# zichunhao/lgn-autoencoder

Measured on AMD Instinct MI355X. Metric: jets/sec fwd+bwd, 30-particle maxdim=2 bs=512, higher is better.
Workload: dtype f64

## Files before the change

### include/lgn_amd.h

```cpp
#ifndef LGN_AMD_H
#define LGN_AMD_H

#include <stddef.h>
#include <stdint.h>

#ifdef __cplusplus
extern "C" {
#endif

#define LGN_AMD_ABI_VERSION 19

int lgn_abi_version(void);
const char* lgn_last_error(void);

int lgn_level_fwd_f64(int B, int N, int C, int CO, int decoder,
                      const double* s_in, const double* v_in, const double* p, const uint8_t* mask,
                      const double* ra, const double* rb, const double* rc,
                      const double* w0, const double* b0, const double* w1, const double* b1,
                      const double* wm0, const double* wm1,
                      double* ag0, double* ag1, double* s_out, double* v_out, void* stream);

int lgn_level_bwd_partial_rows(int B, int N, int decoder, int* rows_mix, int* rows_rad);
int lgn_level_rad_partial_len(int C, int decoder);
int lgn_level_jet_split(int B, int N);

int lgn_level_bwd_f64(int B, int N, int C, int CO, int decoder,
                      const double* s_in, const double* v_in, const double* p, const uint8_t* mask,
                      const double* ra, const double* rb, const double* rc,
                      const double* w0, const double* b0, const double* w1, const double* b1,
                      const double* wm0, const double* wm1, const double* ag0, const double* ag1,
                      const double* g_s_out, const double* g_v_out,
                      double* g_ag, double* g_s_in, double* g_v_in, double* g_p,
                      double* part_mix, double* part_rad, void* stream);

int lgn_cg_product_fwd_f64(int R, int N, int C, int D1, int D2, int DO, int mode, int nnz, const int* row_ptr, const int* col,
                           const double* coef, const double* x1, const double* x2, double* out, void* stream);
int lgn_cg_product_bwd_f64(int R, int N, int C, int D1, int D2, int DO, int mode, int nnz, const int* row_ptr, const int* col,
                           const double* coef, const double* x1, const double* x2, const double* g_out, double* g_x1, double* g_x2,
                           void* stream);

int lgn_reduce_partials_f64(const double* part, int rows, int n, double* out, int accumulate, void* stream);

int lgn_radial_finalize_f64(const double* tot, int C, const double* ra, const double* rb, const double* rc,
                            const double* w0, const double* w1,
                            double* g_a, double* g_b, double* g_c,
                            double* g_w0, double* g_b0, double* g_w1, double* g_b1, void* stream);

#define LGN_ACT_LEAKYRELU 0
#define LGN_ACT_RELU 1
#define LGN_ACT_ELU 2
#define LGN_ACT_SIGMOID 3
#define LGN_ACT_LOGSIGMOID 4
#define LGN_ACT_ATAN 5
#define LGN_ACT_COUNT 6
int lgn_cgmlp_fwd_f64(int M, int C, int H, int nlin, int activation, const double* const* w, const double* const* b,
                      const double* s_in, double* s_out, void* stream);
int lgn_cgmlp_partial_rows(int M, int H);
int lgn_cgmlp_bwd_f64(int M, int C, int H, int nlin, int activation, const double* const* w, const double* const* b,
                      const double* s_in, const double* g_out, double* g_in, double* part, int psize, void* stream);

int lgn_mixreps_fwd_f64(int rows, int Cin, int Cout, int d, const double* w, const double* x, double* y, void* stream);
int lgn_mixreps_partial_rows(int rows);
int lgn_mixreps_bwd_f64(int rows, int Cin, int Cout, int d, const double* w, const double* x, const double* g_y,
                        double* g_x, double* part, void* stream);

int lgn_moments_fwd_f64(int B, int N, int C, int Q, int decoder, const double* X, const double* p, const uint8_t* mask,
                        const double* ra, const double* rb, const double* rc, const double* w0, const double* b0,
                        const double* w1, const double* b1, double* U, void* stream);
long long lgn_moments_scratch_doubles(int B, int N, int C, int decoder);
int lgn_moments_bwd_f64(int B, int N, int C, int Q, int decoder, const double* X, const double* p, const uint8_t* mask,
                        const double* ra, const double* rb, const double* rc, const double* w0, const double* b0,
                        const double* w1, const double* b1, const double* gU, double* gX, double* g_p,
                        double* part_rad, double* scratch, void* stream);

typedef struct lgn_local_tables {
  int n_rows, n_out, n_w;
  int n_terms, n_u, n_x;
  int n_units, static_kind;
  const int *row_ptr, *t_type, *t_a, *t_b;
  const double* t_coef;
  const int *out_dim, *out_nblk, *out_row0, *out_q0, *out_w0;
  const int *u_ptr, *u_row;
  const double* u_coef;
  const int *x_ptr, *x_row, *x_other;
  const double* x_coef;
  int h_out_w0[8];
} lgn_local_tables;

int lgn_local_fwd_f64(int nodes, int C, int CO, int Q, int Qout, const lgn_local_tables* t, const double* X, const double* U,
                      const double* wcat, double* out, void* stream);
int lgn_local_partial_rows(int nodes);
int lgn_local_bwd_f64(int nodes, int C, int CO, int Q, int Qout, const lgn_local_tables* t, const double* X, const double* U,
                      const double* wcat, const double* g_out, double* gU, double* gX, double* part, void* stream);

long long lgn_local_static_packed_doubles(int kind, int C, int CO);
int lgn_local_bwd_static_f64(int kind, int nodes, int C, int CO, const double* XT, const double* UT, const double* wcat,
                             const int* w0, double* wpacked, const double* goT, double* gUT, double* gXT, double* part,
                             double* gpacked, double* g_wcat, void* stream);
int lgn_local_fwd_static_f64(int kind, int nodes, int C, int CO, const double* XT, const double* UT, const double* wcat,
                             const int* w0, double* wpacked, double* outT, double* s_copy, int q_s, void* stream);

typedef struct lgn_net_desc {
  int B, N;
  int n_levels;
  int enc_channels[5];
  int dec_channels[5];
  int tau_s, tau_v;
  int mlp_hidden_mul;
  int mlp_nlin;
  int tau_v_in;
  const lgn_local_tables* enc_tables[4];
  const lgn_local_tables* dec_tables[4];
  int enc_Q[5], enc_qs[5], enc_qv[5];
  int dec_Q[5], dec_qs[5], dec_qv[5];
  int flags;
  int activation;
  int n_in_scalars;
  int latent_pool;
  int dec_N;
  int get_real;
  double jet_loss_scale;
} lgn_net_desc;
#define LGN_REAL_SUM 0
#define LGN_REAL_REAL 1
#define LGN_REAL_IMAG 2
#define LGN_REAL_MEAN 3
#define LGN_REAL_NORM 4
#define LGN_LOSS_CHAMFER 0
#define LGN_LOSS_MSE 1
#define LGN_LOSS_HUNGARIAN 2
typedef struct lgn_loss_desc {
  int kind;
  int abs_coord;
  int polar_coord;
  double scale;
} lgn_loss_desc;
#define LGN_POOL_MIN 0
#define LGN_POOL_MAX 1
#define LGN_POOL_MEAN 2
#define LGN_POOL_MIX 3
#define LGN_POOL(n, avg, o0, o1, o2, o3) ((n) | ((avg) << 3) | ((o0) << 4) | ((o1) << 6) | ((o2) << 8) | ((o3) << 10))
#define LGN_NET_NO_STATIC 1
#define LGN_NET_DEC_PAIRWISE 2
#define LGN_NET_LEVEL_V2 4
#define LGN_NET_MLP_V1 8
#define LGN_NET_MOMENTS_V1 16
#define LGN_NET_BWD_ORDERED 64
#define LGN_NET_DEC_UNFUSED 256
#define LGN_NET_MOMENTS_SPLIT 512
#define LGN_NET_MLP_BWD1 1024
#define LGN_NET_MLP_FULLTILE 2048
#define LGN_NET_SPLIT_TAIL 128

#define LGN_LDS_LIMIT (160 * 1024)
long long lgn_encoder_end_lds_bytes(int N, int C0, int K, int CL, int Ts, int Tv, int pool);
long long lgn_decoder_end_lds_bytes(int N, int C0, int Tin, int CL);
long long lgn_junction_lds_bytes(int N, int CL, int Ts, int Tv, int pool, int C0);

int lgn_step_param_slots(const lgn_net_desc* d, int decoder);
long long lgn_step_workspace_doubles(const lgn_net_desc* d);
int lgn_step_fwd_bwd_f64(const lgn_net_desc* d, const double* params, double* grads, long long n_params,
                         const int64_t* enc_off, const int64_t* dec_off, const double* p4, const double* target,
                         const uint8_t* mask, const double* in_scalars, double* workspace, long long workspace_doubles,
                         double* recon, double* loss_part, const lgn_loss_desc* loss, int* assignment ,
                         int* status , void* stream);
#define LGN_FINALIZE_SCRATCH 2048
int lgn_step_finalize_f64(double* params, double* grads, long long n_params, const double* loss_part, int n_loss,
                          double l1_lambda, double* adam_m, double* adam_v, long long* step_dev,
                          double lr, double beta1, double beta2, double eps, int do_adam, double* loss_out, void* stream);
int lgn_step_train_f64(const lgn_net_desc* d, double* params, double* grads, long long n_params, const int64_t* enc_off,
                       const int64_t* dec_off, const double* p4, const double* target, const uint8_t* mask, const double* in_scalars,
                       double* workspace, long long workspace_doubles, double* recon, double* loss_part, int n_loss, double l1_lambda,
                       double* adam_m, double* adam_v, long long* step_dev, double lr, double beta1, double beta2, double eps,
                       int do_adam, double* loss_out, const lgn_loss_desc* loss, int* assignment ,
                       int* status , void* stream);

#define LGN_OPT_ADAM 0
#define LGN_OPT_RMSPROP 1
typedef struct {
  int kind;
  double l1_lambda, l2_lambda, lr, eps;
  double beta1, beta2;
  double alpha, momentum;
} lgn_optim_desc;
#define LGN_FINALIZE_OPT_SCRATCH 4096
int lgn_step_finalize_opt_f64(double* params, double* grads, long long n_params, const double* loss_part, int n_loss,
                              const lgn_optim_desc* opt, double* state_m, double* state_v, long long* step_dev, int do_step,
                              double* loss_out, void* stream);
int lgn_step_train_opt_f64(const lgn_net_desc* d, double* params, double* grads, long long n_params, const int64_t* enc_off,
                           const int64_t* dec_off, const double* p4, const double* target, const uint8_t* mask,
                           const double* in_scalars, double* workspace, long long workspace_doubles, double* recon,
                           double* loss_part, int n_loss, const lgn_optim_desc* opt, double* state_m, double* state_v,
                           long long* step_dev, int do_step, double* loss_out, const lgn_loss_desc* loss,
                           int* assignment , int* status , void* stream);

long long lgn_eval_workspace_doubles(const lgn_net_desc* d);
int lgn_step_eval_f64(const lgn_net_desc* d, const double* params, const int64_t* enc_off, const int64_t* dec_off,
                      const double* p4_scaled, const double* p4_target, const uint8_t* mask, const double* in_scalars,
                      double* workspace, long long workspace_doubles, double* recon_real, double* lat_s ,
                      double* lat_v , double* loss_part, double* loss_out, const lgn_loss_desc* loss,
                      int* assignment , int* status , void* stream);

long long lgn_net_workspace_doubles(const lgn_net_desc* d, int decoder, int which);
int lgn_encoder_fwd_f64(const lgn_net_desc* d, const double* params, const int64_t* off, const double* p4, const uint8_t* mask,
                        const double* in_scalars, double* act, long long act_doubles, double* lat_s, double* lat_v, void* stream);
int lgn_encoder_bwd_f64(const lgn_net_desc* d, const double* params, double* grads, long long n_params, const int64_t* off,
                        const double* p4, const uint8_t* mask, const double* in_scalars, const double* act, long long act_doubles,
                        const double* g_lat_s, const double* g_lat_v, double* scratch, long long scratch_doubles, void* stream);
int lgn_decoder_fwd_f64(const lgn_net_desc* d, const double* params, const int64_t* off, const double* lat_v, double* act,
                        long long act_doubles, double* recon, void* stream);
int lgn_decoder_bwd_f64(const lgn_net_desc* d, const double* params, double* grads, long long n_params, const int64_t* off,
                        const double* lat_v, const double* act, long long act_doubles, const double* g_recon, double* g_lat_v,
                        double* scratch, long long scratch_doubles, void* stream);

int lgn_chamfer_f64(int B, int N, int M, const double* x, const double* y, int jet_features, double* loss_part, double* gx, double* gy,
                    void* stream);

#define LGN_ANOMALY_NMAX 192
#define LGN_ANOMALY_NSCORES 21
#define LGN_ANOMALY_ALL 0x1FFFFF
#define LGN_ANOMALY_HUNGARIAN 0x403E0
#define LGN_ANOMALY_NO_HUNGARIAN (LGN_ANOMALY_ALL & ~LGN_ANOMALY_HUNGARIAN)
int lgn_anomaly_scores_f64(const double* recons, const double* target, const double* recons_n, const double* target_n, int B, int N,
                           int score_mask, double* scores, int* col4row , int* status, void* stream);

#define LGN_ROC_TILE 2048
#define LGN_ROC_MAX_COLS 65535
#define LGN_ROC_NONFINITE 1
#define LGN_ROC_SINGLE_CLASS 2
#define LGN_ROC_BAD_LABEL 4
#define LGN_ROC_NAN 8
long long lgn_roc_workspace_bytes(long long M, int K);
int lgn_roc_auc_f64(const double* scores, long long M, int ld, int K, const double* labels, double* fpr, double* tpr,
                    double* thresholds, int* length, double* auc, int* flipped, int* status, void* workspace,
                    long long workspace_bytes, void* stream);

#define LGN_EMD_NMAX 191
#define LGN_EMD_INVALID 1
#define LGN_EMD_EMPTY 2
#define LGN_EMD_ITER 4
#define LGN_EMD_INFEASIBLE 8
long long lgn_emd_workspace_bytes(int B, int N);
long long lgn_emd_lds_bytes(int N);
int lgn_emd_f64(const double* ev0, const double* ev1, int B, int n, int m, double R, double* emd, double* flow ,
                double* dual0 , double* dual1 , int* status, void* work, long long work_bytes, void* stream);
int lgn_emd_relative_f64(const double* recons, const double* target, int B, int N, double* emd, int* status, void* work,
                         long long work_bytes, void* stream);
int lgn_emd_debug_max_augmentations(int* out, int reset);

int lgn_linear_sum_assignment_f64(const double* cost, int B, int n, int* col4row, int* status, void* stream);

int lgn_recon_analysis_f64(const double* target, const double* recons, int B, int N, int abs_coord, int find_match,
                           double* part_polar , double* part_polarrel , double* jet_cart, double* jet_polar,
                           double* jet_rel_err, uint8_t* jet_keep, double* rel_err , int* col4row ,
                           uint8_t* is_padded, int* status, void* stream);

int lgn_match_rel_err_f64(const double* target3, const double* recons3, const double* target_polar, const double* recons_polar,
                          const double* target_polarrel, const double* recons_polarrel, int B, int N, double* rel_err,
                          int* col4row , uint8_t* is_padded, int* status, void* stream);

#define LGN_HIST_MAX_EDGES 1025
#define LGN_HIST_MAX_COLS 16
int lgn_histogram_f64(const double* x, long long rows, int ld, int cols, const double* edges, const int* n_edges , int max_edges,
                      const uint8_t* keep , const double* weights , long long* counts, double* wcounts,
                      int max_bins, void* stream);

#define LGN_STATS_TILE 2048
#define LGN_STATS_MAX_COLS 16
#define LGN_STATS_EMPTY 1
#define LGN_STATS_NONFINITE 2
#define LGN_STAT_MEDIAN 0
#define LGN_STAT_IQR 1
#define LGN_STAT_FIRST_QUARTILE 2
#define LGN_STAT_THIRD_QUARTILE 3
#define LGN_STAT_IDR 4
#define LGN_STAT_MAD 5
#define LGN_STAT_MEAN 6
#define LGN_STAT_MAX 7
#define LGN_STAT_MIN 8
#define LGN_STAT_ABS_MIN 9
#define LGN_STAT_STD_DEV 10
#define LGN_STAT_SKEW 11
#define LGN_STAT_KURTOSIS 12
#define LGN_STAT_FWHM 13
#define LGN_STAT_ABS_MEAN 14
#define LGN_STAT_ABS_MEAN_WITHIN_IQR 15
#define LGN_STAT_ABS_MEAN_WITHIN_IDR 16
#define LGN_STAT_Q10 17
#define LGN_STAT_Q90 18
#define LGN_STATS_COUNT 19
long long lgn_column_stats_workspace_bytes(long long rows, int cols);
int lgn_column_stats_f64(const double* x, long long rows, int ld, int cols, const uint8_t* mask , int mask_keep,
                         double alpha, int num_edges, double* stats ,
                         double* edges , long long* kept ,
                         int* status , void* workspace, long long workspace_bytes, void* stream);

int lgn_hist_fwhm_f64(const long long* counts, int max_bins, const double* edges, int max_edges, const int* n_edges , int cols,
                      double* fwhm , void* stream);

#define LGN_JET_IMAGE_MAX_NPIX 64
#define LGN_JET_IMAGE_PARTS 512
long long lgn_jet_images_workspace_bytes(int B, int npix);
int lgn_jet_images_f64(const double* jets, const double* frame_jets , int B, int N, int mode, int npix, double maxR,
                       int first_n, double* images , double* average, void* workspace, long long workspace_bytes,
                       void* stream);

#define LGN_EQUI_TILE 256
#define LGN_EQUI_MAX_PARTS 64
int lgn_transform_jets_f64(const double* p4, const double* R, const int* perm , const double* scalars , int T,
                           int B, int N, int K, double* out, double* scalars_out , void* stream);
long long lgn_rep_deviation_workspace_bytes(int parts, int T, int B, const int* N , const int* C ,
                                            const int* d );
int lgn_rep_deviation_f64(int parts, int T, int B, const double* const* a , const double* const* b ,
                          const double* const* D , const int* N , const int* C , const int* d ,
                          const int* perm , double* stats , void* workspace, long long workspace_bytes,
                          void* stream);

int lgn_hungarian_mse_f64(int B, int N, const double* x, const double* y, int kind, int abs_coord, int polar_coord, double scale,
                          double* loss_part, double* gx, int* assignment , int* status ,
                          void* stream);
long long lgn_assign_loss_lds_bytes(int N, int C);

#define LGN_NORM_NONE 0
#define LGN_NORM_COMPONENT_MAX 1
#define LGN_NORM_OVERALL_MAX 2
#define LGN_NORM_JET_E 3
int lgn_stage_batch_f64(const double* p4, const uint8_t* labels , const double* scalars , int B, int B_pad, int N,
                        int method, double scale, int jet_features, int K, double* p4_in, double* target, uint8_t* mask,
                        double* in_scalars , double* factor, void* stream);
int lgn_denormalize_f64(const double* x0, const double* x1 , const double* factor, int B, int N, double* out0,
                        double* out1 , void* stream);

#define LGN_EPOCH_MAX_COLLECT 4
#define LGN_EPOCH_BAD_INDEX 1
int lgn_stage_gather_f64(const double* p4, const uint8_t* labels , const double* scalars , long long M,
                         const int* index, long long count, const long long* cursor, int B_pad, int N, int method, double scale,
                         int jet_features, int K, double* p4_in, double* target, uint8_t* mask, double* in_scalars ,
                         double* factor, int* status, void* stream);
int lgn_epoch_collect_f64(const double* loss, double* epoch, long long* cursor, long long count, int B, int n,
                          const double* const* src , double* const* dst , const int* row_doubles , void* stream);
int lgn_epoch_reset(long long* cursor, double* epoch, int* status, void* stream);

#ifdef __cplusplus
}
#endif
#endif
```

### lgn-autoencoder_amd/csrc/api_common.cpp

```cpp
#include <stdarg.h>
#include <stdlib.h>

#include "level.hpp"
#include "../../include/lgn_amd.h"

namespace lgn {
static thread_local char g_err[512] = "";
void set_error(const char* fmt, ...) {
  va_list ap;
  va_start(ap, fmt);
  vsnprintf(g_err, sizeof(g_err), fmt, ap);
  va_end(ap);
}
int level_flags_from_env() {
  auto on = [](const char* name) { const char* e = getenv(name); return e && e[0] == '1'; };
  return (on("LGN_AMD_DEC_PAIRWISE") ? LVL_DEC_PAIRWISE : 0) | (on("LGN_AMD_LEVEL_V2") ? LVL_LEVEL_V2 : 0) |
         (on("LGN_AMD_MOMENTS_V1") ? LVL_MOMENTS_V1 : 0) | (on("LGN_AMD_MLP_V1") ? LVL_MLP_V1 : 0) | (on("LGN_AMD_BWD_ORDERED") ? LVL_BWD_ORDERED : 0) |
         (on("LGN_AMD_MOMENTS_SPLIT") ? LVL_MOMENTS_SPLIT : 0) | (on("LGN_AMD_MLP_BWD1") ? LVL_MLP_BWD1 : 0) |
         (on("LGN_AMD_MLP_FULLTILE") ? LVL_MLP_FULLTILE : 0);
}
static_assert(LVL_DEC_PAIRWISE == LGN_NET_DEC_PAIRWISE && LVL_LEVEL_V2 == LGN_NET_LEVEL_V2 && LVL_MOMENTS_V1 == LGN_NET_MOMENTS_V1 &&
                  LVL_MLP_V1 == LGN_NET_MLP_V1 && LVL_MLP_BWD1 == LGN_NET_MLP_BWD1 && LVL_MLP_FULLTILE == LGN_NET_MLP_FULLTILE &&
                  LVL_BWD_ORDERED == LGN_NET_BWD_ORDERED && LVL_MOMENTS_SPLIT == LGN_NET_MOMENTS_SPLIT, "LVL_* and LGN_NET_* are the same bits");
}

extern "C" {
const char* lgn_last_error(void) { return lgn::g_err; }
int lgn_abi_version(void) { return LGN_AMD_ABI_VERSION; }
}
```

### lgn-autoencoder_amd/csrc/level.hpp

```cpp
#pragma once
#include "common.hpp"

namespace lgn {

constexpr int LVL_DEC_PAIRWISE = 2;
constexpr int LVL_LEVEL_V2 = 4;
constexpr int LVL_MLP_V1 = 8;
constexpr int LVL_MOMENTS_V1 = 16;
constexpr int LVL_MLP_BWD1 = 1024;
constexpr int LVL_MLP_FULLTILE = 2048;
constexpr int LVL_MOMENTS_SPLIT = 512;
constexpr int LVL_BWD_ORDERED = 64;
int level_flags_from_env();

template <typename T>
struct LevelArgs {
  int B, N, C, CO;
  const T* s_in;
  const T* v_in;
  const T* p;
  const uint8_t* mask;
  const T *ra, *rb, *rc, *w0, *b0, *w1, *b1;
  const T *wm0, *wm1;
  T* ag0;
  T* ag1;
  T* s_out;
  T* v_out;
  const T* in_w0 = nullptr;
  const T* in_w1 = nullptr;
  T* in_s = nullptr;
  T* in_v = nullptr;
  T* z1 = nullptr;
  size_t z1n = 0;
  T* z2 = nullptr;
  size_t z2n = 0;
  const T* loss_wo1 = nullptr;
  const T* loss_target = nullptr;
  T loss_scale = T(1);
  int loss_real = 0;
  T loss_jscale = T(0);
  T* loss_recon = nullptr;
  T* loss_part = nullptr;
  T* loss_gv = nullptr;
  T* loss_wpart = nullptr;
  int flags = 0;
};

template <typename T>
struct LevelBwdArgs {
  int B, N, C, CO;
  const T *s_in, *v_in, *p;
  const uint8_t* mask;
  const T *ra, *rb, *rc, *w0, *b0, *w1, *b1;
  const T *wm0, *wm1;
  const T *ag0, *ag1;
  const T* g_s_out;
  const T* g_v_out;
  T* g_ag;
  T* g_s_in;
  T* g_v_in;
  T* g_p;
  T* part_mix;
  T* part_rad;
  T* part_in0 = nullptr;
  int flags = 0;
};

__host__ __device__ constexpr int node_stride(int C) { return 10 * C + 4; }

__host__ __device__ constexpr int rad_partial_size(int C, bool dec) {
  return dec ? 2 * C : (2 * 4 * C * NB + 8 * C);
}

inline int level_jet_split(int B, int N) {
  const int groups = (N + 3) / 4;
  int s = 1;
  while (s * 2 <= groups && B * s * 2 <= 512) s *= 2;
  return s;
}

}
```

### lgn-autoencoder_amd/csrc/level_bwd3.hip

```cpp
#include "level_dev.hpp"
#include "ops.hpp"
#include "wave_sum.hpp"

namespace lgn {

typedef double v4d __attribute__((ext_vector_type(4)));

namespace {
__device__ __forceinline__ double dppq(double v, int xor2) {
  int lo = __double2loint(v), hi = __double2hiint(v);
  if (xor2) {
    lo = __builtin_amdgcn_mov_dpp(lo, 0x4E, 0xF, 0xF, true);
    hi = __builtin_amdgcn_mov_dpp(hi, 0x4E, 0xF, 0xF, true);
  } else {
    lo = __builtin_amdgcn_mov_dpp(lo, 0xB1, 0xF, 0xF, true);
    hi = __builtin_amdgcn_mov_dpp(hi, 0xB1, 0xF, 0xF, true);
  }
  return __hiloint2double(hi, lo);
}
__device__ __forceinline__ double quad_sum(double v) {
  v += dppq(v, 0);
  v += dppq(v, 1);
  return v;
}
__device__ __forceinline__ double fast_rcp(double u) {
  double r = __builtin_amdgcn_rcp(u);
  double e = __builtin_fma(-u, r, 1.0);
  r = __builtin_fma(r, e, r);
  e = __builtin_fma(-u, r, 1.0);
  return __builtin_fma(r, e, r);
}
__device__ __forceinline__ void wave_sync() {
  __builtin_amdgcn_fence(__ATOMIC_RELEASE, "workgroup");
  __builtin_amdgcn_wave_barrier();
  __builtin_amdgcn_fence(__ATOMIC_ACQUIRE, "workgroup");
}
template <int C> struct GA3 {
  static constexpr int A3 = 0, A4 = 2 * C, A1 = 4 * C, A2 = 12 * C, SIZE = 20 * C + 2;
};
constexpr int TS = 18;
LGN_STAMP_DECL
}
LGN_STAMP_READER(lgn_debug_stamps_bwd3)

template <int C, bool DEC, int NWV = 4>
struct Bwd3 {
  static constexpr int BLK = 64 * NWV;
  static constexpr int NG = (C + 3) / 4;
  static constexpr int NS = node_stride(C);
  static constexpr int PS = DEC ? 8 : 4;
  static constexpr int TRSZ = DEC ? NWV * 64 : (NWV * (NG + 3) * 16 * TS > NWV * 64 * NG * 12 ? NWV * (NG + 3) * 16 * TS : NWV * 64 * NG * 12);
  static constexpr int MIXP = BLK / (5 * C) < 16 ? BLK / (5 * C) : 16;
  __host__ __device__ static size_t scratch(int N, int CO) {
    size_t p1 = (size_t)N * 10 * CO + 4 * CO * 5 * C + (size_t)N * 20 * C;
    const size_t red = (size_t)MIXP * CO * 5 * C * 4;
    if (red > p1) p1 = red;
    return p1 > (size_t)TRSZ ? p1 : (size_t)TRSZ;
  }
  static constexpr int SMS = 52;
  static constexpr int SEPSZ = DEC ? SMS * C : 0;
  static size_t smem(int N, int CO) {
    return sizeof(double) * ((((size_t)N * NS + 1) & ~size_t(1)) + (size_t)N * (20 * C + 2) + (size_t)N * 10 * C + (size_t)N * PS +
                             scratch(N, CO) + SEPSZ) + N + 16;
  }
};

template <int C, bool DEC, bool SEP, int NWV, bool SYM = false>
__global__ __launch_bounds__(64 * NWV) __attribute__((amdgpu_waves_per_eu(C <= 4 || DEC ? 2 : 1, C <= 4 || DEC ? 2 : 1))) void level_bwd3_kernel(LevelBwdArgs<double> a) {
  static_assert(!SYM || !DEC, "the symmetric sweep is the encoder's");
  using F = Bwd3<C, DEC, NWV>;
  constexpr int BLK = F::BLK;
  using G = GA3<C>;
  constexpr int NG = F::NG, NS = F::NS, PS = F::PS, K = 5 * C;
  const int N = a.N, B = a.B, CO = a.CO;
  const int b = blockIdx.x, tid = threadIdx.x, lane = tid & 63, wave = tid >> 6;
  const int ngroups = (N + 3) >> 2, gper = (ngroups + (int)gridDim.y - 1) / (int)gridDim.y;
  const int glo = min(ngroups, (int)blockIdx.y * gper), ghi = min(ngroups, glo + gper);
  const int nlo = min(N, 4 * glo), nhi = min(N, 4 * ghi);
  const size_t prow = (size_t)b * gridDim.y + blockIdx.y;

  extern __shared__ __align__(16) unsigned char smem_raw[];
  double* nd = reinterpret_cast<double*>(smem_raw);
  double* ga = nd + ((N * NS + 1) & ~1);
  double* gd = ga + N * G::SIZE;
  double* pj = gd + N * 10 * C;
  double* tr = pj + N * PS;
  double* go = tr;
  double* wm = go + N * 10 * CO;
  double* agl = wm + 4 * CO * K;
  double* sm = tr + F::scratch(N, CO);
  uint8_t* mk = reinterpret_cast<uint8_t*>(sm + F::SEPSZ);

  STAMP(0);
  {
    const size_t plo = (size_t)B * N * CO, pa = (size_t)B * N * 2 * C;
    JetRegs<double> jr;
    load_jet_issue<double, C, DEC>(a.s_in, a.v_in, a.p, a.mask, B, N, b, jr);
    const int eg = tid < N * CO ? tid : 0, ea_ = tid < N * 2 * C ? tid : 0, ew = tid < 2 * CO * K ? tid : 0;
    const size_t ig = (size_t)b * N * CO + eg, ia = (size_t)b * N * 2 * C + ea_;
    double rg[10], ra[10];
    rg[0] = a.g_s_out[ig];
    rg[1] = a.g_s_out[plo + ig];
    ra[0] = a.ag0[ia];
    ra[1] = a.ag0[pa + ia];
#pragma unroll
    for (int m = 0; m < 4; ++m) {
      rg[2 + m] = a.g_v_out[ig * 4 + m];
      rg[6 + m] = a.g_v_out[plo * 4 + ig * 4 + m];
      ra[2 + m] = a.ag1[ia * 4 + m];
      ra[6 + m] = a.ag1[(pa + ia) * 4 + m];
    }
    const double w0v = a.wm0[ew], w1v = a.wm1[ew];
    load_jet_commit<double, C, DEC>(a.s_in, a.v_in, a.p, a.mask, B, N, b, jr, nd, pj, mk);
    if (tid < N * CO) {
#pragma unroll
      for (int m = 0; m < 10; ++m) go[tid * 10 + m] = rg[m];
    }
    if (tid < N * 2 * C) {
#pragma unroll
      for (int m = 0; m < 10; ++m) agl[tid * 10 + m] = ra[m];
    }
    if (tid < 2 * CO * K) {
      wm[tid] = w0v;
      wm[2 * CO * K + tid] = w1v;
    }
    for (int e = tid + BLK; e < 2 * CO * K; e += BLK) {
      wm[e] = a.wm0[e];
      wm[2 * CO * K + e] = a.wm1[e];
    }
    for (int e = tid + BLK; e < N * CO; e += BLK) {
      const size_t idx = (size_t)b * N * CO + e;
      double* g = go + e * 10;
      g[0] = a.g_s_out[idx];
      g[1] = a.g_s_out[plo + idx];
#pragma unroll
      for (int m = 0; m < 4; ++m) {
        g[2 + m] = a.g_v_out[idx * 4 + m];
        g[6 + m] = a.g_v_out[plo * 4 + idx * 4 + m];
      }
    }
    for (int e = tid + BLK; e < N * 2 * C; e += BLK) {
      const size_t ea = (size_t)b * N * 2 * C + e;
      double* x = agl + e * 10;
      x[0] = a.ag0[ea];
      x[1] = a.ag0[pa + ea];
#pragma unroll
      for (int m = 0; m < 4; ++m) {
        x[2 + m] = a.ag1[ea * 4 + m];
        x[6 + m] = a.ag1[(pa + ea) * 4 + m];
      }
    }
  }
  __syncthreads();
  STAMP(1);

  {
    const int half = tid >= BLK / 2;
    for (int e = half ? tid - BLK / 2 : tid; e < N * C; e += BLK / 2) {
      const int n = e / C, c = e - n * C;
      const double* w0r = wm + c;
      const double* w1r = wm + 2 * CO * K + c;
      if (half == 0) {
        cx<double> gx0[2] = {{0, 0}, {0, 0}}, gx1[2][4] = {{{0, 0}, {0, 0}, {0, 0}, {0, 0}}, {{0, 0}, {0, 0}, {0, 0}, {0, 0}}};
        for (int o = 0; o < CO; ++o) {
          const double* g = go + (n * CO + o) * 10;
          const cx<double> gs = {g[0], g[1]};
          cx<double> gv[4];
#pragma unroll
          for (int m = 0; m < 4; ++m) gv[m] = {g[2 + m], g[6 + m]};
#pragma unroll
          for (int q = 0; q < 2; ++q) {
            const cx<double> w0 = {w0r[(0 * CO + o) * K + q * C], w0r[(1 * CO + o) * K + q * C]};
            const cx<double> w1 = {w1r[(0 * CO + o) * K + q * C], w1r[(1 * CO + o) * K + q * C]};
            cfmac(gx0[q], gs, w0);
#pragma unroll
            for (int m = 0; m < 4; ++m) cfmac(gx1[q][m], gv[m], w1);
          }
        }
        double* gan = ga + n * G::SIZE;
        gan[G::A3 + 2 * c] = gx0[0].r;  gan[G::A3 + 2 * c + 1] = gx0[0].i;
        gan[G::A4 + 2 * c] = gx0[1].r;  gan[G::A4 + 2 * c + 1] = gx0[1].i;
#pragma unroll
        for (int m = 0; m < 4; ++m) {
          gan[G::A1 + (c * 4 + m) * 2] = gx1[0][m].r;  gan[G::A1 + (c * 4 + m) * 2 + 1] = gx1[0][m].i;
          gan[G::A2 + (c * 4 + m) * 2] = gx1[1][m].r;  gan[G::A2 + (c * 4 + m) * 2 + 1] = gx1[1][m].i;
        }
      } else {
        cx<double> a2 = {0, 0}, a3 = {0, 0}, a4 = {0, 0};
        cx<double> b2[4] = {{0, 0}, {0, 0}, {0, 0}, {0, 0}}, b34[4] = {{0, 0}, {0, 0}, {0, 0}, {0, 0}};
        for (int o = 0; o < CO; ++o) {
          const double* g = go + (n * CO + o) * 10;
          const cx<double> gs = {g[0], g[1]};
          const double* wr0 = w0r + (0 * CO + o) * K;
          const double* wi0 = w0r + (1 * CO + o) * K;
          const double* wr1 = w1r + (0 * CO + o) * K;
          const double* wi1 = w1r + (1 * CO + o) * K;
          cfmac(a2, gs, cx<double>{wr0[2 * C], wi0[2 * C]});
          cfmac(a3, gs, cx<double>{wr0[3 * C], wi0[3 * C]});
          cfmac(a4, gs, cx<double>{wr0[4 * C], wi0[4 * C]});
          const cx<double> w2 = {wr1[2 * C], wi1[2 * C]};
          const cx<double> w34 = {wr1[3 * C] + wr1[4 * C], wi1[3 * C] + wi1[4 * C]};
#pragma unroll
          for (int m = 0; m < 4; ++m) {
            const cx<double> gv = {g[2 + m], g[6 + m]};
            cfmac(b2[m], gv, w2);
            cfmac(b34[m], gv, w34);
          }
        }
        const double* ni = nd + n * NS + c * 10;
        const cx<double> s = {ni[0], ni[1]};
        cx<double> v[4], vt[4];
#pragma unroll
        for (int m = 0; m < 4; ++m) v[m] = {ni[2 + m], ni[6 + m]};
        metric_perm(v, vt);
        cx<double> gs = a2;
        cfmac(gs, cx<double>{2.0 * a4.r, 2.0 * a4.i}, s);
        double* gdn = gd + (n * C + c) * 10;
#pragma unroll
        for (int m = 0; m < 4; ++m) {
          cfmac(gs, b34[m], v[m]);
          cx<double> gv = b2[m];
          cfmac(gv, b34[m], s);
          cfmac(gv, a3, vt[m]);
          gdn[2 + m] = gv.r;
          gdn[6 + m] = gv.i;
        }
        gdn[0] = gs.r;
        gdn[1] = gs.i;
      }
    }
  }
  STAMP(2);
  {
    double* part = a.part_mix + prow * (4 * CO * K);
    constexpr int NPART = F::MIXP;
    const int OK = CO * K, nper = (nhi - nlo + NPART - 1) / NPART;
    const int pi = tid / K, k = tid - pi * K;
    cx<double> d0[8], d1[8];
#pragma unroll
    for (int o = 0; o < 8; ++o) d0[o] = d1[o] = {0, 0};
    if (pi < NPART) {
      const int q = k / C, c = k - q * C;
      const int n1 = min(nhi, nlo + (pi + 1) * nper);
      for (int n = nlo + pi * nper; n < n1; ++n) {
        cx<double> x0, x1[4];
        if (q < 2) {
          const double* x = agl + (n * 2 * C + k) * 10;
          x0 = {x[0], x[1]};
#pragma unroll
          for (int m = 0; m < 4; ++m) x1[m] = {x[2 + m], x[6 + m]};
        } else {
          const double* ni = nd + n * NS + c * 10;
          const cx<double> s = {ni[0], ni[1]};
          cx<double> v[4];
#pragma unroll
          for (int m = 0; m < 4; ++m) v[m] = {ni[2 + m], ni[6 + m]};
          if (q == 2) {
            x0 = s;
#pragma unroll
            for (int m = 0; m < 4; ++m) x1[m] = v[m];
          } else {
            if (q == 3) { x0 = bil2(v, v); x0.r *= 0.5; x0.i *= 0.5; } else x0 = cmul(s, s);
#pragma unroll
            for (int m = 0; m < 4; ++m) x1[m] = cmul(v[m], s);
          }
        }
#pragma unroll
        for (int o = 0; o < 8; ++o)
          if (o < CO) {
            const double* g = go + (n * CO + o) * 10;
            cfmac(d0[o], cx<double>{g[0], g[1]}, x0);
#pragma unroll
            for (int m = 0; m < 4; ++m) cfmac(d1[o], cx<double>{g[2 + m], g[6 + m]}, x1[m]);
          }
      }
    }
    STAMP(48);
    __syncthreads();
    STAMP(49);
    double* red = tr;
    if (pi < NPART) {
#pragma unroll
      for (int o = 0; o < 8; ++o)
        if (o < CO) {
          double* r4 = red + ((pi * CO + o) * K + k) * 4;
          r4[0] = d0[o].r;  r4[1] = d0[o].i;  r4[2] = d1[o].r;  r4[3] = d1[o].i;
        }
    }
    STAMP(50);
    __syncthreads();
    STAMP(51);
    for (int ex = tid; ex < 4 * OK; ex += BLK) {
      const int e = ex >> 2, x = ex & 3;
      double v = red[ex];
#pragma unroll
      for (int pp = 1; pp < NPART; ++pp) v += red[pp * OK * 4 + ex];
      part[x * OK + e] = v;
    }
  }

  if constexpr (DEC && SEP) {
    STAMP(3);
    __syncthreads();
    STAMP(4);
    if (tid < 64) {
      const int k = tid & 7, part = tid >> 3;
      double mean = 0.0;
      for (int n = part; n < N; n += 8) mean += pj[n * 8 + k];
      mean += shfl_xor(mean, 8);
      mean += shfl_xor(mean, 16);
      mean += shfl_xor(mean, 32);
      if (part == 0) sm[k] = mean / N;
    }
    __syncthreads();
    for (int e = tid; e < N * 8; e += BLK) pj[e] -= sm[e & 7];
    __syncthreads();
#define LGN_PUT(k, val)                                       \
  do {                                                        \
    if ((k) < 16) a0[(k) < 16 ? (k) : 0] += (val);                                        \
    else if ((k) < 32) a1[(k) >= 16 && (k) < 32 ? (k) - 16 : 0] += (val);                 \
    else if ((k) < 44) a2[(k) >= 32 && (k) < 44 ? (k) - 32 : 0] += (val);                 \
    else a3[(k) >= 44 ? (k) - 44 : 0] += (val);                                           \
  } while (0)
    for (int c = wave; c < C; c += NWV) {
      double a0[16], a1[16], a2[12], a3[8];
#pragma unroll
      for (int k = 0; k < 16; ++k) a0[k] = a1[k] = 0.0;
#pragma unroll
      for (int k = 0; k < 12; ++k) a2[k] = 0.0;
#pragma unroll
      for (int k = 0; k < 8; ++k) a3[k] = 0.0;
      for (int n = lane; n < N; n += 64) {
        const double* ni = nd + n * NS + c * 10;
        const double* pn = pj + n * 8;
        const double* gi = ga + n * G::SIZE;
        cx<double> pc[4], v[4];
#pragma unroll
        for (int m = 0; m < 4; ++m) {
          pc[m] = {pn[m], pn[4 + m]};
          v[m] = {ni[2 + m], ni[6 + m]};
        }
        const cx<double> sn = {ni[0], ni[1]};
        LGN_PUT(0, sn.r);  LGN_PUT(1, sn.i);
#pragma unroll
        for (int m = 0; m < 4; ++m) {
          LGN_PUT(2 + 2 * m, v[m].r);  LGN_PUT(3 + 2 * m, v[m].i);
          const cx<double> sp = cmul(sn, pc[m]);
          LGN_PUT(10 + 2 * m, sp.r);  LGN_PUT(11 + 2 * m, sp.i);
        }
        const cx<double> vp = bil2(v, pc);
        LGN_PUT(18, vp.r);  LGN_PUT(19, vp.i);
        const cx<double> g3 = {0.5 * gi[G::A3 + 2 * c], 0.5 * gi[G::A3 + 2 * c + 1]};
        LGN_PUT(20, gi[G::A4 + 2 * c]);  LGN_PUT(21, gi[G::A4 + 2 * c + 1]);
        LGN_PUT(22, g3.r);  LGN_PUT(23, g3.i);
        cx<double> gp2 = {0, 0};
#pragma unroll
        for (int m = 0; m < 4; ++m) {
          const cx<double> g1 = {gi[G::A1 + (c * 4 + m) * 2], gi[G::A1 + (c * 4 + m) * 2 + 1]};
          const cx<double> g2 = {gi[G::A2 + (c * 4 + m) * 2], gi[G::A2 + (c * 4 + m) * 2 + 1]};
          LGN_PUT(24 + 2 * m, g1.r);  LGN_PUT(25 + 2 * m, g1.i);
          LGN_PUT(32 + 2 * m, g2.r);  LGN_PUT(33 + 2 * m, g2.i);
          cfmac(gp2, g2, pc[m]);
          const cx<double> gp3 = cmulc(g3, pc[m]);
          LGN_PUT(42 + 2 * m, gp3.r);  LGN_PUT(43 + 2 * m, gp3.i);
        }
        LGN_PUT(40, gp2.r);  LGN_PUT(41, gp2.i);
      }
      double* q = sm + c * F::SMS;
      wave_sum_store<16>(a0, q, lane);
      wave_sum_store<16>(a1, q + 16, lane);
      wave_sum_store<12>(a2, q + 32, lane);
      wave_sum_store<8>(a3, q + 44, lane);
    }
#undef LGN_PUT
    __syncthreads();

    STAMP(5);
    const size_t pls = (size_t)B * N * C;
    for (int e = tid; e < N * C; e += BLK) {
      const int n = e / C, c = e - n * C;
      const double* q = sm + c * F::SMS;
      const double* pn = pj + n * 8;
      const double* gdn = gd + e * 10;
      const cx<double> R0 = {a.b0[c], a.b0[c]}, R1 = {a.b1[c], a.b1[c]};
      const cx<double> e0 = {R0.r - R0.i, R0.r + R0.i};
      cx<double> pc[4], pt[4];
#pragma unroll
      for (int m = 0; m < 4; ++m) pc[m] = {pn[m], pn[4 + m]};
      metric_perm(pc, pt);
      const cx<double> SG4 = {q[20], q[21]}, SG3 = {q[22], q[23]}, GP2 = {q[40], q[41]};
      cx<double> GP3[4], GPT3[4];
#pragma unroll
      for (int m = 0; m < 4; ++m) GP3[m] = {q[42 + 2 * m], q[43 + 2 * m]};
      metric_perm(GP3, GPT3);
      cx<double> u = GP2;
#pragma unroll
      for (int m = 0; m < 4; ++m) {
        const cx<double> t = cmulc(cx<double>{q[32 + 2 * m], q[33 + 2 * m]}, pc[m]);
        u.r -= t.r;  u.i -= t.i;
      }
      cx<double> gs = cmulc(SG4, e0);
      cfmac(gs, u, R1);
      const size_t ge = ((size_t)b * N + n) * C + c;
      a.g_s_in[ge] = gdn[0] + gs.r;
      a.g_s_in[pls + ge] = gdn[1] + gs.i;
#pragma unroll
      for (int m = 0; m < 4; ++m) {
        cx<double> w = GPT3[m];
        const cx<double> t = cmulc(SG3, pt[m]);
        w.r -= t.r;  w.i -= t.i;
        cx<double> gv = cmulc(cx<double>{q[24 + 2 * m], q[25 + 2 * m]}, e0);
        cfmac(gv, w, R1);
        a.g_v_in[ge * 4 + m] = gdn[2 + m] + gv.r;
        a.g_v_in[pls * 4 + ge * 4 + m] = gdn[6 + m] + gv.i;
      }
    }
    STAMP(6);
    {
      const size_t plp = (size_t)B * N * 4;
      for (int e = tid; e < N * 4; e += BLK) {
        const int n = e >> 2, m = e & 3;
        const int mp = m == 1 ? 3 : (m == 3 ? 1 : m);
        const double sg = m == 2 ? -1.0 : 1.0;
        const double* gi = ga + n * G::SIZE;
        cx<double> acc = {0, 0};
        for (int c = 0; c < C; ++c) {
          const double* q = sm + c * F::SMS;
          const double* ni = nd + n * NS + c * 10;
          const cx<double> R1 = {a.b1[c], a.b1[c]};
          const cx<double> S = {q[0], q[1]}, SG3 = {q[22], q[23]};
          const cx<double> VSt = {sg * q[2 + 2 * mp], sg * q[3 + 2 * mp]};
          const cx<double> vt = {sg * ni[2 + mp], sg * ni[6 + mp]};
          const cx<double> g2 = {gi[G::A2 + (c * 4 + m) * 2], gi[G::A2 + (c * 4 + m) * 2 + 1]};
          const cx<double> g3 = {0.5 * gi[G::A3 + 2 * c], 0.5 * gi[G::A3 + 2 * c + 1]};
          cx<double> t = cmulc(g2, S);
          cfmac(t, g3, VSt);
          const cx<double> t2 = cmulc(cx<double>{q[32 + 2 * m], q[33 + 2 * m]}, cx<double>{ni[0], ni[1]});
          t.r -= t2.r;  t.i -= t2.i;
          const cx<double> t3 = cmulc(SG3, vt);
          t.r -= t3.r;  t.i -= t3.i;
          cfmac(acc, t, R1);
        }
        a.g_p[((size_t)b * N + n) * 4 + m] += acc.r;
        a.g_p[plp + ((size_t)b * N + n) * 4 + m] += acc.i;
      }
    }
    if (tid < 2 * C) {
      const int lin = tid / C, c = tid - lin * C;
      const double* q = sm + c * F::SMS;
      const cx<double> S = {q[0], q[1]};
      double* part = a.part_rad + (size_t)blockIdx.x * rad_partial_size(C, true);
      if (lin == 0) {
        cx<double> E0 = cmulc(cx<double>{q[20], q[21]}, S);
#pragma unroll
        for (int m = 0; m < 4; ++m) cfmac(E0, cx<double>{q[24 + 2 * m], q[25 + 2 * m]}, cx<double>{q[2 + 2 * m], q[3 + 2 * m]});
        part[tid] = (E0.r + E0.i) + (E0.i - E0.r);
      } else {
        cx<double> VS[4], VSt[4];
#pragma unroll
        for (int m = 0; m < 4; ++m) VS[m] = {q[2 + 2 * m], q[3 + 2 * m]};
        metric_perm(VS, VSt);
        cx<double> E1 = cmulc(cx<double>{q[40], q[41]}, S);
        cx<double> neg = cmulc(cx<double>{q[22], q[23]}, cx<double>{q[18], q[19]});
#pragma unroll
        for (int m = 0; m < 4; ++m) {
          cfmac(neg, cx<double>{q[32 + 2 * m], q[33 + 2 * m]}, cx<double>{q[10 + 2 * m], q[11 + 2 * m]});
          cfmac(E1, cx<double>{q[42 + 2 * m], q[43 + 2 * m]}, VSt[m]);
        }
        part[tid] = (E1.r - neg.r) + (E1.i - neg.i);
      }
    }
    STAMP(7);
    return;
  }

  STAMP(3);
  const int pr = lane & 15, cg = lane >> 4;
  const int tj = pr >> 2, ti = pr & 3;
  double ak[5], bk[5], ck2[5], wf[NG][5], bias[NG][4];
  if (!DEC) {
#pragma unroll
    for (int s = 0; s < 5; ++s) {
      const int k = 4 * s + cg;
      ak[s] = a.ra[k];
      bk[s] = a.rb[k];
      const double c = a.rc[k];
      ck2[s] = c * c;
    }
#pragma unroll
    for (int g = 0; g < NG; ++g) {
      const int rr = lane & 15, q = rr >> 2, ch = 4 * g + (rr & 3);
      const double* w = (q >> 1) ? a.w1 : a.w0;
#pragma unroll
      for (int s = 0; s < 5; ++s) wf[g][s] = ch < C ? w[(2 * ch + (q & 1)) * NB + 4 * s + cg] : 0.0;
    }
  }
#pragma unroll
  for (int g = 0; g < NG; ++g) {
    const int ch = 4 * g + cg;
#pragma unroll
    for (int q = 0; q < 4; ++q) {
      const double* bb = (q >> 1) ? a.b1 : a.b0;
      bias[g][q] = ch < C ? (DEC ? bb[ch] : bb[2 * ch + (q & 1)]) : 0.0;
    }
  }
  STAMP(4);
  __syncthreads();
  STAMP(5);

  double* trw = tr + wave * (NG + 3) * 16 * TS;
  v4d T[NG][3];
  double dB0[NG], dB1[NG];
#pragma unroll
  for (int g = 0; g < NG; ++g) {
    dB0[g] = dB1[g] = 0.0;
#pragma unroll
    for (int t = 0; t < 3; ++t) T[g][t] = v4d{0, 0, 0, 0};
  }
  const size_t pls = (size_t)B * N * C;
  double in0[NG][4];
#pragma unroll
  for (int g = 0; g < NG; ++g) in0[g][0] = in0[g][1] = in0[g][2] = in0[g][3] = 0.0;
  const int gcount = ghi - glo;
  const int rs = (!SYM && !DEC && NWV == 4 && gcount >= 1 && gcount <= 2) ? NWV / gcount : 1;
  const int rpart = rs > 1 ? wave % rs : 0;
  const int ntl = (N + 3) >> 2, i0lo = rs > 1 ? 4 * (rpart * ntl / rs) : 0, i0hi = rs > 1 ? min(N, 4 * ((rpart + 1) * ntl / rs)) : N;
  for (int u = 0;; ++u) {
    int rg;
    if constexpr (SYM) {
      const int p = wave + NWV * (u >> 1);
      if (p >= (ngroups + 1) >> 1) break;
      rg = (u & 1) ? ngroups - 1 - p : p;
      if ((u & 1) && rg == p) continue;
    } else if (rs > 1) {
      if (u > 0) break;
      rg = glo + wave / rs;
    } else {
      rg = glo + wave + NWV * u;
      if (rg >= ghi) break;
    }
    const int j = rg * 4 + tj;
    const bool jok = j < N;
    const int jj = jok ? j : N - 1;
    double pme[PS];
#pragma unroll
    for (int m = 0; m < PS; ++m) pme[m] = pj[jj * PS + m];
    const bool mj = DEC ? false : (mk[jj] != 0);
    cx<double> Gs[NG], Gv[NG][4], Gq[4];
    cx<double> sj[NG], vj[NG][4], vtj[NG][4];
    cx<double> dvj[NG], svj[NG];
#pragma unroll
    for (int g = 0; g < NG; ++g) {
      Gs[g] = {0, 0};
#pragma unroll
      for (int m = 0; m < 4; ++m) Gv[g][m] = {0, 0};
      const int ch = 4 * g + cg, cs = ch < C ? ch : 0;
      const double* nj = nd + jj * NS + cs * 10;
      sj[g] = {nj[0], nj[1]};
#pragma unroll
      for (int m = 0; m < 4; ++m) vj[g][m] = {nj[2 + m], nj[6 + m]};
      metric_perm(vj[g], vtj[g]);
      dvj[g] = {vj[g][3].r - vj[g][1].r, vj[g][3].i - vj[g][1].i};
      svj[g] = {vj[g][1].r + vj[g][3].r, vj[g][1].i + vj[g][3].i};
    }
#pragma unroll
    for (int m = 0; m < 4; ++m) Gq[m] = {0, 0};

    for (int i0 = i0lo; i0 < i0hi; i0 += 4) {
      if (rg == glo && i0 < 32) STAMP(16 + (i0 >> 2) * 4);
      const int kind = SYM ? ((i0 >> 2) < rg ? 2 : ((i0 >> 2) == rg ? 1 : 0)) : 1;
      const int i = i0 + ti;
      const bool ok = jok && i < N;
      const int ii = i < N ? i : N - 1;
      const double* pii = pj + ii * PS;
      cx<double> q[4];
      v4d R[NG];
      double rho[5], an = 0.0;
      double qd0 = 0.0, qd3 = 0.0, qa = 0.0, qb = 0.0;
      bool on = false;
      if (DEC) {
#pragma unroll
        for (int m = 0; m < 4; ++m) q[m] = {pii[m] - pme[m], pii[4 + m] - pme[4 + m]};
#pragma unroll
        for (int g = 0; g < NG; ++g) R[g] = v4d{bias[g][0], bias[g][1], bias[g][2], bias[g][3]};
      } else {
        const double d0 = pii[0] - pme[0], d1 = pii[1] - pme[1], d2 = pii[2] - pme[2], d3 = pii[3] - pme[3];
        const double q0 = d0 * d0, q1 = d1 * d1, q2 = d2 * d2, q3 = d3 * d3;
        const double nsq = (2.0 * q0 - (((q0 + q1) + q2) + q3)) + 1e-16;
        an = fabs(nsq);
        on = ok && mj && (mk[ii] != 0) && (nsq != 0.0);
        const double h = rsqrt2<double>();
        q[0] = {d0, 0.0};
        q[1] = {d1 * h, -d2 * h};
        q[2] = {d3, 0.0};
        q[3] = {-d1 * h, -d2 * h};
        qd0 = d0;  qd3 = d3;  qa = d1 * h;  qb = d2 * h;
        double beta[5] = {0.0, 0.0, 0.0, 0.0, 0.0};
#pragma unroll
        for (int s = 0; s < 5; ++s) rho[s] = 0.0;
        if (on) {
#pragma unroll
          for (int s = 0; s < 5; ++s) beta[s] = 1.0 + ck2[s] * an;
          rcp5(beta, rho);
#pragma unroll
          for (int s = 0; s < 5; ++s) beta[s] = __builtin_fma(bk[s], rho[s], ak[s]);
        }
#pragma unroll
        for (int g = 0; g < NG; ++g) {
          R[g] = v4d{bias[g][0], bias[g][1], bias[g][2], bias[g][3]};
#pragma unroll
          for (int s = 0; s < 5; ++s) R[g] = __builtin_amdgcn_mfma_f64_16x16x4f64(wf[g][s], beta[s], R[g], 0, 0, 0);
        }
        if (kind != 0) {
          double* xb = trw + NG * 16 * TS;
#pragma unroll
          for (int s = 0; s < 5; ++s) {
            const double x2 = an * rho[s] * rho[s];
            if (s < 4) {
              xb[pr * TS + 4 * s + cg] = rho[s];
              xb[16 * TS + pr * TS + 4 * s + cg] = x2;
            } else {
              xb[32 * TS + pr * TS + cg] = rho[s];
              xb[32 * TS + pr * TS + 4 + cg] = x2;
            }
          }
          xb[32 * TS + pr * TS + 8 + 2 * cg] = cg == 0 ? (on ? 1.0 : 0.0) : 0.0;
          xb[32 * TS + pr * TS + 9 + 2 * cg] = cg == 0 ? (ok ? 1.0 : 0.0) : 0.0;
        }
      }
      if (rg == glo && i0 < 32) STAMP(17 + (i0 >> 2) * 4);
      const double* gi = ga + ii * G::SIZE;
#pragma unroll
      for (int g = 0; g < NG; ++g) {
        const int ch = 4 * g + cg;
        double G0r = 0, G0i = 0, G1r = 0, G1i = 0;
        if (ok && ch < C) {
          const cx<double> R0 = {R[g][0], R[g][1]}, R1 = {R[g][2], R[g][3]};
          const cx<double> e0 = {R0.r - R0.i, R0.r + R0.i};
          const cx<double> gA3 = {0.5 * gi[G::A3 + 2 * ch], 0.5 * gi[G::A3 + 2 * ch + 1]};
          const cx<double> gA4 = {gi[G::A4 + 2 * ch], gi[G::A4 + 2 * ch + 1]};
          cx<double> gA1[4], gA2[4];
#pragma unroll
          for (int m = 0; m < 4; ++m) {
            gA1[m] = {gi[G::A1 + (ch * 4 + m) * 2], gi[G::A1 + (ch * 4 + m) * 2 + 1]};
            gA2[m] = {gi[G::A2 + (ch * 4 + m) * 2], gi[G::A2 + (ch * 4 + m) * 2 + 1]};
          }
          cfmac(Gs[g], gA4, e0);
          cx<double> ge0 = cmulc(gA4, sj[g]);
          cx<double> gR1;
          if (!DEC) {
            const cx<double> dg = {gA2[1].r - gA2[3].r, gA2[1].i - gA2[3].i}, sg = {gA2[1].r + gA2[3].r, gA2[1].i + gA2[3].i};
            cx<double> P2;
            P2.r = __builtin_fma(gA2[0].r, qd0, __builtin_fma(gA2[2].r, qd3, __builtin_fma(qa, dg.r, -qb * sg.i)));
            P2.i = __builtin_fma(gA2[0].i, qd0, __builtin_fma(gA2[2].i, qd3, __builtin_fma(qa, dg.i, qb * sg.r)));
            cfmac(Gs[g], P2, R1);
            const cx<double> Z = cmulc(gA3, R1);
#pragma unroll
            for (int m = 0; m < 4; ++m) cfmac(Gv[g][m], gA1[m], e0);
            Gv[g][0].r = __builtin_fma(Z.r, qd0, Gv[g][0].r);   Gv[g][0].i = __builtin_fma(Z.i, qd0, Gv[g][0].i);
            Gv[g][2].r = __builtin_fma(-Z.r, qd3, Gv[g][2].r);  Gv[g][2].i = __builtin_fma(-Z.i, qd3, Gv[g][2].i);
            const double aZr = qa * Z.r, aZi = qa * Z.i;
            const double bZr = qb * Z.r, bZi = qb * Z.i;
            Gv[g][1].r -= aZr + bZi;  Gv[g][1].i += bZr - aZi;
            Gv[g][3].r += aZr - bZi;  Gv[g][3].i += aZi + bZr;
            gR1 = {0, 0};
            if (kind != 0) {
#pragma unroll
              for (int m = 0; m < 4; ++m) cfmac(ge0, gA1[m], vj[g][m]);
              cx<double> V;
              V.r = __builtin_fma(vj[g][0].r, qd0, __builtin_fma(-vj[g][2].r, qd3, __builtin_fma(qa, dvj[g].r, qb * svj[g].i)));
              V.i = __builtin_fma(vj[g][0].i, qd0, __builtin_fma(-vj[g][2].i, qd3, __builtin_fma(qa, dvj[g].i, -qb * svj[g].r)));
              gR1 = cmulc(P2, sj[g]);
              cfmac(gR1, gA3, V);
            }
            if constexpr (SYM) {
              if (kind == 2) {
                const double* gj = ga + jj * G::SIZE;
                const double* ni = nd + ii * NS + ch * 10;
                const cx<double> si = {ni[0], ni[1]};
                cx<double> vi[4];
#pragma unroll
                for (int m = 0; m < 4; ++m) vi[m] = {ni[2 + m], ni[6 + m]};
                const cx<double> hA3 = {0.5 * gj[G::A3 + 2 * ch], 0.5 * gj[G::A3 + 2 * ch + 1]};
                const cx<double> hA4 = {gj[G::A4 + 2 * ch], gj[G::A4 + 2 * ch + 1]};
                cx<double> he0 = cmulc(hA4, si);
                cx<double> hA2[4];
#pragma unroll
                for (int m = 0; m < 4; ++m) {
                  const cx<double> hA1 = {gj[G::A1 + (ch * 4 + m) * 2], gj[G::A1 + (ch * 4 + m) * 2 + 1]};
                  hA2[m] = {gj[G::A2 + (ch * 4 + m) * 2], gj[G::A2 + (ch * 4 + m) * 2 + 1]};
                  cfmac(he0, hA1, vi[m]);
                }
                const cx<double> hd = {hA2[1].r - hA2[3].r, hA2[1].i - hA2[3].i}, hs = {hA2[1].r + hA2[3].r, hA2[1].i + hA2[3].i};
                cx<double> Q2;
                Q2.r = __builtin_fma(hA2[0].r, qd0, __builtin_fma(hA2[2].r, qd3, __builtin_fma(qa, hd.r, -qb * hs.i)));
                Q2.i = __builtin_fma(hA2[0].i, qd0, __builtin_fma(hA2[2].i, qd3, __builtin_fma(qa, hd.i, qb * hs.r)));
                const cx<double> dvi = {vi[3].r - vi[1].r, vi[3].i - vi[1].i}, svi = {vi[1].r + vi[3].r, vi[1].i + vi[3].i};
                cx<double> W;
                W.r = __builtin_fma(vi[0].r, qd0, __builtin_fma(-vi[2].r, qd3, __builtin_fma(qa, dvi.r, qb * svi.i)));
                W.i = __builtin_fma(vi[0].i, qd0, __builtin_fma(-vi[2].i, qd3, __builtin_fma(qa, dvi.i, -qb * svi.r)));
                cx<double> hR1 = cmulc(Q2, si);
                cfmac(hR1, hA3, W);
                ge0.r += he0.r;  ge0.i += he0.i;
                gR1.r -= hR1.r;  gR1.i -= hR1.i;
              }
            }
          } else {
            cx<double> e1[4], e1t[4];
#pragma unroll
            for (int m = 0; m < 4; ++m) e1[m] = cmul(R1, q[m]);
            metric_perm(e1, e1t);
            gR1 = {0, 0};
#pragma unroll
            for (int m = 0; m < 4; ++m) {
              cfmac(Gv[g][m], gA1[m], e0);
              cfmac(Gv[g][m], gA3, e1t[m]);
              cfmac(Gs[g], gA2[m], e1[m]);
              cfmac(ge0, gA1[m], vj[g][m]);
              cx<double> ge1 = cmulc(gA2[m], sj[g]);
              cfmac(ge1, gA3, vtj[g][m]);
              cfmac(gR1, ge1, q[m]);
              cfmac(Gq[m], ge1, R1);
            }
          }
          G0r = ge0.r + ge0.i;  G0i = ge0.i - ge0.r;
          G1r = gR1.r;  G1i = gR1.i;
        }
        if (DEC) {
          dB0[g] += G0r + G0i;
          dB1[g] += G1r + G1i;
        } else if (kind != 0) {
          double* ta = trw + g * 16 * TS;
          ta[pr * TS + cg] = G0r;
          ta[pr * TS + 4 + cg] = G0i;
          ta[pr * TS + 8 + cg] = G1r;
          ta[pr * TS + 12 + cg] = G1i;
        }
      }
      if (rg == glo && i0 < 32) STAMP(18 + (i0 >> 2) * 4);
      if (!DEC && kind != 0) {
        wave_sync();
        const double* xb = trw + NG * 16 * TS;
#pragma unroll
        for (int s = 0; s < 4; ++s) {
          const int prow = 4 * s + cg;
          double bv[3];
#pragma unroll
          for (int t = 0; t < 3; ++t) bv[t] = xb[t * 16 * TS + prow * TS + pr];
#pragma unroll
          for (int g = 0; g < NG; ++g) {
            const double av = trw[g * 16 * TS + prow * TS + pr];
#pragma unroll
            for (int t = 0; t < 3; ++t) T[g][t] = __builtin_amdgcn_mfma_f64_16x16x4f64(av, bv[t], T[g][t], 0, 0, 0);
          }
        }
        wave_sync();
      }
    }

    if (rg == glo) STAMP(6);
    if (rs > 1) {
      double* mine = trw + lane;
#pragma unroll
      for (int g = 0; g < NG; ++g) {
        Gs[g].r = quad_sum(Gs[g].r);  Gs[g].i = quad_sum(Gs[g].i);
#pragma unroll
        for (int m = 0; m < 4; ++m) { Gv[g][m].r = quad_sum(Gv[g][m].r);  Gv[g][m].i = quad_sum(Gv[g][m].i); }
        if (rpart != 0) {
          mine[(g * 10 + 0) * 64] = Gs[g].r;  mine[(g * 10 + 1) * 64] = Gs[g].i;
#pragma unroll
          for (int m = 0; m < 4; ++m) { mine[(g * 10 + 2 + m) * 64] = Gv[g][m].r;  mine[(g * 10 + 6 + m) * 64] = Gv[g][m].i; }
        }
      }
      __syncthreads();
      if (rpart != 0) break;
      for (int pp = 1; pp < rs; ++pp) {
        const double* oth = trw + pp * (NG + 3) * 16 * TS + lane;
#pragma unroll
        for (int g = 0; g < NG; ++g) {
          Gs[g].r += oth[(g * 10 + 0) * 64];  Gs[g].i += oth[(g * 10 + 1) * 64];
#pragma unroll
          for (int m = 0; m < 4; ++m) { Gv[g][m].r += oth[(g * 10 + 2 + m) * 64];  Gv[g][m].i += oth[(g * 10 + 6 + m) * 64]; }
        }
      }
    }
#pragma unroll
    for (int g = 0; g < NG; ++g) {
      const int ch = 4 * g + cg;
      const double sr = rs > 1 ? Gs[g].r : quad_sum(Gs[g].r), si = rs > 1 ? Gs[g].i : quad_sum(Gs[g].i);
      const bool wr = jok && ti == 0 && ch < C;
      const size_t e = ((size_t)b * N + jj) * C + (ch < C ? ch : 0);
      const double* gdn = gd + (jj * C + (ch < C ? ch : 0)) * 10;
      const double gsr = gdn[0] + sr, gsi = gdn[1] + si;
      if (wr) {
        a.g_s_in[e] = gsr;
        a.g_s_in[pls + e] = gsi;
      }
      cx<double> gvn[4];
#pragma unroll
      for (int m = 0; m < 4; ++m) {
        const double vr = rs > 1 ? Gv[g][m].r : quad_sum(Gv[g][m].r), vi = rs > 1 ? Gv[g][m].i : quad_sum(Gv[g][m].i);
        gvn[m] = {gdn[2 + m] + vr, gdn[6 + m] + vi};
        if (wr) {
          a.g_v_in[e * 4 + m] = gvn[m].r;
          a.g_v_in[pls * 4 + e * 4 + m] = gvn[m].i;
        }
      }
      if constexpr (!DEC) {
        if (a.part_in0 && wr) {
          const double q0 = pme[0] * pme[0], q1 = pme[1] * pme[1], q2 = pme[2] * pme[2], q3 = pme[3] * pme[3];
          const double mass = sqrt(fabs(2.0 * q0 - (((q0 + q1) + q2) + q3)));
          constexpr double H = 0.70710678118654752440084436210484903928;
          const cx<double> q[4] = {{pme[0], 0.0}, {pme[1] * H, -pme[2] * H}, {pme[3], 0.0}, {-pme[1] * H, -pme[2] * H}};
          cx<double> d1 = {0, 0};
#pragma unroll
          for (int m = 0; m < 4; ++m) cfmac(d1, gvn[m], q[m]);
          in0[g][0] += gsr * mass;
          in0[g][1] += gsi * mass;
          in0[g][2] += d1.r;
          in0[g][3] += d1.i;
        }
      }
    }
    if (DEC) {
      const size_t plp = (size_t)B * N * 4;
#pragma unroll
      for (int m = 0; m < 4; ++m) {
        double qr = quad_sum(Gq[m].r), qi = quad_sum(Gq[m].i);
        qr += shfl_xor(qr, 16);  qr += shfl_xor(qr, 32);
        qi += shfl_xor(qi, 16);  qi += shfl_xor(qi, 32);
        if (jok && ti == 0 && cg == 0) {
          a.g_p[((size_t)b * N + jj) * 4 + m] -= qr;
          a.g_p[plp + ((size_t)b * N + jj) * 4 + m] -= qi;
        }
      }
    }
  }

  STAMP(7);
  if (DEC) {
    const int ti2 = pr >> 2, tj2 = pr & 3;
    const size_t plp = (size_t)B * N * 4;
    for (int rg = glo + wave; rg < ghi; rg += NWV) {
      const int i = rg * 4 + ti2;
      const bool iok = i < N;
      const int ii = iok ? i : N - 1;
      const double* gi = ga + ii * G::SIZE;
      cx<double> Gq[4] = {{0, 0}, {0, 0}, {0, 0}, {0, 0}};
      for (int j0 = 0; j0 < N; j0 += 4) {
        const int j = j0 + tj2;
        if (iok && j < N) {
#pragma unroll
          for (int g = 0; g < NG; ++g) {
            const int ch = 4 * g + cg;
            if (ch < C) {
              const double* nj = nd + j * NS + ch * 10;
              const cx<double> s = {nj[0], nj[1]};
              cx<double> v[4], vt[4];
#pragma unroll
              for (int m = 0; m < 4; ++m) v[m] = {nj[2 + m], nj[6 + m]};
              metric_perm(v, vt);
              const cx<double> R1 = {bias[g][2], bias[g][3]};
              const cx<double> gA3 = {0.5 * gi[G::A3 + 2 * ch], 0.5 * gi[G::A3 + 2 * ch + 1]};
#pragma unroll
              for (int m = 0; m < 4; ++m) {
                const cx<double> gA2 = {gi[G::A2 + (ch * 4 + m) * 2], gi[G::A2 + (ch * 4 + m) * 2 + 1]};
                cx<double> ge1 = cmulc(gA2, s);
                cfmac(ge1, gA3, vt[m]);
                cfmac(Gq[m], ge1, R1);
              }
            }
          }
        }
      }
#pragma unroll
      for (int m = 0; m < 4; ++m) {
        double qr = quad_sum(Gq[m].r), qi = quad_sum(Gq[m].i);
        qr += shfl_xor(qr, 16);  qr += shfl_xor(qr, 32);
        qi += shfl_xor(qi, 16);  qi += shfl_xor(qi, 32);
        if (iok && tj2 == 0 && cg == 0) {
          a.g_p[((size_t)b * N + i) * 4 + m] += qr;
          a.g_p[plp + ((size_t)b * N + i) * 4 + m] += qi;
        }
      }
    }
  }

  __shared__ double in0l[NWV][8][4];
  if constexpr (!DEC) {
    if (a.part_in0) {
#pragma unroll
      for (int g = 0; g < NG; ++g)
#pragma unroll
        for (int k = 0; k < 4; ++k) {
          double x = in0[g][k];
          x += shfl_xor(x, 4);
          x += shfl_xor(x, 8);
          if (pr == 0 && 4 * g + cg < C) in0l[wave][4 * g + cg][k] = x;
        }
    }
  }

  STAMP(8);
  __syncthreads();
  STAMP(9);
  if constexpr (!DEC) {
    if (a.part_in0 && tid < 4 * C) {
      const int k = tid / C, c = tid - k * C;
      double s = 0;
#pragma unroll
      for (int w = 0; w < NWV; ++w) s += in0l[w][c][k];
      a.part_in0[prow * 4 * C + k * C + c] = s;
    }
  }
  double* part = a.part_rad + prow * rad_partial_size(C, DEC);
  if (DEC) {
    double* red = tr;
#pragma unroll
    for (int g = 0; g < NG; ++g) {
      double x0 = dB0[g], x1 = dB1[g];
      for (int m = 1; m < 16; m <<= 1) { x0 += shfl_xor(x0, m); x1 += shfl_xor(x1, m); }
      if (pr == 0) {
        red[(wave * NG + g) * 8 + cg] = x0;
        red[(wave * NG + g) * 8 + 4 + cg] = x1;
      }
    }
    __syncthreads();
    if (tid < 2 * C) {
      const int lin = tid / C, ch = tid - lin * C, g = ch >> 2, c4 = ch & 3;
      double s = 0;
      for (int w = 0; w < NWV; ++w) s += red[(w * NG + g) * 8 + lin * 4 + c4];
      part[tid] = s;
    }
  } else {
    double* red = tr;
    {
      double* mine = red + (size_t)(wave * 64 + lane) * NG * 12;
#pragma unroll
      for (int g = 0; g < NG; ++g)
#pragma unroll
        for (int t = 0; t < 3; ++t)
#pragma unroll
          for (int q = 0; q < 4; ++q) mine[(g * 3 + t) * 4 + q] = T[g][t][q];
    }
    __syncthreads();
    const int wq = __builtin_amdgcn_readfirstlane(wave);
    if (wq < 4) {
      constexpr int R = 4 * C;
      const int col = lane & 15;
#pragma unroll
      for (int g = 0; g < NG; ++g) {
        const int ch = 4 * g + cg;
#pragma unroll
        for (int t = 0; t < 3; ++t)
#pragma unroll
          for (int q = 0; q < 4; ++q) {
            if (q != wq) continue;
            const int e = (g * 3 + t) * 4 + q;
            double v = (red[(size_t)(0 * 64 + lane) * NG * 12 + e] + red[(size_t)(1 * 64 + lane) * NG * 12 + e]) +
                       (red[(size_t)(2 * 64 + lane) * NG * 12 + e] + red[(size_t)(3 * 64 + lane) * NG * 12 + e]);
            if (NWV == 8)
              v += (red[(size_t)(4 * 64 + lane) * NG * 12 + e] + red[(size_t)(5 * 64 + lane) * NG * 12 + e]) +
                   (red[(size_t)(6 * 64 + lane) * NG * 12 + e] + red[(size_t)(7 * 64 + lane) * NG * 12 + e]);
            if (ch >= C) continue;
            const int r = (q >> 1) * 2 * C + 2 * ch + (q & 1);
            if (t == 0) part[r * NB + col] = v;
            else if (t == 1) part[R * NB + r * NB + col] = v;
            else {
              if (col < 4) part[r * NB + 16 + col] = v;
              else if (col < 8) part[R * NB + r * NB + 16 + (col - 4)] = v;
              else if (col == 8) part[2 * R * NB + r] = v;
              else if (col == 9) part[2 * R * NB + R + r] = v;
            }
          }
      }
    }
  }
  STAMP(10);
}

bool level_bwd3_fits(int N) { return N <= 40; }

template <int C, bool DEC, bool SEP, int NWV>
static int launch_bwd3_w(const LevelBwdArgs<double>& a, int split, hipStream_t stream) {
  size_t smem = Bwd3<C, DEC, NWV>::smem(a.N, a.CO);
  LGN_CHECK_ARG(smem <= 160 * 1024, "level_bwd: N=%d C=%d needs %zu B of LDS", a.N, a.C, smem);
  LGN_CHECK_ARG(a.CO <= 8, "level_bwd: C_out=%d unsupported (1..8)", a.CO);
  auto kern = level_bwd3_kernel<C, DEC, SEP, NWV>;
  if constexpr (!DEC && C <= 4) {
    if (split == 1 && !(a.flags & LVL_BWD_ORDERED)) kern = level_bwd3_kernel<C, DEC, SEP, NWV, true>;
  }
  if (smem > 64 * 1024) (void)hipFuncSetAttribute(reinterpret_cast<const void*>(kern), hipFuncAttributeMaxDynamicSharedMemorySize, (int)smem);
  hipLaunchKernelGGL(kern, dim3(a.B, split), dim3(64 * NWV), smem, stream, a);
  LGN_CHECK_LAUNCH();
  return 0;
}
template <int C, bool DEC, bool SEP>
static int launch_bwd3(const LevelBwdArgs<double>& a, hipStream_t stream) {
  return launch_bwd3_w<C, DEC, SEP, 4>(a, SEP ? 1 : level_jet_split(a.B, a.N), stream);
}

int level_bwd3_dispatch(const LevelBwdArgs<double>& a, int decoder, hipStream_t stream) {
  const bool pairwise = (a.flags & LVL_DEC_PAIRWISE) != 0;
#define LGN_CASE(CC)                                                                \
  case CC:                                                                          \
    if (!decoder) return launch_bwd3<CC, false, false>(a, stream);                  \
    return pairwise ? launch_bwd3<CC, true, false>(a, stream) : launch_bwd3<CC, true, true>(a, stream);
  switch (a.C) {
#ifdef LGN_DEV_ONLY_C4
    LGN_CASE(4)
#else
    LGN_CASE(1) LGN_CASE(2) LGN_CASE(3) LGN_CASE(4) LGN_CASE(5) LGN_CASE(6) LGN_CASE(7) LGN_CASE(8)
#endif
    default: set_error("level_bwd: C_in=%d unsupported (1..8)", a.C); return -1;
  }
#undef LGN_CASE
}

}
```

### lgn-autoencoder_amd/csrc/level_fwd2.hip

```cpp
#include "level_dev.hpp"
#include "net_dev.hpp"
#include "ops.hpp"
#include "wave_sum.hpp"

namespace lgn {

typedef double v4d __attribute__((ext_vector_type(4)));
LGN_STAMP_DECL
LGN_STAMP_READER(lgn_debug_stamps_fwd2)

__device__ __forceinline__ double dpp_quad(double v, int ctrl_is_xor2) {
  int lo = __double2loint(v), hi = __double2hiint(v);
  if (ctrl_is_xor2) {
    lo = __builtin_amdgcn_mov_dpp(lo, 0x4E, 0xF, 0xF, true);
    hi = __builtin_amdgcn_mov_dpp(hi, 0x4E, 0xF, 0xF, true);
  } else {
    lo = __builtin_amdgcn_mov_dpp(lo, 0xB1, 0xF, 0xF, true);
    hi = __builtin_amdgcn_mov_dpp(hi, 0xB1, 0xF, 0xF, true);
  }
  return __hiloint2double(hi, lo);
}
__device__ __forceinline__ double quad_sum(double v) {
  v += dpp_quad(v, 0);
  v += dpp_quad(v, 1);
  return v;
}

__device__ __forceinline__ double fast_rcp(double u) {
  double r = __builtin_amdgcn_rcp(u);
  double e = __builtin_fma(-u, r, 1.0);
  r = __builtin_fma(r, e, r);
  e = __builtin_fma(-u, r, 1.0);
  return __builtin_fma(r, e, r);
}

template <int C, bool DEC>
struct Fwd2 {
  static constexpr int NG = (C + 3) / 4;
  static constexpr int NS = node_stride(C);
  static constexpr int PS = DEC ? 8 : 4;
  static constexpr int AGS = 20 * C;
  static constexpr int A3 = 0, A4 = 2 * C, A1 = 4 * C, A2 = 12 * C;
};

template <int C, bool DEC, bool SEP, bool TRAIN>
__global__ __launch_bounds__(2 * BLOCK) void level_fwd2_kernel(LevelArgs<double> a, int chunk) {
  using F = Fwd2<C, DEC>;
  constexpr int NG = F::NG;
  const int N = a.N, B = a.B, CO = a.CO;
  const int b = blockIdx.x, tid = threadIdx.x, lane = tid & 63, wave = tid >> 6;
  const int nthr = blockDim.x, nw = nthr >> 6;

  extern __shared__ __align__(16) unsigned char smem_raw[];
  double* nd = reinterpret_cast<double*>(smem_raw);
  double* pj = nd + ((N * F::NS + 1) & ~1);
  double* wm = pj + N * F::PS;
  double* agl = wm + 4 * CO * 5 * C;
  double* sums = agl + chunk * F::AGS;
  uint8_t* mk = reinterpret_cast<uint8_t*>(sums + 20 * C);

  STAMP(0);
  if (!DEC && a.in_w0) {
    {
      const size_t wg = (size_t)blockIdx.y * gridDim.x + blockIdx.x, stride = (size_t)gridDim.x * gridDim.y * nthr;
      for (size_t e = wg * nthr + tid; e < a.z1n; e += stride) a.z1[e] = 0.0;
      for (size_t e = wg * nthr + tid; e < a.z2n; e += stride) a.z2[e] = 0.0;
    }
    const double* p0 = a.p + (size_t)b * N * 4;
    const size_t plane_s = (size_t)B * N * C;
    const int nw2 = 2 * CO * 5 * C;
    for (int e = tid; e < N * 4; e += nthr) pj[e] = p0[e];
    for (int e = tid; e < N; e += nthr) mk[e] = a.mask[(size_t)b * N + e];
    for (int e = tid; e < nw2; e += nthr) {
      wm[e] = a.wm0[e];
      wm[nw2 + e] = a.wm1[e];
    }
    for (int e = tid; e < N * C; e += nthr) {
      const int j = e / C, c = e - j * C;
      const double* p = p0 + j * 4;
      const double pe = p[0], px = p[1], py = p[2], pz = p[3];
      const double q0 = pe * pe, q1 = px * px, q2 = py * py, q3 = pz * pz;
      const double mass = sqrt(fabs(2.0 * q0 - (((q0 + q1) + q2) + q3)));
      constexpr double H = 0.70710678118654752440084436210484903928;
      const cx<double> q[4] = {{pe, 0.0}, {px * H, -py * H}, {pz, 0.0}, {-px * H, -py * H}};
      const double w0r = a.in_w0[c], w0i = a.in_w0[C + c];
      const cx<double> w1 = {a.in_w1[c], a.in_w1[C + c]};
      double* d = nd + j * F::NS + c * 10;
      d[0] = w0r * mass;
      d[1] = w0i * mass;
#pragma unroll
      for (int m = 0; m < 4; ++m) {
        const cx<double> r = cmul(w1, q[m]);
        d[2 + m] = r.r;
        d[6 + m] = r.i;
      }
      if (blockIdx.y == 0) {
        const size_t ge = (size_t)b * N * C + e;
        a.in_s[ge] = d[0];
        a.in_s[plane_s + ge] = d[1];
#pragma unroll
        for (int m = 0; m < 4; ++m) {
          a.in_v[ge * 4 + m] = d[2 + m];
          a.in_v[plane_s * 4 + ge * 4 + m] = d[6 + m];
        }
      }
    }
  } else {
    JetRegs<double> jr;
    load_jet_issue<double, C, DEC>(a.s_in, a.v_in, a.p, a.mask, B, N, b, jr);
    const int nw2 = 2 * CO * 5 * C, ew = tid < nw2 ? tid : 0;
    const double w0v = a.wm0[ew], w1v = a.wm1[ew];
    load_jet_commit<double, C, DEC>(a.s_in, a.v_in, a.p, a.mask, B, N, b, jr, nd, pj, mk);
    if (tid < nw2) {
      wm[tid] = w0v;
      wm[nw2 + tid] = w1v;
    }
    for (int e = tid + nthr; e < nw2; e += nthr) {
      wm[e] = a.wm0[e];
      wm[nw2 + e] = a.wm1[e];
    }
  }

  const int pr = lane & 15, cg = lane >> 4;
  const int ti = pr >> 2, tj = pr & 3;
  double ak[5], bk[5], ck2[5];
  double wf[NG][5];
  double bias[NG][4];
  if (!DEC) {
#pragma unroll
    for (int s = 0; s < 5; ++s) {
      const int k = 4 * s + cg;
      ak[s] = a.ra[k];
      bk[s] = a.rb[k];
      const double c = a.rc[k];
      ck2[s] = c * c;
    }
#pragma unroll
    for (int g = 0; g < NG; ++g) {
      const int rr = lane & 15, q = rr >> 2, ch = 4 * g + (rr & 3);
      const double* w = (q >> 1) ? a.w1 : a.w0;
#pragma unroll
      for (int s = 0; s < 5; ++s) wf[g][s] = ch < C ? w[(2 * ch + (q & 1)) * NB + 4 * s + cg] : 0.0;
    }
  }
#pragma unroll
  for (int g = 0; g < NG; ++g) {
    const int ch = 4 * g + cg;
#pragma unroll
    for (int q = 0; q < 4; ++q) {
      const double* bb = (q >> 1) ? a.b1 : a.b0;
      bias[g][q] = ch < C ? (DEC ? bb[ch] : bb[2 * ch + (q & 1)]) : 0.0;
    }
  }
  __syncthreads();
  STAMP(1);

  if constexpr (DEC && SEP) {
    if (tid < 64) {
      const int k = tid & 7, part = tid >> 3;
      double mean = 0.0;
      for (int n = part; n < N; n += 8) mean += pj[n * 8 + k];
      mean += shfl_xor(mean, 8);
      mean += shfl_xor(mean, 16);
      mean += shfl_xor(mean, 32);
      if (part == 0) sums[k] = mean / N;
    }
    __syncthreads();
    for (int e = tid; e < N * 8; e += nthr) pj[e] -= sums[e & 7];
    __syncthreads();
#define LGN_PUT(k, val)                                           \
  do {                                                            \
    if ((k) < 12) a0[(k) < 12 ? (k) : 0] += (val);                \
    else a1[(k) >= 12 ? (k) - 12 : 0] += (val);                   \
  } while (0)
    for (int c = wave; c < C; c += nw) {
      double a0[12], a1[8];
#pragma unroll
      for (int k = 0; k < 12; ++k) a0[k] = 0.0;
#pragma unroll
      for (int k = 0; k < 8; ++k) a1[k] = 0.0;
      for (int n = lane; n < N; n += 64) {
        const double* ni = nd + n * F::NS + c * 10;
        const double* pn = pj + n * 8;
        const cx<double> sn = {ni[0], ni[1]};
        cx<double> v[4], pc[4];
#pragma unroll
        for (int m = 0; m < 4; ++m) {
          v[m] = {ni[2 + m], ni[6 + m]};
          pc[m] = {pn[m], pn[4 + m]};
        }
        LGN_PUT(0, sn.r);  LGN_PUT(1, sn.i);
#pragma unroll
        for (int m = 0; m < 4; ++m) {
          LGN_PUT(2 + 2 * m, v[m].r);  LGN_PUT(3 + 2 * m, v[m].i);
          const cx<double> sp = cmul(sn, pc[m]);
          LGN_PUT(10 + 2 * m, sp.r);  LGN_PUT(11 + 2 * m, sp.i);
        }
        const cx<double> vp = bil2(v, pc);
        LGN_PUT(18, vp.r);  LGN_PUT(19, vp.i);
      }
      wave_sum_store<12>(a0, sums + c * 20, lane);
      wave_sum_store<8>(a1, sums + c * 20 + 12, lane);
    }
#undef LGN_PUT
    __syncthreads();
  }

  const int ngroups = (N + 3) >> 2, gper = (ngroups + (int)gridDim.y - 1) / (int)gridDim.y;
  const int rlo = min(N, 4 * (int)blockIdx.y * gper), rhi = min(N, rlo + 4 * gper);
  auto catmix = [&](int c0, int c1) {
    constexpr int K = 5 * C;
    const int nr = c1 - c0;
    const size_t plo = (size_t)B * N * CO;
    if (wave == 0) {
      for (int rl = lane; rl < nr; rl += 64) {
        const int r = c0 + rl;
        const double* st = agl + rl * F::AGS;
        const double* ni = nd + r * F::NS;
        cx<double> x[K];
#pragma unroll
        for (int c = 0; c < C; ++c) {
          const cx<double> sc = {ni[c * 10], ni[c * 10 + 1]};
          cx<double> v[4];
#pragma unroll
          for (int mm = 0; mm < 4; ++mm) v[mm] = {ni[c * 10 + 2 + mm], ni[c * 10 + 6 + mm]};
          cx<double> vv = bil2(v, v);
          vv.r *= 0.5;  vv.i *= 0.5;
          x[c] = {st[F::A3 + 2 * c], st[F::A3 + 2 * c + 1]};
          x[C + c] = {st[F::A4 + 2 * c], st[F::A4 + 2 * c + 1]};
          x[2 * C + c] = sc;
          x[3 * C + c] = vv;
          x[4 * C + c] = cmul(sc, sc);
        }
#pragma unroll 2
        for (int o = 0; o < CO; ++o) {
          const double* wr = wm + (0 * CO + o) * K;
          const double* wi = wm + (1 * CO + o) * K;
          cx<double> acc = {0, 0};
#pragma unroll
          for (int k = 0; k < K; ++k) cfma(acc, cx<double>{wr[k], wi[k]}, x[k]);
          const size_t e = ((size_t)b * N + r) * CO + o;
          a.s_out[e] = acc.r;
          a.s_out[plo + e] = acc.i;
        }
      }
    } else {
      for (int it = lane + 64 * (wave - 1); it < nr * 4; it += 64 * (nw - 1)) {
        const int rl = it >> 2, m = it & 3, r = c0 + rl;
        const double* st = agl + rl * F::AGS;
        const double* ni = nd + r * F::NS;
        cx<double> x[K];
#pragma unroll
        for (int c = 0; c < C; ++c) {
          const cx<double> sc = {ni[c * 10], ni[c * 10 + 1]};
          const cx<double> v = {ni[c * 10 + 2 + m], ni[c * 10 + 6 + m]};
          x[c] = {st[F::A1 + (c * 4 + m) * 2], st[F::A1 + (c * 4 + m) * 2 + 1]};
          x[C + c] = {st[F::A2 + (c * 4 + m) * 2], st[F::A2 + (c * 4 + m) * 2 + 1]};
          x[2 * C + c] = v;
          x[3 * C + c] = x[4 * C + c] = cmul(v, sc);
        }
#pragma unroll 2
        for (int o = 0; o < CO; ++o) {
          const double* wr = wm + 2 * CO * K + (0 * CO + o) * K;
          const double* wi = wm + 2 * CO * K + (1 * CO + o) * K;
          cx<double> acc = {0, 0};
#pragma unroll
          for (int k = 0; k < K; ++k) cfma(acc, cx<double>{wr[k], wi[k]}, x[k]);
          const size_t e = ((size_t)b * N + r) * CO + o;
          a.v_out[e * 4 + m] = acc.r;
          a.v_out[plo * 4 + e * 4 + m] = acc.i;
        }
      }
    }
    };
  for (int c0 = rlo; c0 < rhi; c0 += chunk) {
  const int c1 = min(rhi, c0 + chunk);
  if constexpr (DEC && SEP) {
    for (int e = tid; e < (c1 - c0) * C; e += nthr) {
      const int rl = e / C, c = e - rl * C, n = c0 + rl;
      const double* sm = sums + c * 20;
      const double* pn = pj + n * 8;
      const cx<double> R0 = {a.b0[c], a.b0[c]}, R1 = {a.b1[c], a.b1[c]};
      const cx<double> e0 = {R0.r - R0.i, R0.r + R0.i};
      const cx<double> S = {sm[0], sm[1]};
      cx<double> VS[4], pc[4];
#pragma unroll
      for (int m = 0; m < 4; ++m) {
        VS[m] = {sm[2 + 2 * m], sm[3 + 2 * m]};
        pc[m] = {pn[m], pn[4 + m]};
      }
      double* st = agl + rl * F::AGS;
      const cx<double> a4 = cmul(S, e0);
      cx<double> t = bil2(VS, pc);
      t.r -= sm[18];  t.i -= sm[19];
      cx<double> a3 = cmul(R1, t);
      st[F::A3 + 2 * c] = 0.5 * a3.r;  st[F::A3 + 2 * c + 1] = 0.5 * a3.i;
      st[F::A4 + 2 * c] = a4.r;        st[F::A4 + 2 * c + 1] = a4.i;
#pragma unroll
      for (int m = 0; m < 4; ++m) {
        const cx<double> a1 = cmul(VS[m], e0);
        cx<double> u = cmul(pc[m], S);
        u.r -= sm[10 + 2 * m];  u.i -= sm[11 + 2 * m];
        const cx<double> a2 = cmul(R1, u);
        st[F::A1 + (c * 4 + m) * 2] = a1.r;  st[F::A1 + (c * 4 + m) * 2 + 1] = a1.i;
        st[F::A2 + (c * 4 + m) * 2] = a2.r;  st[F::A2 + (c * 4 + m) * 2 + 1] = a2.i;
      }
    }
  } else {
  const int ngr = (c1 - c0 + 3) >> 2;
  const int rs = (!DEC && nw == 4 && ngr >= 1 && ngr <= 2 && chunk >= 16) ? 4 / ngr : 1;
  const int rpart = rs > 1 ? wave % rs : 0, ntl = (N + 3) >> 2;
  auto row_group = [&](const int rg, const int jlo, const int jhi, const int slab) __attribute__((always_inline)) {
    const int i0 = rg * 4;
    const int i = i0 + ti;
    const bool iok = i < N;
    const int ii = iok ? i : N - 1;
    double pi[F::PS];
#pragma unroll
    for (int m = 0; m < F::PS; ++m) pi[m] = pj[ii * F::PS + m];
    const bool mi = DEC ? false : (mk[ii] != 0);

    cx<double> A1[NG][4], A2[NG][4], A3[NG], A4[NG];
#pragma unroll
    for (int g = 0; g < NG; ++g) {
      A3[g] = {0, 0};
      A4[g] = {0, 0};
#pragma unroll
      for (int m = 0; m < 4; ++m) { A1[g][m] = {0, 0}; A2[g][m] = {0, 0}; }
    }

    STAMP(2 + ((rg >> 2) & 3) * 4);
    struct Tile {
      cx<double> q[4];
      double qd0, qd3, qa, qb;
      v4d R[NG];
      int jj;
      bool ok;
    };
    auto prep = [&](int j0, Tile& T) {
      const int j = j0 + tj;
      T.ok = iok && j < N;
      T.jj = j < N ? j : N - 1;
      const double* pjj = pj + T.jj * F::PS;
      if (DEC) {
#pragma unroll
        for (int m = 0; m < 4; ++m) T.q[m] = {pi[m] - pjj[m], pi[4 + m] - pjj[4 + m]};
#pragma unroll
        for (int g = 0; g < NG; ++g) T.R[g] = v4d{bias[g][0], bias[g][1], bias[g][2], bias[g][3]};
      } else {
        const double d0 = pi[0] - pjj[0], d1 = pi[1] - pjj[1], d2 = pi[2] - pjj[2], d3 = pi[3] - pjj[3];
        const double q0 = d0 * d0, q1 = d1 * d1, q2 = d2 * d2, q3 = d3 * d3;
        const double nsq = (2.0 * q0 - (((q0 + q1) + q2) + q3)) + 1e-16;
        const double an = fabs(nsq);
        const bool on = T.ok && mi && (mk[T.jj] != 0) && (nsq != 0.0);
        const double h = rsqrt2<double>();
        T.qd0 = d0;  T.qd3 = d3;  T.qa = d1 * h;  T.qb = d2 * h;
        double beta[5] = {0.0, 0.0, 0.0, 0.0, 0.0};
        if (on) {
#pragma unroll
          for (int s = 0; s < 5; ++s) beta[s] = 1.0 + ck2[s] * an;
          double rho5[5];
          rcp5(beta, rho5);
#pragma unroll
          for (int s = 0; s < 5; ++s) beta[s] = __builtin_fma(bk[s], rho5[s], ak[s]);
        }
#pragma unroll
        for (int g = 0; g < NG; ++g) {
          T.R[g] = v4d{bias[g][0], bias[g][1], bias[g][2], bias[g][3]};
#pragma unroll
          for (int s = 0; s < 5; ++s) T.R[g] = __builtin_amdgcn_mfma_f64_16x16x4f64(wf[g][s], beta[s], T.R[g], 0, 0, 0);
        }
      }
    };
    auto agg = [&](const Tile& T) {
      if (T.ok) {
        const double* nj = nd + T.jj * F::NS;
#pragma unroll
        for (int g = 0; g < NG; ++g) {
          const int ch = 4 * g + cg;
          if (ch < C) {
            const cx<double> R0 = {T.R[g][0], T.R[g][1]}, R1 = {T.R[g][2], T.R[g][3]};
            const cx<double> e0 = {R0.r - R0.i, R0.r + R0.i};
            const cx<double> sj = {nj[ch * 10], nj[ch * 10 + 1]};
            cx<double> vj[4];
#pragma unroll
            for (int m = 0; m < 4; ++m) {
              vj[m] = {nj[ch * 10 + 2 + m], nj[ch * 10 + 6 + m]};
              cfma(A1[g][m], vj[m], e0);
            }
            cfma(A4[g], sj, e0);
            if (!DEC) {
              const double qd0 = T.qd0, qd3 = T.qd3, qa = T.qa, qb = T.qb;
              const cx<double> Tm = cmul(sj, R1);
              A2[g][0].r = __builtin_fma(Tm.r, qd0, A2[g][0].r);  A2[g][0].i = __builtin_fma(Tm.i, qd0, A2[g][0].i);
              A2[g][2].r = __builtin_fma(Tm.r, qd3, A2[g][2].r);  A2[g][2].i = __builtin_fma(Tm.i, qd3, A2[g][2].i);
              const double aTr = qa * Tm.r, aTi = qa * Tm.i, bTr = qb * Tm.r, bTi = qb * Tm.i;
              A2[g][1].r += aTr + bTi;  A2[g][1].i += aTi - bTr;
              A2[g][3].r += bTi - aTr;  A2[g][3].i -= aTi + bTr;
              const cx<double> dv = {vj[3].r - vj[1].r, vj[3].i - vj[1].i}, sv = {vj[1].r + vj[3].r, vj[1].i + vj[3].i};
              cx<double> V;
              V.r = __builtin_fma(vj[0].r, qd0, __builtin_fma(-vj[2].r, qd3, __builtin_fma(qa, dv.r, qb * sv.i)));
              V.i = __builtin_fma(vj[0].i, qd0, __builtin_fma(-vj[2].i, qd3, __builtin_fma(qa, dv.i, -qb * sv.r)));
              cfma(A3[g], R1, V);
            } else {
              cx<double> e1[4];
#pragma unroll
              for (int m = 0; m < 4; ++m) {
                e1[m] = cmul(R1, T.q[m]);
                cfma(A2[g][m], sj, e1[m]);
              }
              const cx<double> t = bil2(vj, e1);
              A3[g].r += t.r;
              A3[g].i += t.i;
            }
          }
        }
      }
    };
    if (jlo < jhi) {
      Tile ta, tb;
      prep(jlo, ta);
      int j0 = jlo;
      while (true) {
        if (j0 + 4 < jhi) prep(j0 + 4, tb);
        agg(ta);
        j0 += 4;
        if (j0 >= jhi) break;
        if (j0 + 4 < jhi) prep(j0 + 4, ta);
        agg(tb);
        j0 += 4;
        if (j0 >= jhi) break;
      }
    }

    STAMP(3 + ((rg >> 2) & 3) * 4);
#pragma unroll
    for (int g = 0; g < NG; ++g) {
      A3[g].r = quad_sum(A3[g].r) * 0.5;  A3[g].i = quad_sum(A3[g].i) * 0.5;
      A4[g].r = quad_sum(A4[g].r);        A4[g].i = quad_sum(A4[g].i);
#pragma unroll
      for (int m = 0; m < 4; ++m) {
        A1[g][m].r = quad_sum(A1[g][m].r);  A1[g][m].i = quad_sum(A1[g][m].i);
        A2[g][m].r = quad_sum(A2[g][m].r);  A2[g][m].i = quad_sum(A2[g][m].i);
      }
    }
    if (tj == 0) {
      double* st = agl + (slab + i0 + ti - c0) * F::AGS;
#pragma unroll
      for (int g = 0; g < NG; ++g) {
        const int ch = 4 * g + cg;
        if (ch < C) {
          st[F::A3 + 2 * ch] = A3[g].r;  st[F::A3 + 2 * ch + 1] = A3[g].i;
          st[F::A4 + 2 * ch] = A4[g].r;  st[F::A4 + 2 * ch + 1] = A4[g].i;
#pragma unroll
          for (int m = 0; m < 4; ++m) {
            st[F::A1 + (ch * 4 + m) * 2] = A1[g][m].r;  st[F::A1 + (ch * 4 + m) * 2 + 1] = A1[g][m].i;
            st[F::A2 + (ch * 4 + m) * 2] = A2[g][m].r;  st[F::A2 + (ch * 4 + m) * 2 + 1] = A2[g][m].i;
          }
        }
      }
    }
    STAMP(4 + ((rg >> 2) & 3) * 4);
  };
  if (rs > 1) {
    const int rg = (c0 >> 2) + wave / rs;
    if (rg * 4 < c1) row_group(rg, 4 * (rpart * ntl / rs), min(N, 4 * ((rpart + 1) * ntl / rs)), rpart * 4 * ngr);
  } else {
    for (int rg = (c0 >> 2) + wave; rg * 4 < c1; rg += nw) row_group(rg, 0, N, 0);
  }
  if (rs > 1) {
    __syncthreads();
    const int tot = 4 * ngr * F::AGS;
    for (int e = tid; e < tot; e += nthr) {
      double v = agl[e];
      for (int pp = 1; pp < rs; ++pp) v += agl[pp * tot + e];
      agl[e] = v;
    }
  }
  }
  __syncthreads();
  STAMP(20);

  if constexpr (TRAIN) {
    const size_t pl0 = (size_t)B * N * 2 * C;
    for (int e = tid; e < (c1 - c0) * 2 * C; e += nthr) {
      const int n = e / (2 * C), r = e - n * 2 * C, blk = r / C, ch = r - blk * C;
      const double* st = agl + n * F::AGS + (blk ? F::A4 : F::A3) + 2 * ch;
      const size_t ge = ((size_t)b * N + c0) * 2 * C + e;
      a.ag0[ge] = st[0];
      a.ag0[pl0 + ge] = st[1];
    }
    for (int e = tid; e < (c1 - c0) * 2 * C * 4; e += nthr) {
      const int n = e / (8 * C), r = e - n * 8 * C, blk = r / (4 * C), cm = r - blk * 4 * C;
      const double* st = agl + n * F::AGS + (blk ? F::A2 : F::A1) + 2 * cm;
      const size_t ge = ((size_t)b * N + c0) * 8 * C + e;
      a.ag1[ge] = st[0];
      a.ag1[pl0 * 4 + ge] = st[1];
    }
  }
  STAMP(21);

  catmix(c0, c1);
  STAMP(22);
  if (c1 < rhi) __syncthreads();
  }
  STAMP(40);
  if constexpr (DEC) {
    if (a.loss_wo1) {
      __syncthreads();
      dec_output_loss_body<TRAIN>(B, N, CO, a.v_out, a.loss_wo1, a.loss_target, a.loss_scale, a.loss_real, a.loss_jscale,
                                  a.loss_recon, a.loss_part, a.loss_gv, a.loss_wpart, smem_raw);
    }
  }
}

template <int C, bool DEC, bool SEP, bool TRAIN>
static int launch_level_fwd2(const LevelArgs<double>& a, hipStream_t stream) {
  using F = Fwd2<C, DEC>;
  const size_t fixed = sizeof(double) * (((size_t)a.N * F::NS + 1 & ~size_t(1)) + (size_t)a.N * F::PS + 4 * a.CO * 5 * C + 20 * C) + a.N + 16;
  const bool wide = a.B <= 320 && a.N >= 64;
  const size_t row = sizeof(double) * F::AGS, budget1 = 160 * 1024, budget2 = wide ? budget1 : 78 * 1024;
  const int full = (a.N + 15) & ~15;
  int chunk = full;
  if (fixed + full * row > budget2) {
    const size_t room = fixed + 16 * row <= budget2 ? budget2 - fixed : (fixed < budget1 ? budget1 - fixed : 0);
    chunk = (int)(room / row) & ~15;
    if (chunk > full) chunk = full;
    if (chunk < 16) chunk = 16;
  }
  size_t smem = fixed + chunk * row;
  if (a.loss_wo1) {
    LGN_CHECK_ARG(DEC && SEP && a.N <= 40 && !wide && a.loss_target && a.loss_recon && a.loss_part && (!TRAIN || (a.loss_gv && a.loss_wpart)),
                  "level_fwd: the loss rides on the separable decoder forward of jets of <= 40 particles only");
    if (smem < dec_out_loss_bytes(a.N, a.CO)) smem = dec_out_loss_bytes(a.N, a.CO);
  }
  LGN_CHECK_ARG(smem <= 160 * 1024, "level_fwd: N=%d C=%d needs %zu B of LDS (> 160 KiB)", a.N, a.C, smem);
  auto kern = level_fwd2_kernel<C, DEC, SEP, TRAIN>;
  if (smem > 64 * 1024) {
    hipError_t e = hipFuncSetAttribute(reinterpret_cast<const void*>(kern), hipFuncAttributeMaxDynamicSharedMemorySize, (int)smem);
    if (e != hipSuccess) { set_error("hipFuncSetAttribute: %s", hipGetErrorString(e)); return (int)e; }
  }
  const int nthreads = wide ? 2 * BLOCK : BLOCK;
  const int split = (SEP || a.N > 40) ? 1 : level_jet_split(a.B, a.N);
  hipLaunchKernelGGL(kern, dim3(a.B, split), dim3(nthreads), smem, stream, a, chunk);
  LGN_CHECK_LAUNCH();
  return 0;
}

bool level_fwd_carries_loss(int N, int flags) { return N <= 40 && !(flags & LVL_DEC_PAIRWISE); }

template <bool TRAIN>
static int level_fwd_run(const LevelArgs<double>& a, int decoder, hipStream_t stream) {
  LGN_CHECK_ARG(a.B > 0 && a.N > 0, "level_fwd: empty batch (B=%d N=%d)", a.B, a.N);
  LGN_CHECK_ARG(!a.in_w0 || (!decoder && a.in_w1 && a.in_s && a.in_v), "level_fwd: the input stage rides on encoder levels only");
  LGN_CHECK_ARG(a.CO >= 1 && a.CO <= 8, "level_fwd: C_out=%d unsupported (1..8)", a.CO);
  const bool pairwise = (a.flags & LVL_DEC_PAIRWISE) != 0;
#define LGN_CASE(CC)                                                                                         \
  case CC:                                                                                                   \
    if (!decoder) return launch_level_fwd2<CC, false, false, TRAIN>(a, stream);                              \
    return pairwise ? launch_level_fwd2<CC, true, false, TRAIN>(a, stream) : launch_level_fwd2<CC, true, true, TRAIN>(a, stream);
  switch (a.C) {
#ifdef LGN_DEV_ONLY_C4
    LGN_CASE(4)
#else
    LGN_CASE(1) LGN_CASE(2) LGN_CASE(3) LGN_CASE(4) LGN_CASE(5) LGN_CASE(6) LGN_CASE(7) LGN_CASE(8)
#endif
    default:
      set_error("level_fwd: C_in=%d unsupported (1..8)", a.C);
      return -1;
  }
#undef LGN_CASE
}

template <>
int level_fwd_dispatch<double>(const LevelArgs<double>& a, int decoder, hipStream_t stream) {
  return level_fwd_run<true>(a, decoder, stream);
}

int level_fwd_eval(const LevelArgs<double>& a, int decoder, hipStream_t stream) { return level_fwd_run<false>(a, decoder, stream); }

}
```

### lgn-autoencoder_amd/csrc/step.hip

```cpp
#include <stdlib.h>

#include <algorithm>
#include <mutex>
#include <vector>

#include "net.hpp"
#include "../../include/lgn_amd.h"

namespace lgn {
namespace {

struct Bump {
  double* base;
  size_t off = 0;
  double* take(size_t n) {
    n = (n + 15) & ~size_t(15);
    double* p = base ? base + off : nullptr;
    off += n;
    return p;
  }
};

struct NetBuf {
  double *s[5], *v[5], *smix[4], *ag0[4], *ag1[4];
  double* hsave[4];
};

struct Work {
  NetBuf enc, dec;
  double *lat_s, *lat_v, *pdec, *g_lat_s, *g_lat_v, *g_p;
  double *gs[2], *gv[2], *gsmix, *g_ag, *zeros_s;
  double *parts;
  size_t parts_size;
  double* tot[2][4];
  int* idx;
  size_t total;
  double* tail_cnt;
  double* zero0() const { return tail_cnt < zeros_s ? tail_cnt : zeros_s; }
  size_t zero_doubles;
};

struct Deferred {
  std::vector<RedSeg<double>> segs;
  double* parts;
  size_t off = 0, cap = 0;
  double* take(size_t n) {
    n = (n + 15) & ~size_t(15);
    if (off + n > cap) return nullptr;
    double* p = parts + off;
    off += n;
    return p;
  }
  void add(const double* part, int rows, int stride, int col0, int n, double* out) {
    if (n > 0) segs.push_back(RedSeg<double>{part, rows, stride, col0, n, out});
  }
  int flush(hipStream_t st) {
    for (size_t i = 0; i < segs.size(); i += RED_MAX_SEG) {
      RedJob<double> job{};
      for (size_t k = i; k < segs.size() && k < i + RED_MAX_SEG; ++k) job.seg[job.nseg++] = segs[k];
      if (int rc = reduce_segments<double>(job, st)) return rc;
    }
    segs.clear();
    return 0;
  }
};

int finish_reductions(Deferred& dq, const RadFinJob& fin, double* grads, long long n_params, double* counters, int flags, hipStream_t st) {
  if (counters && !(flags & LGN_NET_SPLIT_TAIL)) {
    StepTailArgs ro{};
    ro.g = grads;
    ro.n = (long)n_params;
    ro.reduce_only = 1;
    ro.counters = reinterpret_cast<unsigned long long*>(counters);
    const int rc = step_tail(dq.segs, fin, ro, st);
    if (rc == 0) { dq.segs.clear(); return 0; }
    if (rc != -2) return rc;
  }
  if (int rc = dq.flush(st)) return rc;
  return rad_finalize_batch(fin, st);
}

int finalize_tail(const StepTailArgs& t, hipStream_t st) {
  if (t.opt_form) return finalize_step_opt(t, st);
  return finalize_step(t.w, t.g, t.n, t.loss_part, t.nB, t.lambda, t.m, t.v, t.step_dev, t.lr, t.beta1, t.beta2, t.eps, t.do_adam,
                       t.loss_out, st);
}

int end_step(Deferred& dq, const RadFinJob& fin, double* grads, long long n_params, double* counters, int flags, const StepTailArgs* tail,
             hipStream_t st) {
  if (tail && !(flags & LGN_NET_SPLIT_TAIL)) {
    const int rc = step_tail(dq.segs, fin, *tail, st);
    if (rc != -2) return rc;
  }
  if (int rc = finish_reductions(dq, fin, grads, n_params, tail ? nullptr : counters, flags, st)) return rc;
  if (!tail) return 0;
  return finalize_tail(*tail, st);
}

inline int in_K(const lgn_net_desc& d) { return d.n_in_scalars > 1 ? d.n_in_scalars : 1; }

int mlp_psize(int C, int H, int nlin) {
  const int D = 2 * C;
  return nlin == 1 ? D * D + D : (H * D + H) + (nlin - 2) * (H * H + H) + (D * H + D);
}

inline int dec_nodes(const lgn_net_desc& d) { return d.dec_N > 0 ? d.dec_N : d.N; }
inline bool step_is_split(const lgn_net_desc& d) { return dec_nodes(d) != d.N || d.n_in_scalars > 1; }
inline int dec_tin(const lgn_net_desc& d) { return d.tau_v_in > 0 ? d.tau_v_in : pool_blocks(d.latent_pool) * d.tau_v; }
int check_latent_match(const lgn_net_desc& d) {
  const int Tin = pool_blocks(d.latent_pool) * d.tau_v;
  LGN_CHECK_ARG(d.tau_v_in == 0 || d.tau_v_in == Tin, "step: the decoder must consume the encoder's %d pooled latent vectors", Tin);
  return 0;
}

struct Slots {
  int L, nlin;
  int in0(bool dec) const { return dec ? 2 : 0; }
  int rad(bool dec, int l, int k) const { return in0(dec) + 2 + 7 * l + k; }
  int mix(bool dec, int l, int k) const { return in0(dec) + 2 + 7 * L + 2 * l + k; }
  int mlp(bool dec, int l, int k) const { return in0(dec) + 2 + 9 * L + 2 * nlin * l + k; }
  int out0(bool dec) const { return in0(dec) + 2 + 9 * L + 2 * nlin * L; }
  int count(bool dec) const { return out0(dec) + 2; }
};

struct RowLayout {
  int width, nseg, col[3], n[3], slot[3];
  void add(Deferred& dq, const double* part, int rows, double* G, const int64_t* off) const {
    for (int i = 0; i < nseg; ++i) dq.add(part, rows, width, col[i], n[i], G + off[slot[i]]);
  }
};
RowLayout enc_latent_rows(const lgn_net_desc& d, int N, int CL) {
  const int KL = pool_mix_in(d.latent_pool, N, CL), o = Slots{d.n_levels, d.mlp_nlin}.out0(false);
  return {2 * (d.tau_s + d.tau_v) * KL, 2, {0, 2 * d.tau_s * KL}, {2 * d.tau_s * KL, 2 * d.tau_v * KL}, {o, o + 1}};
}
RowLayout enc_input_rows(int K, int C0) { return {(2 * K + 2) * C0, 2, {0, 2 * C0 * K}, {2 * C0 * K, 2 * C0}, {0, 1}}; }
RowLayout dec_input_rows(int C0, int N, int Tin) {
  return {4 * C0 + 2 * N * Tin, 3, {0, 2 * C0, 4 * C0}, {2 * C0, 2 * C0, 2 * N * Tin}, {2, 3, 1}};
}
RowLayout dec_output_rows(const lgn_net_desc& d, int CL) {
  return {2 * CL, 1, {0}, {2 * CL}, {Slots{d.n_levels, d.mlp_nlin}.out0(true) + 1}};
}

inline size_t r16(size_t n) { return (n + 15) & ~size_t(15); }
size_t end_parts(const lgn_net_desc& d, bool dec, int N, int in_rows) {
  const int* ch = dec ? d.dec_channels : d.enc_channels;
  const int L = d.n_levels;
  if (dec) return r16((size_t)d.B * dec_output_rows(d, ch[L]).width) + r16((size_t)d.B * dec_input_rows(ch[0], N, dec_tin(d)).width);
  return r16((size_t)d.B * enc_latent_rows(d, N, ch[L]).width) + r16((size_t)in_rows * enc_input_rows(in_K(d), ch[0]).width);
}
size_t net_parts(const lgn_net_desc& d, bool dec, int N) {
  const int* ch = dec ? d.dec_channels : d.enc_channels;
  int rm, rr;
  level_bwd_partial_rows(d.B, N, dec, d.flags, &rm, &rr);
  size_t sum = 0;
  for (int l = 0; l < d.n_levels; ++l) {
    const int H = d.mlp_hidden_mul * 2 * ch[l + 1];
    sum += r16((size_t)rm * 4 * ch[l + 1] * 5 * ch[l]) + r16((size_t)rr * rad_partial_size(ch[l], dec)) +
           r16((size_t)mlp_partial_rows(d.B * (dec ? dec_nodes(d) : N), H) * mlp_psize(ch[l + 1], H, d.mlp_nlin));
  }
  return sum + end_parts(d, dec, N, rm > d.B ? rm : d.B);
}

Work carve(const lgn_net_desc& d, double* base) {
  Work w{};
  Bump b{base};
  const int Nd = dec_nodes(d), Nmax = d.N > Nd ? d.N : Nd;
  const size_t BNe = (size_t)d.B * d.N, BNd = (size_t)d.B * Nd, BN = (size_t)d.B * Nmax;
  const int L = d.n_levels;
  int cmax = 0;
  for (int l = 0; l <= L; ++l) cmax = cmax > d.enc_channels[l] ? cmax : d.enc_channels[l], cmax = cmax > d.dec_channels[l] ? cmax : d.dec_channels[l];
  auto net = [&](NetBuf& n, const int* ch, bool dec) {
    const size_t BN = dec ? BNd : BNe;
    for (int l = 0; l <= L; ++l) {
      n.s[l] = b.take(2 * BN * ch[l]);
      n.v[l] = b.take(8 * BN * ch[l]);
    }
    for (int l = 0; l < L; ++l) {
      n.smix[l] = b.take(2 * BN * ch[l + 1]);
      n.ag0[l] = b.take(4 * BN * ch[l]);
      n.ag1[l] = b.take(16 * BN * ch[l]);
      const size_t hs = l + 1 < L && BN <= mlp_save_max_rows()
                            ? mlp_saved_doubles((int)BN, d.mlp_hidden_mul * 2 * ch[l + 1], d.mlp_nlin) : 0;
      n.hsave[l] = hs ? b.take(hs) : nullptr;
    }
  };
  net(w.enc, d.enc_channels, false);
  net(w.dec, d.dec_channels, true);
  const int Ts = d.tau_s, Tv = d.tau_v, PB = pool_blocks(d.latent_pool);
  w.lat_s = b.take((size_t)2 * d.B * PB * Ts);
  w.lat_v = b.take((size_t)2 * d.B * PB * Tv * 4);
  w.g_lat_v = b.take((size_t)2 * d.B * PB * Tv * 4);
  w.pdec = b.take(8 * BN);
  for (int q = 0; q < 2; ++q) {
    w.gs[q] = b.take(2 * BN * cmax);
    w.gv[q] = b.take(8 * BN * cmax);
  }
  w.gsmix = b.take(2 * BN * cmax);
  w.g_ag = b.take(20 * BN * cmax);
  {
    const size_t z0 = b.off;
    w.zeros_s = b.take(2 * BN * cmax);
    w.g_p = b.take(8 * BN);
    w.g_lat_s = b.take((size_t)2 * d.B * PB * d.tau_s);
    w.tail_cnt = b.take(8);
    w.zero_doubles = b.off - z0;
  }
  w.idx = reinterpret_cast<int*>(b.take(((size_t)d.B * 2 * (Ts + Tv) * 2 + 1) / 2 + 8));
  for (int dec = 0; dec < 2; ++dec)
    for (int l = 0; l < L; ++l) w.tot[dec][l] = b.take(rad_partial_size((dec ? d.dec_channels : d.enc_channels)[l], dec != 0) + 16);
  const size_t psum = net_parts(d, false, d.N) + net_parts(d, true, Nd);
  w.parts = b.take(psum);
  w.parts_size = psum;
  w.total = b.off;
  return w;
}

#define HIPOK(e) do { hipError_t e_ = (e); if (e_ != hipSuccess) { set_error("%s: %s", #e, hipGetErrorString(e_)); return (int)e_; } } while (0)
#define DQ_NEW(var, n) double* var = nullptr; DQ_TAKE(var, n)
#define DQ_TAKE(lhs, n)                                                                                           \
  lhs = dq.take(n);                                                                                             \
  LGN_CHECK_ARG((lhs) != nullptr, "partial-row workspace overflow: %zu + %zu doubles > capacity %zu (carve / take mismatch)", \
                dq.off, (size_t)(n), dq.cap)
#define LGN_TRY(expr)            \
  do {                           \
    int rc_ = (expr);            \
    if (rc_ != 0) return rc_;    \
  } while (0)

struct InputStage {
  const double *w0, *w1;
  double* z1 = nullptr;
  size_t z1n = 0;
  double* z2 = nullptr;
  size_t z2n = 0;
};
struct LossStage {
  const double *wo1, *target;
  double scale;
  int method;
  double jscale;
  double *recon, *loss_part, *g_v, *wpart;
};

MlpArgs<double> level_mlp_args(const lgn_net_desc& d, bool dec, int l, const double* P, const int64_t* off) {
  const Slots S{d.n_levels, d.mlp_nlin};
  const int CO = (dec ? d.dec_channels : d.enc_channels)[l + 1];
  MlpArgs<double> m{};
  m.M = d.B * d.N; m.C = CO; m.H = d.mlp_hidden_mul * 2 * CO; m.nlin = d.mlp_nlin; m.act = d.activation; m.flags = d.flags;
  for (int q = 0; q < d.mlp_nlin; ++q) { m.w[q] = P + off[S.mlp(dec, l, 2 * q)]; m.b[q] = P + off[S.mlp(dec, l, 2 * q + 1)]; }
  return m;
}

int levels_fwd(const lgn_net_desc& d, bool dec, const int* ch, const double* P, const int64_t* off, NetBuf& n, const double* pos,
               const uint8_t* mask, hipStream_t st, const InputStage* in0 = nullptr, const LossStage* loss = nullptr, bool eval = false,
               bool last_scalars = true) {
  const Slots S{d.n_levels, d.mlp_nlin};
  for (int l = 0; l < d.n_levels; ++l) {
    auto p = [&](int slot) { return P + off[slot]; };
    LevelArgs<double> a{d.B, d.N, ch[l], ch[l + 1], n.s[l], n.v[l], pos, mask,
                        p(S.rad(dec, l, 0)), p(S.rad(dec, l, 1)), p(S.rad(dec, l, 2)), p(S.rad(dec, l, 3)), p(S.rad(dec, l, 4)),
                        p(S.rad(dec, l, 5)), p(S.rad(dec, l, 6)), p(S.mix(dec, l, 0)), p(S.mix(dec, l, 1)),
                        n.ag0[l], n.ag1[l], n.smix[l], n.v[l + 1]};
    if (l == 0 && !dec && in0) {
      a.in_w0 = in0->w0; a.in_w1 = in0->w1; a.in_s = n.s[0]; a.in_v = n.v[0];
      a.z1 = in0->z1; a.z1n = in0->z1n; a.z2 = in0->z2; a.z2n = in0->z2n;
    }
    if (l + 1 == d.n_levels && dec && loss) {
      a.loss_wo1 = loss->wo1; a.loss_target = loss->target; a.loss_scale = loss->scale; a.loss_real = loss->method;
      a.loss_jscale = loss->jscale; a.loss_recon = loss->recon;
      a.loss_part = loss->loss_part; a.loss_gv = loss->g_v; a.loss_wpart = loss->wpart;
    }
    a.flags = d.flags;
    LGN_TRY(eval ? level_fwd_eval(a, dec, st) : level_fwd_dispatch<double>(a, dec, st));
    if (l + 1 == d.n_levels && (!last_scalars || (eval && dec))) break;
    MlpArgs<double> m = level_mlp_args(d, dec, l, P, off);
    m.s_in = n.smix[l]; m.s_out = n.s[l + 1];
    m.h_saved = n.hsave[l]; m.h_rows = mlp_saved_rows(m.M);
    LGN_TRY(mlp_dispatch<double>(m, false, st));
  }
  return 0;
}

int levels_bwd(const lgn_net_desc& d, bool dec, const int* ch, const double* P, double* G, const int64_t* off, const NetBuf& n,
               const double* pos, const uint8_t* mask, Work& w, Deferred& dq, RadFinJob& fin, int& cur, bool has_s_grad,
               hipStream_t st, bool* in0_done = nullptr) {
  const Slots S{d.n_levels, d.mlp_nlin};
  const int BN = d.B * d.N;
  for (int l = d.n_levels - 1; l >= 0; --l) {
    auto p = [&](int slot) { return P + off[slot]; };
    auto g = [&](int slot) { return G + off[slot]; };
    const int C = ch[l], CO = ch[l + 1];
    const double* g_smix = w.zeros_s;
    if (has_s_grad) {
      MlpArgs<double> m = level_mlp_args(d, dec, l, P, off);
      m.s_in = n.smix[l]; m.g_out = w.gs[cur]; m.g_in = w.gsmix;
      m.h_saved = n.hsave[l];
      m.h_rows = mlp_saved_rows(BN);
      m.psize = mlp_psize(CO, m.H, m.nlin);
      DQ_TAKE(m.part, (size_t)mlp_partial_rows(BN, m.H) * m.psize);
      LGN_TRY(mlp_dispatch<double>(m, true, st));
      dq.add(m.part, mlp_partial_rows(BN, m.H), m.psize, 0, m.psize, g(S.mlp(dec, l, 0)));
      g_smix = w.gsmix;
    }
    int rm, rr;
    level_bwd_partial_rows(d.B, d.N, dec, d.flags, &rm, &rr);
    const int nmix = 4 * CO * 5 * C, nrad = rad_partial_size(C, dec);
    DQ_NEW(part_mix, (size_t)rm * nmix);
    DQ_NEW(part_rad, (size_t)rr * nrad);
    const int nxt = cur ^ 1;
    LevelBwdArgs<double> a{d.B, d.N, C, CO, n.s[l], n.v[l], pos, mask,
                           p(S.rad(dec, l, 0)), p(S.rad(dec, l, 1)), p(S.rad(dec, l, 2)), p(S.rad(dec, l, 3)), p(S.rad(dec, l, 4)),
                           p(S.rad(dec, l, 5)), p(S.rad(dec, l, 6)), p(S.mix(dec, l, 0)), p(S.mix(dec, l, 1)), n.ag0[l], n.ag1[l],
                           g_smix, w.gv[cur], w.g_ag, w.gs[nxt], w.gv[nxt], dec ? w.g_p : nullptr, part_mix, part_rad};
    const bool carry_in0 = !dec && l == 0 && in0_done && level_bwd_carries_input(d.N, d.flags);
    const RowLayout rin = enc_input_rows(1, C);
    if (carry_in0) { DQ_TAKE(a.part_in0, (size_t)rm * rin.width); }
    a.flags = d.flags;
    LGN_TRY(level_bwd_dispatch<double>(a, dec, st));
    if (carry_in0) {
      rin.add(dq, a.part_in0, rm, G, off);
      *in0_done = true;
    }
    dq.add(part_mix, rm, nmix, 0, nmix / 2, g(S.mix(dec, l, 0)));
    dq.add(part_mix, rm, nmix, nmix / 2, nmix / 2, g(S.mix(dec, l, 1)));
    if (dec) {
      dq.add(part_rad, rr, nrad, 0, C, g(S.rad(dec, l, 4)));
      dq.add(part_rad, rr, nrad, C, C, g(S.rad(dec, l, 6)));
    } else {
      double* tot = w.tot[0][l];
      dq.add(part_rad, rr, nrad, 0, nrad, tot);
      fin.it[fin.n++] = RadFinJob::Item{tot, C, p(S.rad(dec, l, 0)), p(S.rad(dec, l, 1)), p(S.rad(dec, l, 2)), p(S.rad(dec, l, 3)),
                                        p(S.rad(dec, l, 5)), g(S.rad(dec, l, 0)), g(S.rad(dec, l, 1)), g(S.rad(dec, l, 2)),
                                        g(S.rad(dec, l, 3)), g(S.rad(dec, l, 4)), g(S.rad(dec, l, 5)), g(S.rad(dec, l, 6))};
    }
    cur = nxt;
    has_s_grad = true;
  }
  return 0;
}

int check_desc(const lgn_net_desc* d) {
  LGN_CHECK_ARG(d, "step: null descriptor");
  LGN_CHECK_ARG(d->B > 0 && d->N > 0, "step: empty batch (B=%d N=%d)", d->B, d->N);
  LGN_CHECK_ARG(d->n_levels >= 1 && d->n_levels <= 4, "step: n_levels=%d unsupported (1..4)", d->n_levels);
  LGN_CHECK_ARG(d->mlp_nlin >= 4 && d->mlp_nlin <= 7, "step: mlp_depth must be 3 .. 6 (4 .. 7 Linear layers), got %d layers", d->mlp_nlin);
  LGN_CHECK_ARG(d->tau_s >= 1 && d->tau_v >= 1 && d->tau_v_in >= 0, "step: latent multiplicities must be positive");
  LGN_CHECK_ARG(d->n_in_scalars >= 0 && d->n_in_scalars <= 8, "step: n_in_scalars=%d unsupported (0..8)", d->n_in_scalars);
  LGN_CHECK_ARG(pool_valid(d->latent_pool), "step: latent_pool=%d is not an LGN_POOL(...) code", d->latent_pool);
  for (int l = 0; l <= d->n_levels; ++l)
    LGN_CHECK_ARG(d->enc_channels[l] >= 1 && d->enc_channels[l] <= 8 && d->dec_channels[l] >= 1 && d->dec_channels[l] <= 8,
                  "step: channel counts must be in 1..8");
  LGN_CHECK_ARG(d->get_real >= LGN_REAL_SUM && d->get_real <= LGN_REAL_NORM, "step: get_real=%d is not an LGN_REAL_* code", d->get_real);
  LGN_CHECK_ARG(d->jet_loss_scale >= 0.0, "step: jet_loss_scale=%g must be >= 0", d->jet_loss_scale);
  LGN_CHECK_ARG(d->dec_N >= 0, "step: dec_N=%d must be >= 0", d->dec_N);
  if (d->dec_N > 0) {
    const size_t need = decoder_end_lds_bytes(d->dec_N, d->dec_channels[0], dec_tin(*d), d->dec_channels[d->n_levels]);
    LGN_CHECK_ARG(need <= LGN_LDS_LIMIT, "step: dec_N=%d: the decoder end stages need %zu B of LDS (> %d)", d->dec_N, need, LGN_LDS_LIMIT);
  }
  return 0;
}

int plan_assign_loss(const lgn_net_desc* d, const lgn_loss_desc* loss, int* assignment, int* status, AssignLoss& al, const AssignLoss** out) {
  *out = nullptr;
  if (!loss || loss->kind == LGN_LOSS_CHAMFER) return 0;
  if (int rc = check_desc(d)) return rc;
  al = AssignLoss{loss->kind, loss->abs_coord, loss->polar_coord, loss->scale, assignment, status};
  const int Nd = dec_nodes(*d), CL = d->dec_channels[d->n_levels];
  if (int rc = check_assign_loss(al, Nd)) return rc;
  LGN_CHECK_ARG(d->jet_loss_scale == 0.0, "step: jet_loss_scale=%g with loss kind %d: the jet-feature term is a Chamfer option "
                "(--chamfer-jet-features)", d->jet_loss_scale, loss->kind);
  const size_t need = assign_loss_lds_bytes(Nd, CL);
  LGN_CHECK_ARG(need <= LGN_LDS_LIMIT, "step: the assignment-loss stage at N=%d needs %zu B of LDS (> %d)", Nd, need, LGN_LDS_LIMIT);
  *out = &al;
  return 0;
}

}

}


namespace lgn {
namespace {
struct ZeroJob { double* p[3]; size_t n[3]; };
__global__ __launch_bounds__(BLOCK) void zero_ranges_kernel(ZeroJob job) {
  const size_t stride = (size_t)gridDim.x * BLOCK;
#pragma unroll
  for (int q = 0; q < 3; ++q)
    for (size_t i = (size_t)blockIdx.x * BLOCK + threadIdx.x; i < job.n[q]; i += stride) job.p[q][i] = 0.0;
}
int zero_ranges(double* a, size_t na, double* b, size_t nb, double* c, size_t nc, hipStream_t st) {
  const ZeroJob job{{a, b, c}, {a ? na : 0, b ? nb : 0, c ? nc : 0}};
  const size_t most = std::max(job.n[0], std::max(job.n[1], job.n[2]));
  if (!most) return 0;
  const int blocks = (int)std::min<size_t>((most + BLOCK - 1) / BLOCK, 1024);
  hipLaunchKernelGGL(zero_ranges_kernel, dim3(blocks), dim3(BLOCK), 0, st, job);
  LGN_CHECK_LAUNCH();
  return 0;
}
int zero_grads_and_block(double* grads, size_t n, double* zeros, size_t nz, hipStream_t st) {
  if (zeros >= grads + n && zeros <= grads + n + 16) return zero_ranges(grads, (size_t)((zeros + nz) - grads), nullptr, 0, nullptr, 0, st);
  return zero_ranges(grads, n, zeros, nz, nullptr, 0, st);
}

int check_mlp_contiguous(const lgn_net_desc& d, bool dec, const int64_t* off) {
  const Slots S{d.n_levels, d.mlp_nlin};
  const int* ch = dec ? d.dec_channels : d.enc_channels;
  for (int l = 0; l < d.n_levels; ++l) {
    const int D = 2 * ch[l + 1], H = d.mlp_hidden_mul * D;
    int64_t expect = off[S.mlp(dec, l, 0)];
    for (int q = 0; q < d.mlp_nlin; ++q) {
      const int hin = q == 0 ? D : H, hout = q == d.mlp_nlin - 1 ? D : H;
      LGN_CHECK_ARG(off[S.mlp(dec, l, 2 * q)] == expect, "MLP weights are not contiguous in the flat parameter buffer");
      expect += (int64_t)hin * hout;
      LGN_CHECK_ARG(off[S.mlp(dec, l, 2 * q + 1)] == expect, "MLP biases are not contiguous in the flat parameter buffer");
      expect += hout;
    }
  }
  return 0;
}

}
}

namespace lgn {
namespace {

inline bool is_generic(const lgn_net_desc& d, bool dec) { return (dec ? d.dec_tables[0] : d.enc_tables[0]) != nullptr; }

struct GenGeom {
  const int *ch, *Q, *qs, *qv;
  const lgn_local_tables* const* tab;
};
inline GenGeom geom(const lgn_net_desc& d, bool dec) {
  return dec ? GenGeom{d.dec_channels, d.dec_Q, d.dec_qs, d.dec_qv, d.dec_tables}
             : GenGeom{d.enc_channels, d.enc_Q, d.enc_qs, d.enc_qv, d.enc_tables};
}

inline bool is_static(const lgn_net_desc& d, bool dec) {
  const GenGeom g = geom(d, dec);
  if (d.N > 32) return false;
  for (int l = 0; l < d.n_levels; ++l)
    if (!g.tab[l] || g.tab[l]->static_kind == 0) return false;
  return !(d.flags & LGN_NET_NO_STATIC);
}
inline bool is_sep_fused(const lgn_net_desc& d, bool dec) {
  return dec && is_static(d, dec) && !(d.flags & (LGN_NET_DEC_PAIRWISE | LGN_NET_DEC_UNFUSED));
}
inline size_t tb_doubles(const lgn_net_desc& d, int C, int Qx) { return (size_t)(((size_t)d.B * d.N + 63) / 64) * C * Qx * 128; }

int check_generic(const lgn_net_desc& d, bool dec) {
  const GenGeom g = geom(d, dec);
  for (int l = 0; l < d.n_levels; ++l) {
    LGN_CHECK_ARG(g.tab[l], "table-driven network: level %d has no tables (every level needs one)", l);
    LGN_CHECK_ARG(g.tab[l]->n_w > 0 && g.tab[l]->n_rows > 0, "table-driven network: empty tables at level %d", l);
  }
  for (int l = 0; l <= d.n_levels; ++l)
    LGN_CHECK_ARG(g.Q[l] >= 5 && g.Q[l] <= 64 && g.qs[l] >= 0 && g.qs[l] < g.Q[l] && g.qv[l] >= 0 && g.qv[l] + 4 <= g.Q[l],
                  "table-driven network: bad component layout at level %d (Q=%d qs=%d qv=%d)", l, g.Q[l], g.qs[l], g.qv[l]);
  LGN_CHECK_ARG(g.Q[0] == 5, "table-driven network: the input level carries (1,1) and (0,0) only (Q=5), got %d", g.Q[0]);
  return 0;
}

struct GenAct {
  double *s0, *v0;
  double *X[5], *U[4], *smix[4];
  double* wp[4];
  double* tbl[4];
  double* pc;
  double *sL, *vL;
  double* pdec;
  int* idx;
  size_t total;
};
GenAct carve_gen_act(const lgn_net_desc& d, bool dec, double* base) {
  GenAct a{};
  Bump b{base};
  const GenGeom g = geom(d, dec);
  const size_t BN = (size_t)d.B * d.N;
  const int L = d.n_levels;
  a.s0 = b.take(2 * BN * g.ch[0]);
  a.v0 = b.take(8 * BN * g.ch[0]);
  const bool tb = is_static(d, dec);
  const bool sep = is_sep_fused(d, dec);
  for (int l = 0; l <= L; ++l) a.X[l] = b.take(tb ? tb_doubles(d, g.ch[l], g.Q[l]) : 2 * BN * g.ch[l] * g.Q[l]);
  a.pc = sep ? b.take(8 * BN) : nullptr;
  for (int l = 0; l < L; ++l) {
    a.U[l] = sep ? nullptr : b.take(tb ? tb_doubles(d, g.ch[l], 5 * g.Q[l]) : 10 * BN * g.ch[l] * g.Q[l]);
    a.tbl[l] = sep ? b.take((size_t)d.B * g.ch[l] * g.Q[l] * SEP_TBL_STRIDE) : nullptr;
    a.smix[l] = b.take(2 * BN * g.ch[l + 1]);
    a.wp[l] = tb ? b.take(local_static_packed_doubles(g.tab[l]->static_kind, g.ch[l], g.ch[l + 1])) : nullptr;
  }
  a.sL = b.take(2 * BN * g.ch[L]);
  a.vL = b.take(8 * BN * g.ch[L]);
  if (dec) a.pdec = b.take(8 * BN);
  else a.idx = reinterpret_cast<int*>(b.take(((size_t)d.B * 2 * (d.tau_s + d.tau_v) * 2 + 1) / 2 + 8));
  a.total = b.off;
  return a;
}

struct GenScratch {
  double *zero0, *g_p, *g_lat_s;
  size_t zero_doubles;
  double *gs, *gv;
  double *gX[2], *gU;
  double* gbuf;
  double* gpk[4];
  double* gpb[4];
  double* tot[4];
  double* parts;
  size_t parts_size, total;
};
size_t gen_net_parts(const lgn_net_desc& d, bool dec) {
  const GenGeom g = geom(d, dec);
  const size_t BN = (size_t)d.B * d.N, tiles = (BN + 63) / 64;
  const bool tb = is_static(d, dec), sep = is_sep_fused(d, dec);
  size_t sum = 0;
  for (int l = 0; l < d.n_levels; ++l) {
    const int H = d.mlp_hidden_mul * 2 * g.ch[l + 1];
    const size_t lrows = tb ? (sep ? (size_t)local_sep_part_rows(d.B) : tiles) * local_static_packed_doubles(g.tab[l]->static_kind, g.ch[l], g.ch[l + 1])
                            : (size_t)local_partial_rows((int)BN) * 2 * g.tab[l]->n_w;
    sum += r16(lrows) + r16((size_t)d.B * rad_partial_size(g.ch[l], dec)) +
           r16((size_t)mlp_partial_rows((int)BN, H) * mlp_psize(g.ch[l + 1], H, d.mlp_nlin));
  }
  return sum + end_parts(d, dec, d.N, d.B);
}

GenScratch carve_gen_scratch(const lgn_net_desc& d, bool dec, double* base) {
  GenScratch s{};
  Bump b{base};
  const GenGeom g = geom(d, dec);
  const size_t BN = (size_t)d.B * d.N;
  const int L = d.n_levels;
  size_t cq = 0, cmax = 0;
  for (int l = 0; l <= L; ++l) {
    cq = cq > (size_t)g.ch[l] * g.Q[l] ? cq : (size_t)g.ch[l] * g.Q[l];
    cmax = cmax > (size_t)g.ch[l] ? cmax : (size_t)g.ch[l];
  }
  {
    const size_t z0 = b.off;
    s.zero0 = b.take(2 * BN * cmax);
    s.g_p = b.take(dec ? 8 * BN : 0);
    s.g_lat_s = b.take(dec ? 0 : (size_t)2 * d.B * pool_blocks(d.latent_pool) * d.tau_s);
    s.zero_doubles = b.off - z0;
  }
  s.gs = b.take(2 * BN * cmax);
  s.gv = b.take(8 * BN * cmax);
  const bool tb = is_static(d, dec), sep = is_sep_fused(d, dec);
  const size_t tiles = (BN + 63) / 64;
  s.gX[0] = b.take(tb ? tiles * cq * 128 : 2 * BN * cq);
  s.gX[1] = b.take(tb ? tiles * cq * 128 : 2 * BN * cq);
  s.gU = sep ? nullptr : b.take(tb ? tiles * cq * 640 : 10 * BN * cq);
  for (int l = 0; l < L; ++l) {
    s.gpk[l] = tb ? b.take(local_static_packed_doubles(g.tab[l]->static_kind, g.ch[l], g.ch[l + 1])) : nullptr;
    s.gpb[l] = sep ? b.take((size_t)g.ch[l] * BN * 8) : nullptr;
  }
  s.gbuf = (!dec && d.N <= 32) ? b.take(moments2_gbuf_doubles(d.B, d.N, (int)cmax)) : nullptr;
  for (int l = 0; l < L; ++l) s.tot[l] = b.take(rad_partial_size(g.ch[l], dec) + 16);
  const size_t psum = gen_net_parts(d, dec);
  s.parts = b.take(psum);
  s.parts_size = psum;
  s.total = b.off;
  return s;
}

GenArgs gen_level_args(const lgn_net_desc& d, bool dec, int l, const double* P, const int64_t* off, const double* X, const double* pos,
                       const uint8_t* mask) {
  const Slots S{d.n_levels, d.mlp_nlin};
  const GenGeom g = geom(d, dec);
  GenArgs a{};
  a.B = d.B; a.N = d.N; a.C = g.ch[l]; a.Q = g.Q[l]; a.X = X; a.p = pos; a.mask = mask;
  a.flags = d.flags;
  a.ra = P + off[S.rad(dec, l, 0)]; a.rb = P + off[S.rad(dec, l, 1)]; a.rc = P + off[S.rad(dec, l, 2)];
  a.w0 = P + off[S.rad(dec, l, 3)]; a.b0 = P + off[S.rad(dec, l, 4)]; a.w1 = P + off[S.rad(dec, l, 5)]; a.b1 = P + off[S.rad(dec, l, 6)];
  return a;
}

int gen_levels_fwd(const lgn_net_desc& d, bool dec, const double* P, const int64_t* off, GenAct& a, const double* pos,
                   const uint8_t* mask, hipStream_t st) {
  const Slots S{d.n_levels, d.mlp_nlin};
  const GenGeom g = geom(d, dec);
  const int BN = d.B * d.N;
  const bool tb = is_static(d, dec);
  if (tb) {
    StaticPackJob jobs[8];
    for (int l = 0; l < d.n_levels; ++l) {
      jobs[l] = StaticPackJob{g.tab[l]->static_kind, g.ch[l], g.ch[l + 1], {0, 0, 0, 0, 0}, P + off[S.mix(dec, l, 0)], a.wp[l]};
      for (int k = 0; k < 5; ++k) jobs[l].w0[k] = g.tab[l]->h_out_w0[k];
    }
    LGN_TRY(local_static_pack_batch(jobs, d.n_levels, false, st));
  }
  const bool sep = is_sep_fused(d, dec);
  for (int l = 0; l < d.n_levels; ++l) {
    GenArgs m = gen_level_args(d, dec, l, P, off, a.X[l], pos, mask);
    m.U = a.U[l];
    m.tb = tb;
    if (sep) {
      LGN_TRY(dec_sep_tab(m, a.tbl[l], a.pc, st));
      LGN_TRY(local_fwd_sep(g.tab[l]->static_kind, d.B, d.N, g.ch[l], g.ch[l + 1], a.X[l], a.tbl[l], a.pc, a.wp[l], a.X[l + 1], a.smix[l],
                            g.qs[l + 1], st));
    } else if (tb) {
      LGN_TRY(moments_dispatch(m, dec, 0, st));
      int w0[8];
      for (int k = 0; k < 5; ++k) w0[k] = g.tab[l]->h_out_w0[k];
      LGN_TRY(local_fwd_static(g.tab[l]->static_kind, BN, g.ch[l], g.ch[l + 1], a.X[l], a.U[l], P + off[S.mix(dec, l, 0)], w0, a.wp[l],
                               a.X[l + 1], a.smix[l], g.qs[l + 1], st, true));
    } else {
      LGN_TRY(moments_dispatch(m, dec, 0, st));
      LocalArgs la{};
      LGN_TRY(local_args(la, BN, g.ch[l], g.ch[l + 1], g.Q[l], g.Q[l + 1], g.tab[l]));
      la.X = a.X[l]; la.U = a.U[l]; la.wcat = P + off[S.mix(dec, l, 0)]; la.out = a.X[l + 1];
      la.s_copy = a.smix[l]; la.q_s = g.qs[l + 1];
      LGN_TRY(local_fwd(la, st));
    }
    MlpArgs<double> mm = level_mlp_args(d, dec, l, P, off);
    mm.s_in = a.smix[l];
    if (tb) { mm.s_out = a.X[l + 1] + (size_t)g.qs[l + 1] * 128; mm.tbQ = g.Q[l + 1]; }
    else { mm.s_out = a.X[l + 1] + g.qs[l + 1]; mm.ld = g.Q[l + 1]; }
    LGN_TRY(mlp_dispatch<double>(mm, false, st));
  }
  return 0;
}

typedef StaticPackJob UnpackJob;
int run_unpack_jobs(const std::vector<UnpackJob>& post, hipStream_t st) {
  if (post.empty()) return 0;
// ... 900 lines not shown
```

### lgn-autoencoder_amd/lgn/_native.py

```python
from __future__ import annotations

import ctypes as C
import os
from typing import Optional, Sequence

import torch

_HERE = os.path.dirname(os.path.abspath(__file__))
LIB_PATH = os.environ.get("LGN_AMD_LIB") or os.path.join(_HERE, "_lib", "liblgn_amd.so")
ABI_VERSION = 19
FINALIZE_SCRATCH = 2048
FINALIZE_OPT_SCRATCH = 4096

_lib: Optional[C.CDLL] = None

_vp, _i, _ip = C.c_void_p, C.c_int, C.POINTER(C.c_int)

_SIGNATURES = {
    "lgn_level_fwd_f64": [_i] * 5 + [_vp] * 18,
    "lgn_level_bwd_partial_rows": [_i, _i, _i, _ip, _ip],
    "lgn_level_rad_partial_len": [_i, _i],
    "lgn_level_jet_split": [_i, _i],
    "lgn_cg_product_fwd_f64": [_i] * 8 + [_vp] * 7,
    "lgn_cg_product_bwd_f64": [_i] * 8 + [_vp] * 9,
    "lgn_level_bwd_f64": [_i] * 5 + [_vp] * 24,
    "lgn_reduce_partials_f64": [_vp, _i, _i, _vp, _i, _vp],
    "lgn_radial_finalize_f64": [_vp, _i] + [_vp] * 13,
    "lgn_cgmlp_fwd_f64": [_i] * 5 + [_vp] * 5,
    "lgn_cgmlp_partial_rows": [_i, _i],
    "lgn_cgmlp_bwd_f64": [_i] * 5 + [_vp] * 6 + [_i, _vp],
    "lgn_mixreps_fwd_f64": [_i] * 4 + [_vp] * 4,
    "lgn_chamfer_f64": [_i] * 3 + [_vp] * 2 + [_i] + [_vp] * 4,
    "lgn_mixreps_partial_rows": [_i],
    "lgn_mixreps_bwd_f64": [_i] * 4 + [_vp] * 6,
}


class LocalTables(C.Structure):
    _fields_ = [("n_rows", C.c_int), ("n_out", C.c_int), ("n_w", C.c_int), ("n_terms", C.c_int), ("n_u", C.c_int),
                ("n_x", C.c_int), ("n_units", C.c_int), ("static_kind", C.c_int)] + [
        (name, C.c_void_p) for name in ("row_ptr", "t_type", "t_a", "t_b", "t_coef", "out_dim", "out_nblk", "out_row0", "out_q0",
                                        "out_w0", "u_ptr", "u_row", "u_coef", "x_ptr", "x_row", "x_other", "x_coef")] + [("h_out_w0", C.c_int * 8)]


_tp = C.POINTER(LocalTables)


_POOL_OPS = {"min": 0, "max": 1, "mean": 2, "average": 2}


def pool_code(map_to_latent: str):
    m = map_to_latent.lower()
    if m == "mix":
        return 1 | (3 << 4)
    if "&" in m and "+" in m:
        return None
    avg = "+" in m
    ops = m.split("+") if avg else m.split("&")
    if not 1 <= len(ops) <= 4 or any(o not in _POOL_OPS for o in ops):
        return None
    code = len(ops) | (int(avg) << 3)
    for i, o in enumerate(ops):
        code |= _POOL_OPS[o] << (4 + 2 * i)
    return code


def end_stages_fit(encoder=None, decoder=None, junction: bool = False) -> bool:
    L = lib()
    need = 0
    if encoder is not None:
        code = pool_code(encoder.map_to_latent)
        if code is None:
            return False
        n = encoder.num_input_particles
        ch = encoder.num_channels
        ts, tv = encoder.tau_latent[(0, 0)], encoder.tau_latent[(1, 1)]
        need = max(need, L.lgn_encoder_end_lds_bytes(n, ch[0], max(1, encoder.tau_input_scalars), ch[-1], ts, tv, code))
        if junction and decoder is not None:
            need = max(need, L.lgn_junction_lds_bytes(n, ch[-1], ts, tv, code, decoder.num_channels[0]))
    if decoder is not None:
        ch = decoder.num_channels
        need = max(need, L.lgn_decoder_end_lds_bytes(decoder.num_output_particles, ch[0], decoder.tau_latent_vectors, ch[-1]))
    return 0 <= need <= LDS_LIMIT


def pool_blocks(code: int) -> int:
    if code == 0:
        return 2
    return 1 if (code >> 3) & 1 else code & 7


class NetDesc(C.Structure):
    _fields_ = [("B", C.c_int), ("N", C.c_int), ("n_levels", C.c_int), ("enc_channels", C.c_int * 5),
                ("dec_channels", C.c_int * 5), ("tau_s", C.c_int), ("tau_v", C.c_int), ("mlp_hidden_mul", C.c_int),
                ("mlp_nlin", C.c_int), ("tau_v_in", C.c_int),
                ("enc_tables", _tp * 4), ("dec_tables", _tp * 4),
                ("enc_Q", C.c_int * 5), ("enc_qs", C.c_int * 5), ("enc_qv", C.c_int * 5),
                ("dec_Q", C.c_int * 5), ("dec_qs", C.c_int * 5), ("dec_qv", C.c_int * 5), ("flags", C.c_int),
                ("activation", C.c_int), ("n_in_scalars", C.c_int), ("latent_pool", C.c_int), ("dec_N", C.c_int),
                ("get_real", C.c_int), ("jet_loss_scale", C.c_double)]

    def __init__(self, *a, **kw):
        super().__init__(*a, **kw)
        self.flags = net_flags()


NET_NO_STATIC = 1
_NET_FLAG_ENV = {"LGN_AMD_NO_STATIC": 1, "LGN_AMD_DEC_PAIRWISE": 2, "LGN_AMD_LEVEL_V2": 4, "LGN_AMD_MLP_V1": 8,
                 "LGN_AMD_MOMENTS_V1": 16, "LGN_AMD_BWD_ORDERED": 64, "LGN_AMD_SPLIT_TAIL": 128, "LGN_AMD_DEC_UNFUSED": 256, "LGN_AMD_MOMENTS_SPLIT": 512,
                 "LGN_AMD_MLP_BWD1": 1024, "LGN_AMD_MLP_FULLTILE": 2048}
ACTIVATIONS = {"leakyrelu": 0, "relu": 1, "elu": 2, "sigmoid": 3, "logsigmoid": 4, "atan": 5}


def activation_id(name: str) -> int:
    try:
        return ACTIVATIONS[name.lower()]
    except KeyError:
        raise ValueError(f"Activation function {name} not implemented!") from None


def net_flags() -> int:
    return sum(bit for name, bit in _NET_FLAG_ENV.items() if os.environ.get(name, "") == "1")


class LossDesc(C.Structure):
    _fields_ = [("kind", C.c_int), ("abs_coord", C.c_int), ("polar_coord", C.c_int), ("scale", C.c_double)]


class OptimDesc(C.Structure):
    _fields_ = [("kind", C.c_int), ("l1_lambda", C.c_double), ("l2_lambda", C.c_double), ("lr", C.c_double), ("eps", C.c_double),
                ("beta1", C.c_double), ("beta2", C.c_double), ("alpha", C.c_double), ("momentum", C.c_double)]


OPT_ADAM, OPT_RMSPROP = 0, 1
LOSS_CHAMFER, LOSS_MSE, LOSS_HUNGARIAN = 0, 1, 2
ASSIGN_NMAX = 192
_dp = C.POINTER(NetDesc)
_lp = C.POINTER(LossDesc)
_op = C.POINTER(OptimDesc)
_ll = C.c_longlong
_d = C.c_double
_SIGNATURES.update({
    "lgn_moments_fwd_f64": [_i] * 5 + [_vp] * 12,
    "lgn_moments_bwd_f64": [_i] * 5 + [_vp] * 16,
    "lgn_local_fwd_f64": [_i] * 5 + [_tp] + [_vp] * 5,
    "lgn_local_partial_rows": [_i],
    "lgn_local_fwd_static_f64": [_i] * 4 + [_vp] * 3 + [_ip] + [_vp] * 3 + [_i, _vp],
    "lgn_local_bwd_static_f64": [_i] * 4 + [_vp] * 3 + [_ip] + [_vp] * 8,
    "lgn_local_bwd_f64": [_i] * 5 + [_tp] + [_vp] * 8,
    "lgn_step_param_slots": [_dp, _i],
    "lgn_step_fwd_bwd_f64": [_dp, _vp, _vp, _ll, _vp, _vp, _vp, _vp, _vp, _vp, _vp, _ll, _vp, _vp, _lp, _vp, _vp, _vp],
    "lgn_encoder_fwd_f64": [_dp, _vp, _vp, _vp, _vp, _vp, _vp, _ll, _vp, _vp, _vp],
    "lgn_encoder_bwd_f64": [_dp, _vp, _vp, _ll, _vp, _vp, _vp, _vp, _vp, _ll, _vp, _vp, _vp, _ll, _vp],
    "lgn_decoder_fwd_f64": [_dp, _vp, _vp, _vp, _vp, _ll, _vp, _vp],
    "lgn_decoder_bwd_f64": [_dp, _vp, _vp, _ll, _vp, _vp, _vp, _ll, _vp, _vp, _vp, _ll, _vp],
    "lgn_step_finalize_f64": [_vp, _vp, _ll, _vp, _i, _d, _vp, _vp, _vp, _d, _d, _d, _d, _i, _vp, _vp],
    "lgn_step_train_f64": [_dp, _vp, _vp, _ll, _vp, _vp, _vp, _vp, _vp, _vp, _vp, _ll, _vp, _vp, _i, _d, _vp, _vp, _vp, _d, _d, _d, _d, _i,
                           _vp, _lp, _vp, _vp, _vp],
    "lgn_step_finalize_opt_f64": [_vp, _vp, _ll, _vp, _i, _op, _vp, _vp, _vp, _i, _vp, _vp],
    "lgn_step_train_opt_f64": [_dp, _vp, _vp, _ll, _vp, _vp, _vp, _vp, _vp, _vp, _vp, _ll, _vp, _vp, _i, _op, _vp, _vp, _vp, _i, _vp, _lp,
                               _vp, _vp, _vp],
    "lgn_step_eval_f64": [_dp, _vp, _vp, _vp, _vp, _vp, _vp, _vp, _vp, _ll, _vp, _vp, _vp, _vp, _vp, _lp, _vp, _vp, _vp],
    "lgn_anomaly_scores_f64": [_vp] * 4 + [_i] * 3 + [_vp] * 4,
    "lgn_linear_sum_assignment_f64": [_vp, _i, _i, _vp, _vp, _vp],
    "lgn_hungarian_mse_f64": [_i, _i, _vp, _vp, _i, _i, _i, _d] + [_vp] * 5,
    "lgn_recon_analysis_f64": [_vp, _vp] + [_i] * 4 + [_vp] * 11,
    "lgn_match_rel_err_f64": [_vp] * 6 + [_i, _i] + [_vp] * 5,
    "lgn_histogram_f64": [_vp, _ll, _i, _i, _vp, _ip, _i, _vp, _vp, _vp, _vp, _i, _vp],
    "lgn_stage_batch_f64": [_vp] * 3 + [_i] * 4 + [_d, _i, _i] + [_vp] * 6,
    "lgn_denormalize_f64": [_vp] * 3 + [_i, _i] + [_vp] * 3,
    "lgn_stage_gather_f64": [_vp] * 3 + [_ll, _vp, _ll, _vp] + [_i] * 3 + [_d, _i, _i] + [_vp] * 7,
    "lgn_epoch_collect_f64": [_vp] * 3 + [_ll, _i, _i, C.POINTER(_vp), C.POINTER(_vp), _ip, _vp],
    "lgn_epoch_reset": [_vp] * 4,
    "lgn_roc_auc_f64": [_vp, _ll, _i, _i] + [_vp] * 9 + [_ll, _vp],
    "lgn_emd_f64": [_vp, _vp, _i, _i, _i, _d] + [_vp] * 6 + [_ll, _vp],
    "lgn_emd_relative_f64": [_vp, _vp, _i, _i, _vp, _vp, _vp, _ll, _vp],
    "lgn_emd_debug_max_augmentations": [_ip, _i],
    "lgn_column_stats_f64": [_vp, _ll, _i, _i, _vp, _i, _d, _i] + [_vp] * 5 + [_ll, _vp],
    "lgn_hist_fwhm_f64": [_vp, _i, _vp, _i, _ip, _i, _vp, _vp],
    "lgn_jet_images_f64": [_vp, _vp, _i, _i, _i, _i, _d, _i, _vp, _vp, _vp, _ll, _vp],
    "lgn_transform_jets_f64": [_vp] * 4 + [_i] * 4 + [_vp] * 3,
    "lgn_rep_deviation_f64": [_i] * 3 + [C.POINTER(_vp)] * 3 + [_ip] * 3 + [_vp] * 3 + [_ll, _vp],
})
EPOCH_MAX_COLLECT, EPOCH_BAD_INDEX = 4, 1
NORM_NONE, NORM_COMPONENT_MAX, NORM_OVERALL_MAX, NORM_JET_E = 0, 1, 2, 3


_LL_SIGNATURES = {
    "lgn_step_workspace_doubles": [_dp],
    "lgn_eval_workspace_doubles": [_dp],
    "lgn_net_workspace_doubles": [_dp, _i, _i],
    "lgn_moments_scratch_doubles": [_i, _i, _i, _i],
    "lgn_local_static_packed_doubles": [_i, _i, _i],
    "lgn_encoder_end_lds_bytes": [_i] * 7,
    "lgn_decoder_end_lds_bytes": [_i] * 4,
    "lgn_junction_lds_bytes": [_i] * 6,
    "lgn_assign_loss_lds_bytes": [_i, _i],
    "lgn_roc_workspace_bytes": [_ll, _i],
    "lgn_emd_workspace_bytes": [_i, _i],
    "lgn_emd_lds_bytes": [_i],
    "lgn_column_stats_workspace_bytes": [_ll, _i],
    "lgn_jet_images_workspace_bytes": [_i, _i],
    "lgn_rep_deviation_workspace_bytes": [_i, _i, _i, _ip, _ip, _ip],
}
ROC_TILE, ROC_MAX_COLS = 2048, 65535
ROC_NONFINITE, ROC_SINGLE_CLASS, ROC_BAD_LABEL, ROC_NAN = 1, 2, 4, 8
EMD_NMAX = 191
EMD_INVALID, EMD_EMPTY, EMD_ITER, EMD_INFEASIBLE = 1, 2, 4, 8
HIST_MAX_EDGES, HIST_MAX_COLS = 1025, 16
STATS_TILE, STATS_MAX_COLS, STATS_EMPTY, STATS_NONFINITE = 2048, 16, 1, 2
STAT_NAMES = ("median", "IQR", "first_quartile", "third_quartile", "IDR", "MAD", "mean", "max", "min", "abs_min", "std_dev", "skew",
              "kurtosis", "FWHM", "abs_mean", "abs_mean_within_iqr", "abs_mean_within_idr", "q10", "q90")
STATS_COUNT = len(STAT_NAMES)
JET_IMAGE_MAX_NPIX, JET_IMAGE_PARTS = 64, 512
EQUI_TILE, EQUI_MAX_PARTS = 256, 64
LDS_LIMIT = 160 * 1024
EXPORTED_SYMBOLS = ["lgn_abi_version", "lgn_last_error"] + list(_LL_SIGNATURES) + list(_SIGNATURES)


def lib() -> C.CDLL:
    global _lib
    if _lib is None:
        if not os.path.exists(LIB_PATH):
            raise RuntimeError(
                f"liblgn_amd.so not found at {LIB_PATH}. Build it with `python -c 'import __graft_entry__ as g; "
                "g.build()'` or `make -C lgn-autoencoder_amd/csrc`. There is no CPU fallback.")
        l = C.CDLL(LIB_PATH)
        l.lgn_abi_version.restype = C.c_int
        l.lgn_last_error.restype = C.c_char_p
        got = l.lgn_abi_version()
        if got != ABI_VERSION:
            raise RuntimeError(f"liblgn_amd.so ABI version {got} != expected {ABI_VERSION}; rebuild the library")
        for name, argtypes in _SIGNATURES.items():
            fn = getattr(l, name)
            fn.argtypes = argtypes
            fn.restype = C.c_int
        for name, argtypes in _LL_SIGNATURES.items():
            fn = getattr(l, name)
            fn.argtypes = argtypes
            fn.restype = C.c_longlong
        _lib = l
    return _lib


def last_error() -> str:
    return lib().lgn_last_error().decode()


def _check(rc: int, what: str):
    if rc != 0:
        raise RuntimeError(f"{what} failed (code {rc}): {last_error()}")


def stream_ptr() -> int:
    return torch.cuda.current_stream().cuda_stream


def ptr(t: Optional[torch.Tensor]):
    if t is None:
        return None
    if not t.is_cuda:
        raise RuntimeError("liblgn_amd.so operates on GPU tensors only (got a CPU tensor); there is no CPU fallback")
    if not t.is_contiguous():
        raise RuntimeError("non-contiguous tensor passed to the native library")
    return t.data_ptr()


def f64(t: torch.Tensor) -> torch.Tensor:
    if t.dtype != torch.float64:
        raise RuntimeError(f"the native path is fp64 (reference precision); got {t.dtype}")
    return t.contiguous()



def level_fwd(decoder, s_in, v_in, p, mask, rad, wm0, wm1):
    _, B, N, Cc = s_in.shape
    CO = wm0.shape[1]
    dev, dt = s_in.device, s_in.dtype
    ag0 = torch.empty(2, B, N, 2 * Cc, device=dev, dtype=dt)
    ag1 = torch.empty(2, B, N, 2 * Cc, 4, device=dev, dtype=dt)
    s_out = torch.empty(2, B, N, CO, device=dev, dtype=dt)
    v_out = torch.empty(2, B, N, CO, 4, device=dev, dtype=dt)
    a, b, c, w0, b0, w1, b1 = rad
    rc = lib().lgn_level_fwd_f64(B, N, Cc, CO, int(decoder), ptr(s_in), ptr(v_in), ptr(p), ptr(mask),
                                 ptr(a), ptr(b), ptr(c), ptr(w0), ptr(b0), ptr(w1), ptr(b1), ptr(wm0), ptr(wm1),
                                 ptr(ag0), ptr(ag1), ptr(s_out), ptr(v_out), stream_ptr())
    _check(rc, "lgn_level_fwd_f64")
    return ag0, ag1, s_out, v_out


def reduce_partials(part: torch.Tensor, out: torch.Tensor, accumulate: bool = False):
    rows, n = part.shape
    _check(lib().lgn_reduce_partials_f64(ptr(part), rows, n, ptr(out), int(accumulate), stream_ptr()),
           "lgn_reduce_partials_f64")
    return out


def level_bwd(decoder, s_in, v_in, p, mask, rad, wm0, wm1, ag0, ag1, g_s_out, g_v_out, g_p=None):
    _, B, N, Cc = s_in.shape
    CO = wm0.shape[1]
    dev, dt = s_in.device, s_in.dtype
    L = lib()
    rm, rr = C.c_int(), C.c_int()
    _check(L.lgn_level_bwd_partial_rows(B, N, int(decoder), C.byref(rm), C.byref(rr)), "lgn_level_bwd_partial_rows")
    nmix = 4 * CO * 5 * Cc
    nrad = L.lgn_level_rad_partial_len(Cc, int(decoder))
    part_mix = torch.empty(rm.value, nmix, device=dev, dtype=dt)
    part_rad = torch.empty(rr.value, nrad, device=dev, dtype=dt)
    g_ag = torch.empty(B, N, 20 * Cc, device=dev, dtype=dt)
    g_s_in = torch.empty_like(s_in)
    g_v_in = torch.empty_like(v_in)
    a, b, c, w0, b0, w1, b1 = rad
    rc = L.lgn_level_bwd_f64(B, N, Cc, CO, int(decoder), ptr(s_in), ptr(v_in), ptr(p), ptr(mask),
                             ptr(a), ptr(b), ptr(c), ptr(w0), ptr(b0), ptr(w1), ptr(b1), ptr(wm0), ptr(wm1),
                             ptr(ag0), ptr(ag1), ptr(g_s_out), ptr(g_v_out), ptr(g_ag), ptr(g_s_in), ptr(g_v_in),
                             ptr(g_p), ptr(part_mix), ptr(part_rad), stream_ptr())
    _check(rc, "lgn_level_bwd_f64")
    g_mix = torch.empty(nmix, device=dev, dtype=dt)
    reduce_partials(part_mix, g_mix)
    g_wm0 = g_mix[: nmix // 2].view(2, CO, 5 * Cc)
    g_wm1 = g_mix[nmix // 2:].view(2, CO, 5 * Cc)
    tot = torch.empty(nrad, device=dev, dtype=dt)
    reduce_partials(part_rad, tot)
    if decoder:
        rad_grads = (tot[:Cc], tot[Cc:])
    else:
        g_a, g_b, g_c = (torch.empty_like(x) for x in (a, b, c))
        g_w0, g_b0, g_w1, g_b1 = (torch.empty_like(x) for x in (w0, b0, w1, b1))
        _check(L.lgn_radial_finalize_f64(ptr(tot), Cc, ptr(a), ptr(b), ptr(c), ptr(w0), ptr(w1), ptr(g_a), ptr(g_b),
                                         ptr(g_c), ptr(g_w0), ptr(g_b0), ptr(g_w1), ptr(g_b1), stream_ptr()),
               "lgn_radial_finalize_f64")
        rad_grads = (g_a, g_b, g_c, g_w0, g_b0, g_w1, g_b1)
    return g_s_in, g_v_in, g_wm0, g_wm1, rad_grads


def _ptr_array(ts: Sequence[torch.Tensor]):
    arr = (C.c_void_p * len(ts))()
    for i, t in enumerate(ts):
        arr[i] = ptr(t)
    return arr


def cgmlp_fwd(s_in, ws, bs, act: int = 0):
    _, B, N, Cc = s_in.shape
    H = ws[0].shape[0]
    s_out = torch.empty_like(s_in)
    rc = lib().lgn_cgmlp_fwd_f64(B * N, Cc, H, len(ws), act, _ptr_array(ws), _ptr_array(bs), ptr(s_in), ptr(s_out), stream_ptr())
    _check(rc, "lgn_cgmlp_fwd_f64")
    return s_out


def cgmlp_bwd(s_in, ws, bs, g_out, act: int = 0):
    _, B, N, Cc = s_in.shape
    H = ws[0].shape[0]
    L = lib()
    rows = L.lgn_cgmlp_partial_rows(B * N, H)
    psize = sum(w.numel() + b.numel() for w, b in zip(ws, bs))
    part = torch.empty(rows, psize, device=s_in.device, dtype=s_in.dtype)
    g_in = torch.empty_like(s_in)
    rc = L.lgn_cgmlp_bwd_f64(B * N, Cc, H, len(ws), act, _ptr_array(ws), _ptr_array(bs), ptr(s_in), ptr(g_out), ptr(g_in),
                             ptr(part), psize, stream_ptr())
    _check(rc, "lgn_cgmlp_bwd_f64")
    flat = torch.empty(psize, device=s_in.device, dtype=s_in.dtype)
    reduce_partials(part, flat)
    gws, gbs, off = [], [], 0
    for w, b in zip(ws, bs):
        gws.append(flat[off: off + w.numel()].view_as(w)); off += w.numel()
        gbs.append(flat[off: off + b.numel()].view_as(b)); off += b.numel()
    return g_in, gws, gbs


def chamfer(x, y, jet_features=False):
    x, y = f64(x), f64(y)
    B, Np, M = x.shape[0], x.shape[1], y.shape[1]
    out = torch.empty(B + 4 * B * (Np + M), device=x.device, dtype=x.dtype)
    part, gx, gy = out[:B], out[B:B + 4 * B * Np].view(B, Np, 4), out[B + 4 * B * Np:].view(B, M, 4)
    _check(lib().lgn_chamfer_f64(B, Np, M, ptr(x), ptr(y), int(bool(jet_features)), ptr(part), ptr(gx), ptr(gy), stream_ptr()),
           "lgn_chamfer_f64")
    return part, gx, gy


def hungarian_mse(x, y, kind=LOSS_HUNGARIAN, abs_coord=True, polar_coord=False, scale=None):
    x, y = f64(x), f64(y)
    B, Np = x.shape[0], x.shape[1]
    if scale is None:
        scale = 1.0 / (B * Np * (4 if kind == LOSS_MSE or (abs_coord and not polar_coord) else 3))
    out = torch.empty(B + 4 * B * Np, device=x.device, dtype=x.dtype)
    ints = torch.empty(B * Np + B, device=x.device, dtype=torch.int32)
    part, gx = out[:B], out[B:].view(B, Np, 4)
    assignment, status = ints[:B * Np].view(B, Np), ints[B * Np:]
    _check(lib().lgn_hungarian_mse_f64(B, Np, ptr(x), ptr(y), int(kind), int(bool(abs_coord)), int(bool(polar_coord)), float(scale),
                                       ptr(part), ptr(gx), ptr(assignment), ptr(status), stream_ptr()), "lgn_hungarian_mse_f64")
    return part, gx, assignment, status


def mixreps_fwd(w, x):
    Co, Ci = w.shape[1], w.shape[2]
    d = x.shape[-1]
    rows = x[0].numel() // (Ci * d)
    y = torch.empty(x.shape[:-2] + (Co, d), device=x.device, dtype=x.dtype)
    _check(lib().lgn_mixreps_fwd_f64(rows, Ci, Co, d, ptr(w), ptr(x), ptr(y), stream_ptr()), "lgn_mixreps_fwd_f64")
    return y


def mixreps_bwd(w, x, g_y, need_gx=True):
    Co, Ci = w.shape[1], w.shape[2]
    d = x.shape[-1]
    rows = x[0].numel() // (Ci * d)
    L = lib()
    part = torch.empty(L.lgn_mixreps_partial_rows(rows), 2 * Co * Ci, device=x.device, dtype=x.dtype)
    g_x = torch.empty_like(x) if need_gx else None
    _check(L.lgn_mixreps_bwd_f64(rows, Ci, Co, d, ptr(w), ptr(x), ptr(g_y), ptr(g_x), ptr(part), stream_ptr()),
# ... 85 lines not shown
```

Measured before the change: 1.090 million.

## Skip dead scalar-channel work in last level forward and backward kernels

Adds a NOS template specialization to the level forward and backward kernels. It is selected when the scalar output of a level is unused: the last level without an MLP in forward, or no incoming scalar gradient in backward. In that case the kernels skip scalar loads, the A3/A4 aggregates, ag0 stores, scalar weight-gradient reductions and the related gradient terms, and the mix-0 weight gradient is zero-filled. An env flag restores the old path. This saves FLOPs, LDS traffic and memory traffic, at the cost of extra template instantiations and the risk of missing a term that is actually live.

After: 1.112 million, median of 6. +2.1%, better.

```diff
diff --git a/include/lgn_amd.h b/include/lgn_amd.h
--- a/include/lgn_amd.h
+++ b/include/lgn_amd.h
@@ -150,6 +150,7 @@
 #define LGN_NET_MOMENTS_SPLIT 512
 #define LGN_NET_MLP_BWD1 1024
 #define LGN_NET_MLP_FULLTILE 2048
+#define LGN_NET_LIVE_SCALARS 4096
 #define LGN_NET_SPLIT_TAIL 128
 
 #define LGN_LDS_LIMIT (160 * 1024)
diff --git a/lgn-autoencoder_amd/csrc/api_common.cpp b/lgn-autoencoder_amd/csrc/api_common.cpp
--- a/lgn-autoencoder_amd/csrc/api_common.cpp
+++ b/lgn-autoencoder_amd/csrc/api_common.cpp
@@ -21,7 +21,8 @@
 }
 static_assert(LVL_DEC_PAIRWISE == LGN_NET_DEC_PAIRWISE && LVL_LEVEL_V2 == LGN_NET_LEVEL_V2 && LVL_MOMENTS_V1 == LGN_NET_MOMENTS_V1 &&
                   LVL_MLP_V1 == LGN_NET_MLP_V1 && LVL_MLP_BWD1 == LGN_NET_MLP_BWD1 && LVL_MLP_FULLTILE == LGN_NET_MLP_FULLTILE &&
-                  LVL_BWD_ORDERED == LGN_NET_BWD_ORDERED && LVL_MOMENTS_SPLIT == LGN_NET_MOMENTS_SPLIT, "LVL_* and LGN_NET_* are the same bits");
+                  LVL_BWD_ORDERED == LGN_NET_BWD_ORDERED && LVL_MOMENTS_SPLIT == LGN_NET_MOMENTS_SPLIT &&
+                  LVL_LIVE_SCALARS == LGN_NET_LIVE_SCALARS, "LVL_* and LGN_NET_* are the same bits");
 }
 
 extern "C" {
diff --git a/lgn-autoencoder_amd/csrc/level.hpp b/lgn-autoencoder_amd/csrc/level.hpp
--- a/lgn-autoencoder_amd/csrc/level.hpp
+++ b/lgn-autoencoder_amd/csrc/level.hpp
@@ -10,6 +10,7 @@
 constexpr int LVL_MLP_BWD1 = 1024;
 constexpr int LVL_MLP_FULLTILE = 2048;
 constexpr int LVL_MOMENTS_SPLIT = 512;
+constexpr int LVL_LIVE_SCALARS = 4096;
 constexpr int LVL_BWD_ORDERED = 64;
 int level_flags_from_env();
 
@@ -44,6 +45,7 @@
   T* loss_gv = nullptr;
   T* loss_wpart = nullptr;
   int flags = 0;
+  int dead_scalars = 0;
 };
 
 template <typename T>
@@ -64,6 +66,7 @@
   T* part_rad;
   T* part_in0 = nullptr;
   int flags = 0;
+  int dead_scalars = 0;
 };
 
 __host__ __device__ constexpr int node_stride(int C) { return 10 * C + 4; }
diff --git a/lgn-autoencoder_amd/csrc/level_bwd3.hip b/lgn-autoencoder_amd/csrc/level_bwd3.hip
--- a/lgn-autoencoder_amd/csrc/level_bwd3.hip
+++ b/lgn-autoencoder_amd/csrc/level_bwd3.hip
@@ -65,7 +65,7 @@
   }
 };
 
-template <int C, bool DEC, bool SEP, int NWV, bool SYM = false>
+template <int C, bool DEC, bool SEP, int NWV, bool SYM = false, bool NOS = false>
 __global__ __launch_bounds__(64 * NWV) __attribute__((amdgpu_waves_per_eu(C <= 4 || DEC ? 2 : 1, C <= 4 || DEC ? 2 : 1))) void level_bwd3_kernel(LevelBwdArgs<double> a) {
   static_assert(!SYM || !DEC, "the symmetric sweep is the encoder's");
   using F = Bwd3<C, DEC, NWV>;
@@ -99,10 +99,12 @@
     const int eg = tid < N * CO ? tid : 0, ea_ = tid < N * 2 * C ? tid : 0, ew = tid < 2 * CO * K ? tid : 0;
     const size_t ig = (size_t)b * N * CO + eg, ia = (size_t)b * N * 2 * C + ea_;
     double rg[10], ra[10];
-    rg[0] = a.g_s_out[ig];
-    rg[1] = a.g_s_out[plo + ig];
-    ra[0] = a.ag0[ia];
-    ra[1] = a.ag0[pa + ia];
+    if constexpr (!NOS) {
+      rg[0] = a.g_s_out[ig];
+      rg[1] = a.g_s_out[plo + ig];
+      ra[0] = a.ag0[ia];
+      ra[1] = a.ag0[pa + ia];
+    }
 #pragma unroll
     for (int m = 0; m < 4; ++m) {
       rg[2 + m] = a.g_v_out[ig * 4 + m];
@@ -114,11 +116,11 @@
     load_jet_commit<double, C, DEC>(a.s_in, a.v_in, a.p, a.mask, B, N, b, jr, nd, pj, mk);
     if (tid < N * CO) {
 #pragma unroll
-      for (int m = 0; m < 10; ++m) go[tid * 10 + m] = rg[m];
+      for (int m = NOS ? 2 : 0; m < 10; ++m) go[tid * 10 + m] = rg[m];
     }
     if (tid < N * 2 * C) {
 #pragma unroll
-      for (int m = 0; m < 10; ++m) agl[tid * 10 + m] = ra[m];
+      for (int m = NOS ? 2 : 0; m < 10; ++m) agl[tid * 10 + m] = ra[m];
     }
     if (tid < 2 * CO * K) {
       wm[tid] = w0v;
@@ -131,8 +133,10 @@
     for (int e = tid + BLK; e < N * CO; e += BLK) {
       const size_t idx = (size_t)b * N * CO + e;
       double* g = go + e * 10;
-      g[0] = a.g_s_out[idx];
-      g[1] = a.g_s_out[plo + idx];
+      if constexpr (!NOS) {
+        g[0] = a.g_s_out[idx];
+        g[1] = a.g_s_out[plo + idx];
+      }
 #pragma unroll
       for (int m = 0; m < 4; ++m) {
         g[2 + m] = a.g_v_out[idx * 4 + m];
@@ -142,8 +146,10 @@
     for (int e = tid + BLK; e < N * 2 * C; e += BLK) {
       const size_t ea = (size_t)b * N * 2 * C + e;
       double* x = agl + e * 10;
-      x[0] = a.ag0[ea];
-      x[1] = a.ag0[pa + ea];
+      if constexpr (!NOS) {
+        x[0] = a.ag0[ea];
+        x[1] = a.ag0[pa + ea];
+      }
 #pragma unroll
       for (int m = 0; m < 4; ++m) {
         x[2 + m] = a.ag1[ea * 4 + m];
@@ -164,22 +170,26 @@
         cx<double> gx0[2] = {{0, 0}, {0, 0}}, gx1[2][4] = {{{0, 0}, {0, 0}, {0, 0}, {0, 0}}, {{0, 0}, {0, 0}, {0, 0}, {0, 0}}};
         for (int o = 0; o < CO; ++o) {
           const double* g = go + (n * CO + o) * 10;
-          const cx<double> gs = {g[0], g[1]};
           cx<double> gv[4];
 #pragma unroll
           for (int m = 0; m < 4; ++m) gv[m] = {g[2 + m], g[6 + m]};
 #pragma unroll
           for (int q = 0; q < 2; ++q) {
-            const cx<double> w0 = {w0r[(0 * CO + o) * K + q * C], w0r[(1 * CO + o) * K + q * C]};
             const cx<double> w1 = {w1r[(0 * CO + o) * K + q * C], w1r[(1 * CO + o) * K + q * C]};
-            cfmac(gx0[q], gs, w0);
+            if constexpr (!NOS) {
+              const cx<double> gs = {g[0], g[1]};
+              const cx<double> w0 = {w0r[(0 * CO + o) * K + q * C], w0r[(1 * CO + o) * K + q * C]};
+              cfmac(gx0[q], gs, w0);
+            }
 #pragma unroll
             for (int m = 0; m < 4; ++m) cfmac(gx1[q][m], gv[m], w1);
           }
         }
         double* gan = ga + n * G::SIZE;
-        gan[G::A3 + 2 * c] = gx0[0].r;  gan[G::A3 + 2 * c + 1] = gx0[0].i;
-        gan[G::A4 + 2 * c] = gx0[1].r;  gan[G::A4 + 2 * c + 1] = gx0[1].i;
+        if constexpr (!NOS) {
+          gan[G::A3 + 2 * c] = gx0[0].r;  gan[G::A3 + 2 * c + 1] = gx0[0].i;
+          gan[G::A4 + 2 * c] = gx0[1].r;  gan[G::A4 + 2 * c + 1] = gx0[1].i;
+        }
 #pragma unroll
         for (int m = 0; m < 4; ++m) {
           gan[G::A1 + (c * 4 + m) * 2] = gx1[0][m].r;  gan[G::A1 + (c * 4 + m) * 2 + 1] = gx1[0][m].i;
@@ -190,14 +200,16 @@
         cx<double> b2[4] = {{0, 0}, {0, 0}, {0, 0}, {0, 0}}, b34[4] = {{0, 0}, {0, 0}, {0, 0}, {0, 0}};
         for (int o = 0; o < CO; ++o) {
           const double* g = go + (n * CO + o) * 10;
-          const cx<double> gs = {g[0], g[1]};
-          const double* wr0 = w0r + (0 * CO + o) * K;
-          const double* wi0 = w0r + (1 * CO + o) * K;
           const double* wr1 = w1r + (0 * CO + o) * K;
           const double* wi1 = w1r + (1 * CO + o) * K;
-          cfmac(a2, gs, cx<double>{wr0[2 * C], wi0[2 * C]});
-          cfmac(a3, gs, cx<double>{wr0[3 * C], wi0[3 * C]});
-          cfmac(a4, gs, cx<double>{wr0[4 * C], wi0[4 * C]});
+          if constexpr (!NOS) {
+            const cx<double> gs = {g[0], g[1]};
+            const double* wr0 = w0r + (0 * CO + o) * K;
+            const double* wi0 = w0r + (1 * CO + o) * K;
+            cfmac(a2, gs, cx<double>{wr0[2 * C], wi0[2 * C]});
+            cfmac(a3, gs, cx<double>{wr0[3 * C], wi0[3 * C]});
+            cfmac(a4, gs, cx<double>{wr0[4 * C], wi0[4 * C]});
+          }
           const cx<double> w2 = {wr1[2 * C], wi1[2 * C]};
           const cx<double> w34 = {wr1[3 * C] + wr1[4 * C], wi1[3 * C] + wi1[4 * C]};
 #pragma unroll
@@ -214,14 +226,14 @@
         for (int m = 0; m < 4; ++m) v[m] = {ni[2 + m], ni[6 + m]};
         metric_perm(v, vt);
         cx<double> gs = a2;
-        cfmac(gs, cx<double>{2.0 * a4.r, 2.0 * a4.i}, s);
+        if constexpr (!NOS) cfmac(gs, cx<double>{2.0 * a4.r, 2.0 * a4.i}, s);
         double* gdn = gd + (n * C + c) * 10;
 #pragma unroll
         for (int m = 0; m < 4; ++m) {
           cfmac(gs, b34[m], v[m]);
           cx<double> gv = b2[m];
           cfmac(gv, b34[m], s);
-          cfmac(gv, a3, vt[m]);
+          if constexpr (!NOS) cfmac(gv, a3, vt[m]);
           gdn[2 + m] = gv.r;
           gdn[6 + m] = gv.i;
         }
@@ -246,7 +258,7 @@
         cx<double> x0, x1[4];
         if (q < 2) {
           const double* x = agl + (n * 2 * C + k) * 10;
-          x0 = {x[0], x[1]};
+          if constexpr (!NOS) x0 = {x[0], x[1]};
 #pragma unroll
           for (int m = 0; m < 4; ++m) x1[m] = {x[2 + m], x[6 + m]};
         } else {
@@ -256,11 +268,13 @@
 #pragma unroll
           for (int m = 0; m < 4; ++m) v[m] = {ni[2 + m], ni[6 + m]};
           if (q == 2) {
-            x0 = s;
+            if constexpr (!NOS) x0 = s;
 #pragma unroll
             for (int m = 0; m < 4; ++m) x1[m] = v[m];
           } else {
-            if (q == 3) { x0 = bil2(v, v); x0.r *= 0.5; x0.i *= 0.5; } else x0 = cmul(s, s);
+            if constexpr (!NOS) {
+              if (q == 3) { x0 = bil2(v, v); x0.r *= 0.5; x0.i *= 0.5; } else x0 = cmul(s, s);
+            }
 #pragma unroll
             for (int m = 0; m < 4; ++m) x1[m] = cmul(v[m], s);
           }
@@ -269,7 +283,7 @@
         for (int o = 0; o < 8; ++o)
           if (o < CO) {
             const double* g = go + (n * CO + o) * 10;
-            cfmac(d0[o], cx<double>{g[0], g[1]}, x0);
+            if constexpr (!NOS) cfmac(d0[o], cx<double>{g[0], g[1]}, x0);
 #pragma unroll
             for (int m = 0; m < 4; ++m) cfmac(d1[o], cx<double>{g[2 + m], g[6 + m]}, x1[m]);
           }
@@ -284,7 +298,8 @@
       for (int o = 0; o < 8; ++o)
         if (o < CO) {
           double* r4 = red + ((pi * CO + o) * K + k) * 4;
-          r4[0] = d0[o].r;  r4[1] = d0[o].i;  r4[2] = d1[o].r;  r4[3] = d1[o].i;
+          if constexpr (!NOS) { r4[0] = d0[o].r;  r4[1] = d0[o].i; }
+          r4[2] = d1[o].r;  r4[3] = d1[o].i;
         }
     }
     STAMP(50);
@@ -292,6 +307,7 @@
     STAMP(51);
     for (int ex = tid; ex < 4 * OK; ex += BLK) {
       const int e = ex >> 2, x = ex & 3;
+      if (NOS && x < 2) continue;
       double v = red[ex];
 #pragma unroll
       for (int pp = 1; pp < NPART; ++pp) v += red[pp * OK * 4 + ex];
@@ -350,9 +366,12 @@
         }
         const cx<double> vp = bil2(v, pc);
         LGN_PUT(18, vp.r);  LGN_PUT(19, vp.i);
-        const cx<double> g3 = {0.5 * gi[G::A3 + 2 * c], 0.5 * gi[G::A3 + 2 * c + 1]};
-        LGN_PUT(20, gi[G::A4 + 2 * c]);  LGN_PUT(21, gi[G::A4 + 2 * c + 1]);
-        LGN_PUT(22, g3.r);  LGN_PUT(23, g3.i);
+        cx<double> g3 = {0, 0};
+        if constexpr (!NOS) {
+          g3 = {0.5 * gi[G::A3 + 2 * c], 0.5 * gi[G::A3 + 2 * c + 1]};
+          LGN_PUT(20, gi[G::A4 + 2 * c]);  LGN_PUT(21, gi[G::A4 + 2 * c + 1]);
+          LGN_PUT(22, g3.r);  LGN_PUT(23, g3.i);
+        }
         cx<double> gp2 = {0, 0};
 #pragma unroll
         for (int m = 0; m < 4; ++m) {
@@ -361,8 +380,10 @@
           LGN_PUT(24 + 2 * m, g1.r);  LGN_PUT(25 + 2 * m, g1.i);
           LGN_PUT(32 + 2 * m, g2.r);  LGN_PUT(33 + 2 * m, g2.i);
           cfmac(gp2, g2, pc[m]);
-          const cx<double> gp3 = cmulc(g3, pc[m]);
-          LGN_PUT(42 + 2 * m, gp3.r);  LGN_PUT(43 + 2 * m, gp3.i);
+          if constexpr (!NOS) {
+            const cx<double> gp3 = cmulc(g3, pc[m]);
+            LGN_PUT(42 + 2 * m, gp3.r);  LGN_PUT(43 + 2 * m, gp3.i);
+          }
         }
         LGN_PUT(40, gp2.r);  LGN_PUT(41, gp2.i);
       }
@@ -399,18 +420,21 @@
         const cx<double> t = cmulc(cx<double>{q[32 + 2 * m], q[33 + 2 * m]}, pc[m]);
         u.r -= t.r;  u.i -= t.i;
       }
-      cx<double> gs = cmulc(SG4, e0);
+      cx<double> gs = {0, 0};
+      if constexpr (!NOS) gs = cmulc(SG4, e0);
       cfmac(gs, u, R1);
       const size_t ge = ((size_t)b * N + n) * C + c;
       a.g_s_in[ge] = gdn[0] + gs.r;
       a.g_s_in[pls + ge] = gdn[1] + gs.i;
 #pragma unroll
       for (int m = 0; m < 4; ++m) {
-        cx<double> w = GPT3[m];
-        const cx<double> t = cmulc(SG3, pt[m]);
-        w.r -= t.r;  w.i -= t.i;
         cx<double> gv = cmulc(cx<double>{q[24 + 2 * m], q[25 + 2 * m]}, e0);
-        cfmac(gv, w, R1);
+        if constexpr (!NOS) {
+          cx<double> w = GPT3[m];
+          const cx<double> t = cmulc(SG3, pt[m]);
+          w.r -= t.r;  w.i -= t.i;
+          cfmac(gv, w, R1);
+        }
         a.g_v_in[ge * 4 + m] = gdn[2 + m] + gv.r;
         a.g_v_in[pls * 4 + ge * 4 + m] = gdn[6 + m] + gv.i;
       }
@@ -432,13 +456,17 @@
           const cx<double> VSt = {sg * q[2 + 2 * mp], sg * q[3 + 2 * mp]};
           const cx<double> vt = {sg * ni[2 + mp], sg * ni[6 + mp]};
           const cx<double> g2 = {gi[G::A2 + (c * 4 + m) * 2], gi[G::A2 + (c * 4 + m) * 2 + 1]};
-          const cx<double> g3 = {0.5 * gi[G::A3 + 2 * c], 0.5 * gi[G::A3 + 2 * c + 1]};
           cx<double> t = cmulc(g2, S);
-          cfmac(t, g3, VSt);
+          if constexpr (!NOS) {
+            const cx<double> g3 = {0.5 * gi[G::A3 + 2 * c], 0.5 * gi[G::A3 + 2 * c + 1]};
+            cfmac(t, g3, VSt);
+          }
           const cx<double> t2 = cmulc(cx<double>{q[32 + 2 * m], q[33 + 2 * m]}, cx<double>{ni[0], ni[1]});
           t.r -= t2.r;  t.i -= t2.i;
-          const cx<double> t3 = cmulc(SG3, vt);
-          t.r -= t3.r;  t.i -= t3.i;
+          if constexpr (!NOS) {
+            const cx<double> t3 = cmulc(SG3, vt);
+            t.r -= t3.r;  t.i -= t3.i;
+          }
           cfmac(acc, t, R1);
         }
         a.g_p[((size_t)b * N + n) * 4 + m] += acc.r;
@@ -451,7 +479,8 @@
       const cx<double> S = {q[0], q[1]};
       double* part = a.part_rad + (size_t)blockIdx.x * rad_partial_size(C, true);
       if (lin == 0) {
-        cx<double> E0 = cmulc(cx<double>{q[20], q[21]}, S);
+        cx<double> E0 = {0, 0};
+        if constexpr (!NOS) E0 = cmulc(cx<double>{q[20], q[21]}, S);
 #pragma unroll
         for (int m = 0; m < 4; ++m) cfmac(E0, cx<double>{q[24 + 2 * m], q[25 + 2 * m]}, cx<double>{q[2 + 2 * m], q[3 + 2 * m]});
         part[tid] = (E0.r + E0.i) + (E0.i - E0.r);
@@ -461,11 +490,12 @@
         for (int m = 0; m < 4; ++m) VS[m] = {q[2 + 2 * m], q[3 + 2 * m]};
         metric_perm(VS, VSt);
         cx<double> E1 = cmulc(cx<double>{q[40], q[41]}, S);
-        cx<double> neg = cmulc(cx<double>{q[22], q[23]}, cx<double>{q[18], q[19]});
+        cx<double> neg = {0, 0};
+        if constexpr (!NOS) neg = cmulc(cx<double>{q[22], q[23]}, cx<double>{q[18], q[19]});
 #pragma unroll
         for (int m = 0; m < 4; ++m) {
           cfmac(neg, cx<double>{q[32 + 2 * m], q[33 + 2 * m]}, cx<double>{q[10 + 2 * m], q[11 + 2 * m]});
-          cfmac(E1, cx<double>{q[42 + 2 * m], q[43 + 2 * m]}, VSt[m]);
+          if constexpr (!NOS) cfmac(E1, cx<double>{q[42 + 2 * m], q[43 + 2 * m]}, VSt[m]);
         }
         part[tid] = (E1.r - neg.r) + (E1.i - neg.i);
       }
@@ -637,16 +667,22 @@
         if (ok && ch < C) {
           const cx<double> R0 = {R[g][0], R[g][1]}, R1 = {R[g][2], R[g][3]};
           const cx<double> e0 = {R0.r - R0.i, R0.r + R0.i};
-          const cx<double> gA3 = {0.5 * gi[G::A3 + 2 * ch], 0.5 * gi[G::A3 + 2 * ch + 1]};
-          const cx<double> gA4 = {gi[G::A4 + 2 * ch], gi[G::A4 + 2 * ch + 1]};
+          cx<double> gA3 = {0, 0}, gA4 = {0, 0};
+          if constexpr (!NOS) {
+            gA3 = {0.5 * gi[G::A3 + 2 * ch], 0.5 * gi[G::A3 + 2 * ch + 1]};
+            gA4 = {gi[G::A4 + 2 * ch], gi[G::A4 + 2 * ch + 1]};
+          }
           cx<double> gA1[4], gA2[4];
 #pragma unroll
           for (int m = 0; m < 4; ++m) {
             gA1[m] = {gi[G::A1 + (ch * 4 + m) * 2], gi[G::A1 + (ch * 4 + m) * 2 + 1]};
             gA2[m] = {gi[G::A2 + (ch * 4 + m) * 2], gi[G::A2 + (ch * 4 + m) * 2 + 1]};
           }
-          cfmac(Gs[g], gA4, e0);
-          cx<double> ge0 = cmulc(gA4, sj[g]);
+          cx<double> ge0 = {0, 0};
+          if constexpr (!NOS) {
+            cfmac(Gs[g], gA4, e0);
+            ge0 = cmulc(gA4, sj[g]);
+          }
           cx<double> gR1;
           if (!DEC) {
             const cx<double> dg = {gA2[1].r - gA2[3].r, gA2[1].i - gA2[3].i}, sg = {gA2[1].r + gA2[3].r, gA2[1].i + gA2[3].i};
@@ -654,24 +690,28 @@
             P2.r = __builtin_fma(gA2[0].r, qd0, __builtin_fma(gA2[2].r, qd3, __builtin_fma(qa, dg.r, -qb * sg.i)));
             P2.i = __builtin_fma(gA2[0].i, qd0, __builtin_fma(gA2[2].i, qd3, __builtin_fma(qa, dg.i, qb * sg.r)));
             cfmac(Gs[g], P2, R1);
-            const cx<double> Z = cmulc(gA3, R1);
 #pragma unroll
             for (int m = 0; m < 4; ++m) cfmac(Gv[g][m], gA1[m], e0);
-            Gv[g][0].r = __builtin_fma(Z.r, qd0, Gv[g][0].r);   Gv[g][0].i = __builtin_fma(Z.i, qd0, Gv[g][0].i);
-            Gv[g][2].r = __builtin_fma(-Z.r, qd3, Gv[g][2].r);  Gv[g][2].i = __builtin_fma(-Z.i, qd3, Gv[g][2].i);
-            const double aZr = qa * Z.r, aZi = qa * Z.i;
-            const double bZr = qb * Z.r, bZi = qb * Z.i;
-            Gv[g][1].r -= aZr + bZi;  Gv[g][1].i += bZr - aZi;
-            Gv[g][3].r += aZr - bZi;  Gv[g][3].i += aZi + bZr;
+            if constexpr (!NOS) {
+              const cx<double> Z = cmulc(gA3, R1);
+              Gv[g][0].r = __builtin_fma(Z.r, qd0, Gv[g][0].r);   Gv[g][0].i = __builtin_fma(Z.i, qd0, Gv[g][0].i);
+              Gv[g][2].r = __builtin_fma(-Z.r, qd3, Gv[g][2].r);  Gv[g][2].i = __builtin_fma(-Z.i, qd3, Gv[g][2].i);
+              const double aZr = qa * Z.r, aZi = qa * Z.i;
+              const double bZr = qb * Z.r, bZi = qb * Z.i;
+              Gv[g][1].r -= aZr + bZi;  Gv[g][1].i += bZr - aZi;
+              Gv[g][3].r += aZr - bZi;  Gv[g][3].i += aZi + bZr;
+            }
             gR1 = {0, 0};
             if (kind != 0) {
 #pragma unroll
               for (int m = 0; m < 4; ++m) cfmac(ge0, gA1[m], vj[g][m]);
-              cx<double> V;
-              V.r = __builtin_fma(vj[g][0].r, qd0, __builtin_fma(-vj[g][2].r, qd3, __builtin_fma(qa, dvj[g].r, qb * svj[g].i)));
-              V.i = __builtin_fma(vj[g][0].i, qd0, __builtin_fma(-vj[g][2].i, qd3, __builtin_fma(qa, dvj[g].i, -qb * svj[g].r)));
               gR1 = cmulc(P2, sj[g]);
-              cfmac(gR1, gA3, V);
+              if constexpr (!NOS) {
+                cx<double> V;
+                V.r = __builtin_fma(vj[g][0].r, qd0, __builtin_fma(-vj[g][2].r, qd3, __builtin_fma(qa, dvj[g].r, qb * svj[g].i)));
+                V.i = __builtin_fma(vj[g][0].i, qd0, __builtin_fma(-vj[g][2].i, qd3, __builtin_fma(qa, dvj[g].i, -qb * svj[g].r)));
+                cfmac(gR1, gA3, V);
+              }
             }
             if constexpr (SYM) {
               if (kind == 2) {
@@ -681,9 +721,11 @@
                 cx<double> vi[4];
 #pragma unroll
                 for (int m = 0; m < 4; ++m) vi[m] = {ni[2 + m], ni[6 + m]};
-                const cx<double> hA3 = {0.5 * gj[G::A3 + 2 * ch], 0.5 * gj[G::A3 + 2 * ch + 1]};
-                const cx<double> hA4 = {gj[G::A4 + 2 * ch], gj[G::A4 + 2 * ch + 1]};
-                cx<double> he0 = cmulc(hA4, si);
+                cx<double> he0 = {0, 0};
+                if constexpr (!NOS) {
+                  const cx<double> hA4 = {gj[G::A4 + 2 * ch], gj[G::A4 + 2 * ch + 1]};
+                  he0 = cmulc(hA4, si);
+                }
                 cx<double> hA2[4];
 #pragma unroll
                 for (int m = 0; m < 4; ++m) {
@@ -695,12 +737,15 @@
                 cx<double> Q2;
                 Q2.r = __builtin_fma(hA2[0].r, qd0, __builtin_fma(hA2[2].r, qd3, __builtin_fma(qa, hd.r, -qb * hs.i)));
                 Q2.i = __builtin_fma(hA2[0].i, qd0, __builtin_fma(hA2[2].i, qd3, __builtin_fma(qa, hd.i, qb * hs.r)));
-                const cx<double> dvi = {vi[3].r - vi[1].r, vi[3].i - vi[1].i}, svi = {vi[1].r + vi[3].r, vi[1].i + vi[3].i};
-                cx<double> W;
-                W.r = __builtin_fma(vi[0].r, qd0, __builtin_fma(-vi[2].r, qd3, __builtin_fma(qa, dvi.r, qb * svi.i)));
-                W.i = __builtin_fma(vi[0].i, qd0, __builtin_fma(-vi[2].i, qd3, __builtin_fma(qa, dvi.i, -qb * svi.r)));
                 cx<double> hR1 = cmulc(Q2, si);
-                cfmac(hR1, hA3, W);
+                if constexpr (!NOS) {
+                  const cx<double> hA3 = {0.5 * gj[G::A3 + 2 * ch], 0.5 * gj[G::A3 + 2 * ch + 1]};
+                  const cx<double> dvi = {vi[3].r - vi[1].r, vi[3].i - vi[1].i}, svi = {vi[1].r + vi[3].r, vi[1].i + vi[3].i};
+                  cx<double> W;
+                  W.r = __builtin_fma(vi[0].r, qd0, __builtin_fma(-vi[2].r, qd3, __builtin_fma(qa, dvi.r, qb * svi.i)));
+                  W.i = __builtin_fma(vi[0].i, qd0, __builtin_fma(-vi[2].i, qd3, __builtin_fma(qa, dvi.i, -qb * svi.r)));
+                  cfmac(hR1, hA3, W);
+                }
                 ge0.r += he0.r;  ge0.i += he0.i;
                 gR1.r -= hR1.r;  gR1.i -= hR1.i;
               }
@@ -714,11 +759,11 @@
 #pragma unroll
             for (int m = 0; m < 4; ++m) {
               cfmac(Gv[g][m], gA1[m], e0);
-              cfmac(Gv[g][m], gA3, e1t[m]);
+              if constexpr (!NOS) cfmac(Gv[g][m], gA3, e1t[m]);
               cfmac(Gs[g], gA2[m], e1[m]);
               cfmac(ge0, gA1[m], vj[g][m]);
               cx<double> ge1 = cmulc(gA2[m], sj[g]);
-              cfmac(ge1, gA3, vtj[g][m]);
+              if constexpr (!NOS) cfmac(ge1, gA3, vtj[g][m]);
               cfmac(gR1, ge1, q[m]);
               cfmac(Gq[m], ge1, R1);
             }
@@ -789,10 +834,11 @@
       const int ch = 4 * g + cg;
       const double sr = rs > 1 ? Gs[g].r : quad_sum(Gs[g].r), si = rs > 1 ? Gs[g].i : quad_sum(Gs[g].i);
       const bool wr = jok && ti == 0 && ch < C;
+      const bool st = wr && (DEC || !a.part_in0);
       const size_t e = ((size_t)b * N + jj) * C + (ch < C ? ch : 0);
       const double* gdn = gd + (jj * C + (ch < C ? ch : 0)) * 10;
       const double gsr = gdn[0] + sr, gsi = gdn[1] + si;
-      if (wr) {
+      if (st) {
         a.g_s_in[e] = gsr;
         a.g_s_in[pls + e] = gsi;
       }
@@ -801,7 +847,7 @@
       for (int m = 0; m < 4; ++m) {
         const double vr = rs > 1 ? Gv[g][m].r : quad_sum(Gv[g][m].r), vi = rs > 1 ? Gv[g][m].i : quad_sum(Gv[g][m].i);
         gvn[m] = {gdn[2 + m] + vr, gdn[6 + m] + vi};
-        if (wr) {
+        if (st) {
           a.g_v_in[e * 4 + m] = gvn[m].r;
           a.g_v_in[pls * 4 + e * 4 + m] = gvn[m].i;
         }
@@ -861,12 +907,13 @@
               for (int m = 0; m < 4; ++m) v[m] = {nj[2 + m], nj[6 + m]};
               metric_perm(v, vt);
               const cx<double> R1 = {bias[g][2], bias[g][3]};
-              const cx<double> gA3 = {0.5 * gi[G::A3 + 2 * ch], 0.5 * gi[G::A3 + 2 * ch + 1]};
+              cx<double> gA3 = {0, 0};
+              if constexpr (!NOS) gA3 = {0.5 * gi[G::A3 + 2 * ch], 0.5 * gi[G::A3 + 2 * ch + 1]};
 #pragma unroll
               for (int m = 0; m < 4; ++m) {
                 const cx<double> gA2 = {gi[G::A2 + (ch * 4 + m) * 2], gi[G::A2 + (ch * 4 + m) * 2 + 1]};
                 cx<double> ge1 = cmulc(gA2, s);
-                cfmac(ge1, gA3, vt[m]);
+                if constexpr (!NOS) cfmac(ge1, gA3, vt[m]);
                 cfmac(Gq[m], ge1, R1);
               }
             }
@@ -981,14 +1028,14 @@
 
 bool level_bwd3_fits(int N) { return N <= 40; }
 
-template <int C, bool DEC, bool SEP, int NWV>
+template <int C, bool DEC, bool SEP, int NWV, bool NOS>
 static int launch_bwd3_w(const LevelBwdArgs<double>& a, int split, hipStream_t stream) {
   size_t smem = Bwd3<C, DEC, NWV>::smem(a.N, a.CO);
   LGN_CHECK_ARG(smem <= 160 * 1024, "level_bwd: N=%d C=%d needs %zu B of LDS", a.N, a.C, smem);
   LGN_CHECK_ARG(a.CO <= 8, "level_bwd: C_out=%d unsupported (1..8)", a.CO);
-  auto kern = level_bwd3_kernel<C, DEC, SEP, NWV>;
+  auto kern = level_bwd3_kernel<C, DEC, SEP, NWV, false, NOS>;
   if constexpr (!DEC && C <= 4) {
-    if (split == 1 && !(a.flags & LVL_BWD_ORDERED)) kern = level_bwd3_kernel<C, DEC, SEP, NWV, true>;
+    if (split == 1 && !(a.flags & LVL_BWD_ORDERED)) kern = level_bwd3_kernel<C, DEC, SEP, NWV, true, NOS>;
   }
   if (smem > 64 * 1024) (void)hipFuncSetAttribute(reinterpret_cast<const void*>(kern), hipFuncAttributeMaxDynamicSharedMemorySize, (int)smem);
   hipLaunchKernelGGL(kern, dim3(a.B, split), dim3(64 * NWV), smem, stream, a);
@@ -997,7 +1044,8 @@
 }
 template <int C, bool DEC, bool SEP>
 static int launch_bwd3(const LevelBwdArgs<double>& a, hipStream_t stream) {
-  return launch_bwd3_w<C, DEC, SEP, 4>(a, SEP ? 1 : level_jet_split(a.B, a.N), stream);
+  const int split = SEP ? 1 : level_jet_split(a.B, a.N);
+  return a.dead_scalars ? launch_bwd3_w<C, DEC, SEP, 4, true>(a, split, stream) : launch_bwd3_w<C, DEC, SEP, 4, false>(a, split, stream);
 }
 
 int level_bwd3_dispatch(const LevelBwdArgs<double>& a, int decoder, hipStream_t stream) {
diff --git a/lgn-autoencoder_amd/csrc/level_fwd2.hip b/lgn-autoencoder_amd/csrc/level_fwd2.hip
--- a/lgn-autoencoder_amd/csrc/level_fwd2.hip
+++ b/lgn-autoencoder_amd/csrc/level_fwd2.hip
@@ -43,7 +43,7 @@
   static constexpr int A3 = 0, A4 = 2 * C, A1 = 4 * C, A2 = 12 * C;
 };
 
-template <int C, bool DEC, bool SEP, bool TRAIN>
+template <int C, bool DEC, bool SEP, bool TRAIN, bool NOS>
 __global__ __launch_bounds__(2 * BLOCK) void level_fwd2_kernel(LevelArgs<double> a, int chunk) {
   using F = Fwd2<C, DEC>;
   constexpr int NG = F::NG;
@@ -196,8 +196,10 @@
           const cx<double> sp = cmul(sn, pc[m]);
           LGN_PUT(10 + 2 * m, sp.r);  LGN_PUT(11 + 2 * m, sp.i);
         }
-        const cx<double> vp = bil2(v, pc);
-        LGN_PUT(18, vp.r);  LGN_PUT(19, vp.i);
+        if constexpr (!NOS) {
+          const cx<double> vp = bil2(v, pc);
+          LGN_PUT(18, vp.r);  LGN_PUT(19, vp.i);
+        }
       }
       wave_sum_store<12>(a0, sums + c * 20, lane);
       wave_sum_store<8>(a1, sums + c * 20 + 12, lane);
@@ -212,7 +214,8 @@
     constexpr int K = 5 * C;
     const int nr = c1 - c0;
     const size_t plo = (size_t)B * N * CO;
-    if (wave == 0) {
+    const int vfirst = NOS ? tid : lane + 64 * (wave - 1), vstep = NOS ? nthr : 64 * (nw - 1);
+    if (!NOS && wave == 0) {
       for (int rl = lane; rl < nr; rl += 64) {
         const int r = c0 + rl;
         const double* st = agl + rl * F::AGS;
@@ -245,7 +248,7 @@
         }
       }
     } else {
-      for (int it = lane + 64 * (wave - 1); it < nr * 4; it += 64 * (nw - 1)) {
+      for (int it = vfirst; it < nr * 4; it += vstep) {
         const int rl = it >> 2, m = it & 3, r = c0 + rl;
         const double* st = agl + rl * F::AGS;
         const double* ni = nd + r * F::NS;
@@ -290,12 +293,14 @@
         pc[m] = {pn[m], pn[4 + m]};
       }
       double* st = agl + rl * F::AGS;
-      const cx<double> a4 = cmul(S, e0);
-      cx<double> t = bil2(VS, pc);
-      t.r -= sm[18];  t.i -= sm[19];
-      cx<double> a3 = cmul(R1, t);
-      st[F::A3 + 2 * c] = 0.5 * a3.r;  st[F::A3 + 2 * c + 1] = 0.5 * a3.i;
-      st[F::A4 + 2 * c] = a4.r;        st[F::A4 + 2 * c + 1] = a4.i;
+      if constexpr (!NOS) {
+        const cx<double> a4 = cmul(S, e0);
+        cx<double> t = bil2(VS, pc);
+        t.r -= sm[18];  t.i -= sm[19];
+        cx<double> a3 = cmul(R1, t);
+        st[F::A3 + 2 * c] = 0.5 * a3.r;  st[F::A3 + 2 * c + 1] = 0.5 * a3.i;
+        st[F::A4 + 2 * c] = a4.r;        st[F::A4 + 2 * c + 1] = a4.i;
+      }
 #pragma unroll
       for (int m = 0; m < 4; ++m) {
         const cx<double> a1 = cmul(VS[m], e0);
@@ -388,7 +393,7 @@
               vj[m] = {nj[ch * 10 + 2 + m], nj[ch * 10 + 6 + m]};
               cfma(A1[g][m], vj[m], e0);
             }
-            cfma(A4[g], sj, e0);
+            if constexpr (!NOS) cfma(A4[g], sj, e0);
             if (!DEC) {
               const double qd0 = T.qd0, qd3 = T.qd3, qa = T.qa, qb = T.qb;
               const cx<double> Tm = cmul(sj, R1);
@@ -397,11 +402,13 @@
               const double aTr = qa * Tm.r, aTi = qa * Tm.i, bTr = qb * Tm.r, bTi = qb * Tm.i;
               A2[g][1].r += aTr + bTi;  A2[g][1].i += aTi - bTr;
               A2[g][3].r += bTi - aTr;  A2[g][3].i -= aTi + bTr;
-              const cx<double> dv = {vj[3].r - vj[1].r, vj[3].i - vj[1].i}, sv = {vj[1].r + vj[3].r, vj[1].i + vj[3].i};
-              cx<double> V;
-              V.r = __builtin_fma(vj[0].r, qd0, __builtin_fma(-vj[2].r, qd3, __builtin_fma(qa, dv.r, qb * sv.i)));
-              V.i = __builtin_fma(vj[0].i, qd0, __builtin_fma(-vj[2].i, qd3, __builtin_fma(qa, dv.i, -qb * sv.r)));
-              cfma(A3[g], R1, V);
+              if constexpr (!NOS) {
+                const cx<double> dv = {vj[3].r - vj[1].r, vj[3].i - vj[1].i}, sv = {vj[1].r + vj[3].r, vj[1].i + vj[3].i};
+                cx<double> V;
+                V.r = __builtin_fma(vj[0].r, qd0, __builtin_fma(-vj[2].r, qd3, __builtin_fma(qa, dv.r, qb * sv.i)));
+                V.i = __builtin_fma(vj[0].i, qd0, __builtin_fma(-vj[2].i, qd3, __builtin_fma(qa, dv.i, -qb * sv.r)));
+                cfma(A3[g], R1, V);
+              }
             } else {
               cx<double> e1[4];
 #pragma unroll
@@ -409,9 +416,11 @@
                 e1[m] = cmul(R1, T.q[m]);
                 cfma(A2[g][m], sj, e1[m]);
               }
-              const cx<double> t = bil2(vj, e1);
-              A3[g].r += t.r;
-              A3[g].i += t.i;
+              if constexpr (!NOS) {
+                const cx<double> t = bil2(vj, e1);
+                A3[g].r += t.r;
+                A3[g].i += t.i;
+              }
             }
           }
         }
@@ -436,8 +445,10 @@
     STAMP(3 + ((rg >> 2) & 3) * 4);
 #pragma unroll
     for (int g = 0; g < NG; ++g) {
-      A3[g].r = quad_sum(A3[g].r) * 0.5;  A3[g].i = quad_sum(A3[g].i) * 0.5;
-      A4[g].r = quad_sum(A4[g].r);        A4[g].i = quad_sum(A4[g].i);
+      if constexpr (!NOS) {
+        A3[g].r = quad_sum(A3[g].r) * 0.5;  A3[g].i = quad_sum(A3[g].i) * 0.5;
+        A4[g].r = quad_sum(A4[g].r);        A4[g].i = quad_sum(A4[g].i);
+      }
 #pragma unroll
       for (int m = 0; m < 4; ++m) {
         A1[g][m].r = quad_sum(A1[g][m].r);  A1[g][m].i = quad_sum(A1[g][m].i);
@@ -450,8 +461,10 @@
       for (int g = 0; g < NG; ++g) {
         const int ch = 4 * g + cg;
         if (ch < C) {
-          st[F::A3 + 2 * ch] = A3[g].r;  st[F::A3 + 2 * ch + 1] = A3[g].i;
-          st[F::A4 + 2 * ch] = A4[g].r;  st[F::A4 + 2 * ch + 1] = A4[g].i;
+          if constexpr (!NOS) {
+            st[F::A3 + 2 * ch] = A3[g].r;  st[F::A3 + 2 * ch + 1] = A3[g].i;
+            st[F::A4 + 2 * ch] = A4[g].r;  st[F::A4 + 2 * ch + 1] = A4[g].i;
+          }
 #pragma unroll
           for (int m = 0; m < 4; ++m) {
             st[F::A1 + (ch * 4 + m) * 2] = A1[g][m].r;  st[F::A1 + (ch * 4 + m) * 2 + 1] = A1[g][m].i;
@@ -472,6 +485,7 @@
     __syncthreads();
     const int tot = 4 * ngr * F::AGS;
     for (int e = tid; e < tot; e += nthr) {
+      if (NOS && e % F::AGS < F::A1) continue;
       double v = agl[e];
       for (int pp = 1; pp < rs; ++pp) v += agl[pp * tot + e];
       agl[e] = v;
@@ -483,12 +497,14 @@
 
   if constexpr (TRAIN) {
     const size_t pl0 = (size_t)B * N * 2 * C;
-    for (int e = tid; e < (c1 - c0) * 2 * C; e += nthr) {
-      const int n = e / (2 * C), r = e - n * 2 * C, blk = r / C, ch = r - blk * C;
-      const double* st = agl + n * F::AGS + (blk ? F::A4 : F::A3) + 2 * ch;
-      const size_t ge = ((size_t)b * N + c0) * 2 * C + e;
-      a.ag0[ge] = st[0];
-      a.ag0[pl0 + ge] = st[1];
+    if constexpr (!NOS) {
+      for (int e = tid; e < (c1 - c0) * 2 * C; e += nthr) {
+        const int n = e / (2 * C), r = e - n * 2 * C, blk = r / C, ch = r - blk * C;
+        const double* st = agl + n * F::AGS + (blk ? F::A4 : F::A3) + 2 * ch;
+        const size_t ge = ((size_t)b * N + c0) * 2 * C + e;
+        a.ag0[ge] = st[0];
+        a.ag0[pl0 + ge] = st[1];
+      }
     }
     for (int e = tid; e < (c1 - c0) * 2 * C * 4; e += nthr) {
       const int n = e / (8 * C), r = e - n * 8 * C, blk = r / (4 * C), cm = r - blk * 4 * C;
@@ -514,7 +530,7 @@
   }
 }
 
-template <int C, bool DEC, bool SEP, bool TRAIN>
+template <int C, bool DEC, bool SEP, bool TRAIN, bool NOS>
 static int launch_level_fwd2(const LevelArgs<double>& a, hipStream_t stream) {
   using F = Fwd2<C, DEC>;
   const size_t fixed = sizeof(double) * (((size_t)a.N * F::NS + 1 & ~size_t(1)) + (size_t)a.N * F::PS + 4 * a.CO * 5 * C + 20 * C) + a.N + 16;
@@ -535,7 +551,7 @@
     if (smem < dec_out_loss_bytes(a.N, a.CO)) smem = dec_out_loss_bytes(a.N, a.CO);
   }
   LGN_CHECK_ARG(smem <= 160 * 1024, "level_fwd: N=%d C=%d needs %zu B of LDS (> 160 KiB)", a.N, a.C, smem);
-  auto kern = level_fwd2_kernel<C, DEC, SEP, TRAIN>;
+  auto kern = level_fwd2_kernel<C, DEC, SEP, TRAIN, NOS>;
   if (smem > 64 * 1024) {
     hipError_t e = hipFuncSetAttribute(reinterpret_cast<const void*>(kern), hipFuncAttributeMaxDynamicSharedMemorySize, (int)smem);
     if (e != hipSuccess) { set_error("hipFuncSetAttribute: %s", hipGetErrorString(e)); return (int)e; }
@@ -549,7 +565,7 @@
 
 bool level_fwd_carries_loss(int N, int flags) { return N <= 40 && !(flags & LVL_DEC_PAIRWISE); }
 
-template <bool TRAIN>
+template <bool TRAIN, bool NOS>
 static int level_fwd_run(const LevelArgs<double>& a, int decoder, hipStream_t stream) {
   LGN_CHECK_ARG(a.B > 0 && a.N > 0, "level_fwd: empty batch (B=%d N=%d)", a.B, a.N);
   LGN_CHECK_ARG(!a.in_w0 || (!decoder && a.in_w1 && a.in_s && a.in_v), "level_fwd: the input stage rides on encoder levels only");
@@ -557,8 +573,8 @@
   const bool pairwise = (a.flags & LVL_DEC_PAIRWISE) != 0;
 #define LGN_CASE(CC)                                                                                         \
   case CC:                                                                                                   \
-    if (!decoder) return launch_level_fwd2<CC, false, false, TRAIN>(a, stream);                              \
-    return pairwise ? launch_level_fwd2<CC, true, false, TRAIN>(a, stream) : launch_level_fwd2<CC, true, true, TRAIN>(a, stream);
+    if (!decoder) return launch_level_fwd2<CC, false, false, TRAIN, NOS>(a, stream);                         \
+    return pairwise ? launch_level_fwd2<CC, true, false, TRAIN, NOS>(a, stream) : launch_level_fwd2<CC, true, true, TRAIN, NOS>(a, stream);
   switch (a.C) {
 #ifdef LGN_DEV_ONLY_C4
     LGN_CASE(4)
@@ -574,9 +590,11 @@
 
 template <>
 int level_fwd_dispatch<double>(const LevelArgs<double>& a, int decoder, hipStream_t stream) {
-  return level_fwd_run<true>(a, decoder, stream);
-}
-
-int level_fwd_eval(const LevelArgs<double>& a, int decoder, hipStream_t stream) { return level_fwd_run<false>(a, decoder, stream); }
-
-}
+  return a.dead_scalars ? level_fwd_run<true, true>(a, decoder, stream) : level_fwd_run<true, false>(a, decoder, stream);
+}
+
+int level_fwd_eval(const LevelArgs<double>& a, int decoder, hipStream_t stream) {
+  return a.dead_scalars ? level_fwd_run<false, true>(a, decoder, stream) : level_fwd_run<false, false>(a, decoder, stream);
+}
+
+}
diff --git a/lgn-autoencoder_amd/csrc/step.hip b/lgn-autoencoder_amd/csrc/step.hip
--- a/lgn-autoencoder_amd/csrc/step.hip
+++ b/lgn-autoencoder_amd/csrc/step.hip
@@ -271,8 +271,10 @@
       a.loss_part = loss->loss_part; a.loss_gv = loss->g_v; a.loss_wpart = loss->wpart;
     }
     a.flags = d.flags;
+    const bool no_mlp = l + 1 == d.n_levels && (!last_scalars || (eval && dec));
+    a.dead_scalars = no_mlp && !(d.flags & LVL_LIVE_SCALARS);
     LGN_TRY(eval ? level_fwd_eval(a, dec, st) : level_fwd_dispatch<double>(a, dec, st));
-    if (l + 1 == d.n_levels && (!last_scalars || (eval && dec))) break;
+    if (no_mlp) break;
     MlpArgs<double> m = level_mlp_args(d, dec, l, P, off);
     m.s_in = n.smix[l]; m.s_out = n.s[l + 1];
     m.h_saved = n.hsave[l]; m.h_rows = mlp_saved_rows(m.M);
@@ -312,6 +314,8 @@
                            p(S.rad(dec, l, 0)), p(S.rad(dec, l, 1)), p(S.rad(dec, l, 2)), p(S.rad(dec, l, 3)), p(S.rad(dec, l, 4)),
                            p(S.rad(dec, l, 5)), p(S.rad(dec, l, 6)), p(S.mix(dec, l, 0)), p(S.mix(dec, l, 1)), n.ag0[l], n.ag1[l],
                            g_smix, w.gv[cur], w.g_ag, w.gs[nxt], w.gv[nxt], dec ? w.g_p : nullptr, part_mix, part_rad};
+    const bool dead_s = !has_s_grad && !(d.flags & LVL_LIVE_SCALARS);
+    a.dead_scalars = dead_s;
     const bool carry_in0 = !dec && l == 0 && in0_done && level_bwd_carries_input(d.N, d.flags);
     const RowLayout rin = enc_input_rows(1, C);
     if (carry_in0) { DQ_TAKE(a.part_in0, (size_t)rm * rin.width); }
@@ -321,7 +325,8 @@
       rin.add(dq, a.part_in0, rm, G, off);
       *in0_done = true;
     }
-    dq.add(part_mix, rm, nmix, 0, nmix / 2, g(S.mix(dec, l, 0)));
+    if (dead_s) dq.add(nullptr, 0, 0, 0, nmix / 2, g(S.mix(dec, l, 0)));
+    else dq.add(part_mix, rm, nmix, 0, nmix / 2, g(S.mix(dec, l, 0)));
     dq.add(part_mix, rm, nmix, nmix / 2, nmix / 2, g(S.mix(dec, l, 1)));
     if (dec) {
       dq.add(part_rad, rr, nrad, 0, C, g(S.rad(dec, l, 4)));
diff --git a/lgn-autoencoder_amd/lgn/_native.py b/lgn-autoencoder_amd/lgn/_native.py
--- a/lgn-autoencoder_amd/lgn/_native.py
+++ b/lgn-autoencoder_amd/lgn/_native.py
@@ -107,7 +107,7 @@
 
 NET_NO_STATIC = 1
 _NET_FLAG_ENV = {"LGN_AMD_NO_STATIC": 1, "LGN_AMD_DEC_PAIRWISE": 2, "LGN_AMD_LEVEL_V2": 4, "LGN_AMD_MLP_V1": 8,
-                 "LGN_AMD_MOMENTS_V1": 16, "LGN_AMD_BWD_ORDERED": 64, "LGN_AMD_SPLIT_TAIL": 128, "LGN_AMD_DEC_UNFUSED": 256, "LGN_AMD_MOMENTS_SPLIT": 512,
+                 "LGN_AMD_MOMENTS_V1": 16, "LGN_AMD_BWD_ORDERED": 64, "LGN_AMD_LIVE_SCALARS": 4096, "LGN_AMD_SPLIT_TAIL": 128, "LGN_AMD_DEC_UNFUSED": 256, "LGN_AMD_MOMENTS_SPLIT": 512,
                  "LGN_AMD_MLP_BWD1": 1024, "LGN_AMD_MLP_FULLTILE": 2048}
 ACTIVATIONS = {"leakyrelu": 0, "relu": 1, "elu": 2, "sigmoid": 3, "logsigmoid": 4, "atan": 5}
 
```
